# 4l3x4ndre/Metadata-Augmented-UNET-for-LST-NDVI

Measured on AMD Instinct MI355X. Metric: train images/sec (256x256x6->2 U-Net, B=32/GPU), higher is better.
Workload: dtype bf16; 1 GPU; metadata-unet base_filters=64, 32x6x256x256 tiles + 4-dim metadata per GPU, fwd+MSE+bwd+AdamW (src/train.py:243-256); global_batch=32, parallelism=dp1, sync_bn=False, launch=hipGraph replay of the captured step

## Files before the change

### include/mau_hip.h

```cpp
#ifndef MAU_HIP_H
#define MAU_HIP_H

#include <stddef.h>
#include <stdint.h>

#ifdef __cplusplus
extern "C" {
#endif

#define MAU_F32 0
#define MAU_BF16 1
#define MAU_F16 2

#define MAU_OK 0
#define MAU_ERR_ARG 1
#define MAU_ERR_HIP 2
#define MAU_ERR_DEVICE 3

typedef void* mau_stream_t;

#define MAU_ABI_VERSION 5
int mau_abi_version(void);
const char* mau_last_error(void);
int mau_device_check(void);

int mau_nchw_to_nhwc(const float* src, void* dst, int dtype, int N, int C, int H, int W, int ld,
                     mau_stream_t stream);
int mau_nhwc_to_nchw(const void* src, float* dst, int dtype, int N, int C, int H, int W, int ld,
                     mau_stream_t stream);

int mau_pack_tile_onehot(const unsigned char* cls_a, const unsigned char* cls_b, const float* cont,
                         const unsigned char* flip, void* out, int ldo, int dtype, int N, int H, int W,
                         int num_classes, int ncont, mau_stream_t stream);
int mau_flip_rows(const float* src, float* dst, const unsigned char* flip, int N, int C, int H, int W,
                  mau_stream_t stream);

int mau_conv3x3_kc(int dtype);
size_t mau_conv3x3_packed_elems(int dtype, int nout, int nin);
int mau_conv3x3_pack_weights(const float* w_oihw, void* wf, void* wd, int dtype, int Cout, int Cin,
                             mau_stream_t stream);
size_t mau_conv3x3_pack_desc_bytes(void);
int mau_conv3x3_pack_desc_fill(void* descs_host, int index, const float* w_oihw, void* wf, void* wd, int dtype, int Cout,
                               int Cin, int tile0, int* next_tile_host);
int mau_conv3x3_pack_weights_multi(const void* descs, int n, int total_tiles, int dtype, mau_stream_t stream);
int mau_conv3x3_num_pixel_tiles(int dtype, int N, int H, int W, int Cout);
int mau_conv3x3_fwd_pool(const void* x, int ldx, int C0, const void* wpk, const float* bias, const float* post_scale,
                         const float* post_shift, void* y, int ldy, int Cout, void* pooled, int ldpool, int dtype, int N, int H,
                         int W, mau_stream_t stream);
int mau_conv3x3_variant(int dtype, int N, int H, int W, int Cin, int Cout, int* tile_rows_host, int* waves_host, int* cout_block_host,
                        int* k_groups_host);
int mau_conv3x3_first_max_channels(void);
int mau_conv3x3_first_rows(int N, int H, int W);
size_t mau_conv3x3_first_wgrad_ws_elems(int N, int H, int W, int Cout);
int mau_conv3x3_first_wgrad(const void* x8, const void* dz, int lddz, float* dw_oihw, float* ws, int Cin, int Cout, int dtype, int N,
                            int H, int W, mau_stream_t stream);
int mau_conv3x3_first_fwd(const float* x_nchw, int Cin, const float* w_oihw, const float* bias, const float* post_scale,
                          const float* post_shift, void* y, int ldy, int Cout, float* slab, void* x8, int dtype, int N, int H,
                          int W, mau_stream_t stream);
int mau_conv3x3_fwd(const void* x, int ldx, int C0, const float* emb, void* emb_ws, int E, const void* wpk,
                    const float* bias, const float* post_scale, const float* post_shift, void* y, int ldy,
                    int Cout, float* slab, int dtype, int N, int H, int W, mau_stream_t stream);
int mau_conv3x3_fwd2(const void* x, int ldx, int C0, const void* x1, int ldx1, int C1, const float* emb, void* emb_ws,
                     int E, const void* wpk, const float* bias, const float* post_scale, const float* post_shift,
                     void* y, int ldy, int Cout, float* slab, int dtype, int N, int H, int W, mau_stream_t stream);
int mau_conv3x3_wgrad_splits(int dtype, int N, int H, int W, int Cout, int Cin);
size_t mau_conv3x3_wgrad_acc_elems(int dtype, int N, int H, int W, int Cout, int Cin);
int mau_conv3x3_wgrad(const void* x, int ldx, int C0, const float* emb, void* emb_ws, int E, const void* dy,
                      int lddy, int Cout, float* acc, int dtype, int N, int H, int W, mau_stream_t stream);
int mau_conv3x3_wgrad2(const void* x, int ldx, int C0, const void* x1, int ldx1, int C1, const float* emb, void* emb_ws,
                       int E, const void* dy, int lddy, int Cout, float* acc, int dtype, int N, int H, int W,
                       mau_stream_t stream);
int mau_conv3x3_unpack_wgrad(const float* acc, int nsplit, float* dw_oihw, int Cout, int Cin,
                             mau_stream_t stream);

size_t mau_reduce_rows_ws_elems(int rows, int M);
int mau_reduce_tickets_elems(void);
int mau_reduce_rows_f64(const float* slab, int rows, int M, int ldrow, double* sums, double* ws, unsigned* tickets,
                        mau_stream_t stream);
int mau_reduce_rows_f64_f32(const float* slab, int rows, int M, int ldrow, double* sums, float* sums32,
                            double* ws, unsigned* tickets, double append, mau_stream_t stream);
int mau_reduce_rows_f32(const float* slab, int rows, int M, int ldrow, float* out, double* ws, unsigned* tickets,
                        mau_stream_t stream);
int mau_bn_stats_sums_f64(const float* slab, int rows, int C, double* sums, double* ws, unsigned* tickets, double append,
                          mau_stream_t stream);
int mau_bn_finalize_train(const double* sums, double count, const float* gamma, const float* beta,
                          float* running_mean, float* running_var, int64_t* num_batches_tracked,
                          float momentum, float eps, float* scale, float* shift, float* mean,
                          float* invstd, int C, mau_stream_t stream);
size_t mau_bn_stats_ws_elems(int rows, int C);
int mau_bn_stats_finalize_train(const float* slab, int rows, double count, const float* gamma, const float* beta,
                                float* running_mean, float* running_var, int64_t* num_batches_tracked,
                                float momentum, float eps, float* scale, float* shift, float* mean, float* invstd,
                                double* ws, unsigned* tickets, int C, mau_stream_t stream);
int mau_bn_coeffs_eval(const float* gamma, const float* beta, const float* running_mean,
                       const float* running_var, float eps, float* scale, float* shift, float* mean,
                       float* invstd, int C, mau_stream_t stream);
int mau_bn_relu_apply(const void* y, int ldy, const float* scale, const float* shift, void* a, int lda,
                      int dtype, int64_t npix, int C, mau_stream_t stream);
int mau_bn_relu_apply_pool(const void* y, int ldy, const float* scale, const float* shift, void* a, int lda,
                           void* pooled, int ldp, unsigned short* argidx, int dtype, int N, int H, int W, int C,
                           mau_stream_t stream);
int mau_bn_relu_bwd_reduce(const void* da, int ldda, const void* y, int ldy, const float* scale,
                           const float* shift, const float* mean, const float* invstd, float* slab,
                           int ldslab, int dtype, int64_t npix, int C, mau_stream_t stream);
int mau_bn_relu_bwd_apply(const void* da, int ldda, const void* y, int ldy, const float* scale,
                          const float* shift, const float* mean, const float* invstd, const double* sums,
                          double count, void* dy, int lddy, int dtype, int64_t npix, int C,
                          mau_stream_t stream);
int mau_bn_bwd_rows(int64_t npix);

int mau_pool_bn_bwd_reduce(const void* y, int ldy, const void* dpl, int lddpl, const unsigned short* argidx,
                           const void* dskip, int lddskip,
                           const float* scale, const float* shift, const float* mean, const float* invstd, float* slab,
                           int ldslab, int dtype, int N, int H, int W, int C, mau_stream_t stream);
int mau_pool_bn_bwd_apply(const void* y, int ldy, const void* dpl, int lddpl, const unsigned short* argidx,
                          const void* dskip, int lddskip,
                          const float* scale, const float* shift, const float* mean, const float* invstd,
                          const double* sums, double count, void* dy, int lddy, int dtype, int N, int H, int W, int C,
                          mau_stream_t stream);
int mau_head_bn_max_channels(void);
int mau_head_bn_fwd(const void* y, int ldy, const float* scale, const float* shift, const float* w, const float* b, float* out,
                    int tanh0, int dtype, int N, int HW, int C, int Co, mau_stream_t stream);
int mau_head_bn_bwd_reduce(const void* y, int ldy, const float* scale, const float* shift, const float* mean,
                           const float* invstd, const float* w, const float* out, const float* dout, float* bn_slab,
                           int ldslab, float* head_slab, int tanh0, int dtype, int N, int HW, int C, int Co,
                           mau_stream_t stream);
int mau_head_bn_bwd_apply(const void* y, int ldy, const float* scale, const float* shift, const float* mean,
                          const float* invstd, const double* sums, double count, const float* w, const float* out,
                          const float* dout, void* dy, int lddy, int tanh0, int dtype, int N, int HW, int C, int Co,
                          mau_stream_t stream);

int mau_sum_tensors_max(void);
int mau_sum_tensors(const void* const* srcs, const int* lds, int k, void* dst, int lddst, int dtype, int64_t npix, int C,
                    mau_stream_t stream);

int mau_emb_fold_fwd(const float* w, const float* emb, float* weff, int Cout, int Ct, int E, int N, int Ep, mau_stream_t stream);
size_t mau_emb_fold_ws_elems(int Cout, int N, int E);
int mau_emb_fold_bwd(const float* w, const float* emb, const float* dweff, float* dw, float* demb, float* ws, int Cout, int Ct, int E,
                     int N, int Ep, mau_stream_t stream);

int mau_maxpool2x2_fwd(const void* x, int ldx, void* y, int ldy, int dtype, int N, int H, int W, int C,
                       mau_stream_t stream);
int mau_maxpool2x2_bwd(const void* x, int ldx, const void* dy, int lddy, void* dx, int lddx, int dtype,
                       int N, int H, int W, int C, mau_stream_t stream);
int mau_maxpool2x2_bwd_add(const void* x, int ldx, const void* dy, int lddy, const void* dskip, int lddskip, void* dx,
                           int lddx, int dtype, int N, int H, int W, int C, mau_stream_t stream);

int mau_resize_bilinear_fwd(const void* src, int ldsrc, int h, int w, void* dst, int lddst, int choff,
                            int dtype, int N, int H, int W, int C, mau_stream_t stream);
int mau_resize_bilinear_bn_fwd(const void* y, int ldy, int h, int w, const float* scale, const float* shift, void* dst,
                               int lddst, int choff, int dtype, int N, int H, int W, int C, mau_stream_t stream);
int mau_resize_bilinear_bwd(const void* ddst, int ldddst, int choff, int H, int W, void* dsrc, int lddsrc,
                            int dtype, int N, int h, int w, int C, mau_stream_t stream);
#define MAU_RESIZE_FWD_ROWCOL 0
#define MAU_RESIZE_FWD_CELL 1
#define MAU_RESIZE_FWD_DEST 2
#define MAU_RESIZE_BWD_2X2 0
#define MAU_RESIZE_BWD_GATHER 1
int mau_resize_bilinear_plan(int N, int h, int w, int H, int W, int C, int* fwd_kernel_host, int* fwd_rows_host, int* bwd_kernel_host);
int mau_copy_channels(const void* src, int ldsrc, void* dst, int lddst, int choff, int zero_to, int dtype,
                      int64_t npix, int C, mau_stream_t stream);
int mau_bcast_fill(const float* emb, void* dst, int lddst, int choff, int zero_to, int dtype, int N, int HW,
                   int E, mau_stream_t stream);
size_t mau_bcast_bwd_ws_elems(int N, int HW, int E);
int mau_bcast_bwd(const void* dx, int lddx, int choff, float* demb, float* ws, int dtype, int N, int HW, int E,
                  mau_stream_t stream);

int mau_head_fwd(const void* a, int lda, const float* w, const float* b, float* out, int tanh0, int dtype,
                 int N, int HW, int C, int Co, mau_stream_t stream);
size_t mau_head_mean_ws_elems(int N, int HW, int Co);
int mau_head_mean(const void* a, int lda, const float* w, const float* b, const double* scale, const double* shift,
                  double* means, double* ws, unsigned* tickets, int tanh0, int dtype, int N, int HW, int C, int Co,
                  mau_stream_t stream);
int mau_head_bwd(const void* a, int lda, const float* w, const float* out, const float* dout, void* da,
                 int ldda, float* slab, int tanh0, int dtype, int N, int HW, int C, int Co,
                 mau_stream_t stream);
int mau_head_bwd_rows(int N, int HW);
int mau_head_bwd_rowlen(int C, int Co);

int mau_meta_mlp_fwd(const float* md, const float* w0, const float* b0, const float* w2, const float* b2,
                     float* hidden, float* emb, int N, int F, int Hd, int D, mau_stream_t stream);
int mau_meta_mlp_bwd(const float* md, const float* w0, const float* w2, const float* hidden,
                     const float* demb, float* dw0, float* db0, float* dw2, float* db2, float* dhidden_ws,
                     int N, int F, int Hd, int D, mau_stream_t stream);

int mau_lstm_max_hidden(void);
int mau_lstm_fwd(const float* x, const float* w_ih, const float* w_hh, const float* b_ih, const float* b_hh,
                 float* h_last, float* gates, float* cells, int B, int T, int H, mau_stream_t stream);
size_t mau_lstm_bwd_ws_elems(int B, int T, int H);
int mau_lstm_bwd(const float* x, const float* w_hh, const float* gates, const float* cells, const float* dh_last,
                 float* dw_ih, float* dw_hh, float* db_ih, float* db_hh, float* ws, int B, int T, int H,
                 mau_stream_t stream);

int mau_linear_fwd(const float* x, const float* w, const float* b, float* out, int N, int F, int D, mau_stream_t stream);
int mau_linear_bwd(const float* x, const float* w, const float* dout, float* dx, float* dw, float* db, int N, int F,
                   int D, mau_stream_t stream);

size_t mau_adamw_pack_desc_bytes(void);
int mau_adamw_pack_desc_fill(void* descs_host, int index, float* w, const float* grad, float* exp_avg, float* exp_avg_sq,
                             void* wf, void* wd, int Cout, int Cin, int tile0, int* next_tile_host);
int mau_adamw_pack_step(const void* descs, int n, int total_tiles, int dtype, const float* step, float lr, float beta1,
                        float beta2, float eps, float weight_decay, mau_stream_t stream);

#define MAU_OPT_ADAMW 0
#define MAU_OPT_ADAM 1
#define MAU_OPT_SGD 2
int mau_opt_pack_desc_fill(void* descs_host, int index, float* w, const float* grad, float* m, float* v, void* wf, void* wd,
                           int Cout, int Cin, int tile0, int* next_tile_host);
// ... 107 lines not shown
```

### metadata-augmented-unet-for-lst-ndvi_amd/_lib.py

```python
from __future__ import annotations

import ctypes as C
import os

import torch

_HERE = os.path.dirname(os.path.abspath(__file__))
LIB_PATH = os.environ.get("MAU_LIB") or os.path.join(_HERE, "libmau_hip.so")

MAU_F32 = 0
MAU_BF16 = 1
MAU_F16 = 2
MAU_OPT_ADAMW, MAU_OPT_ADAM, MAU_OPT_SGD = 0, 1, 2

_p, _i, _i64, _f, _d, _sz = C.c_void_p, C.c_int, C.c_int64, C.c_float, C.c_double, C.c_size_t

PROTOTYPES = {
    "mau_abi_version": (_i, []),
    "mau_last_error": (C.c_char_p, []),
    "mau_device_check": (_i, []),
    "mau_nchw_to_nhwc": (_i, [_p, _p, _i, _i, _i, _i, _i, _i, _p]),
    "mau_pack_tile_onehot": (_i, [_p, _p, _p, _p, _p, _i, _i, _i, _i, _i, _i, _i, _p]),
    "mau_flip_rows": (_i, [_p, _p, _p, _i, _i, _i, _i, _p]),
    "mau_nhwc_to_nchw": (_i, [_p, _p, _i, _i, _i, _i, _i, _i, _p]),
    "mau_conv3x3_kc": (_i, [_i]),
    "mau_conv3x3_packed_elems": (_sz, [_i, _i, _i]),
    "mau_conv3x3_pack_weights": (_i, [_p, _p, _p, _i, _i, _i, _p]),
    "mau_conv3x3_pack_desc_bytes": (_sz, []),
    "mau_conv3x3_pack_desc_fill": (_i, [_p, _i, _p, _p, _p, _i, _i, _i, _i, _p]),
    "mau_conv3x3_pack_weights_multi": (_i, [_p, _i, _i, _i, _p]),
    "mau_conv3x3_num_pixel_tiles": (_i, [_i, _i, _i, _i, _i]),
    "mau_conv3x3_variant": (_i, [_i, _i, _i, _i, _i, _i, _p, _p, _p, _p]),
    "mau_conv3x3_first_max_channels": (_i, []),
    "mau_conv3x3_first_rows": (_i, [_i, _i, _i]),
    "mau_conv3x3_first_wgrad_ws_elems": (_sz, [_i, _i, _i, _i]),
    "mau_conv3x3_first_wgrad": (_i, [_p, _p, _i, _p, _p, _i, _i, _i, _i, _i, _i, _p]),
    "mau_conv3x3_first_fwd": (_i, [_p, _i, _p, _p, _p, _p, _p, _i, _i, _p, _p, _i, _i, _i, _i, _p]),
    "mau_conv3x3_fwd": (_i, [_p, _i, _i, _p, _p, _i, _p, _p, _p, _p, _p, _i, _i, _p, _i, _i, _i, _i, _p]),
    "mau_conv3x3_fwd_pool": (_i, [_p, _i, _i, _p, _p, _p, _p, _p, _i, _i, _p, _i, _i, _i, _i, _i, _p]),
    "mau_conv3x3_fwd2": (_i, [_p, _i, _i, _p, _i, _i, _p, _p, _i, _p, _p, _p, _p, _p, _i, _i, _p, _i, _i, _i, _i, _p]),
    "mau_conv3x3_wgrad_splits": (_i, [_i, _i, _i, _i, _i, _i]),
    "mau_conv3x3_wgrad_acc_elems": (_sz, [_i, _i, _i, _i, _i, _i]),
    "mau_conv3x3_wgrad": (_i, [_p, _i, _i, _p, _p, _i, _p, _i, _i, _p, _i, _i, _i, _i, _p]),
    "mau_conv3x3_wgrad2": (_i, [_p, _i, _i, _p, _i, _i, _p, _p, _i, _p, _i, _i, _p, _i, _i, _i, _i, _p]),
    "mau_conv3x3_unpack_wgrad": (_i, [_p, _i, _p, _i, _i, _p]),
    "mau_reduce_rows_ws_elems": (_sz, [_i, _i]),
    "mau_reduce_tickets_elems": (_i, []),
    "mau_reduce_rows_f64": (_i, [_p, _i, _i, _i, _p, _p, _p, _p]),
    "mau_reduce_rows_f64_f32": (_i, [_p, _i, _i, _i, _p, _p, _p, _p, _d, _p]),
    "mau_reduce_rows_f32": (_i, [_p, _i, _i, _i, _p, _p, _p, _p]),
    "mau_bn_stats_sums_f64": (_i, [_p, _i, _i, _p, _p, _p, _d, _p]),
    "mau_bn_finalize_train": (_i, [_p, _d, _p, _p, _p, _p, _p, _f, _f, _p, _p, _p, _p, _i, _p]),
    "mau_bn_stats_ws_elems": (_sz, [_i, _i]),
    "mau_bn_stats_finalize_train": (_i, [_p, _i, _d, _p, _p, _p, _p, _p, _f, _f, _p, _p, _p, _p, _p, _p, _i, _p]),
    "mau_bn_coeffs_eval": (_i, [_p, _p, _p, _p, _f, _p, _p, _p, _p, _i, _p]),
    "mau_bn_relu_apply": (_i, [_p, _i, _p, _p, _p, _i, _i, _i64, _i, _p]),
    "mau_bn_relu_apply_pool": (_i, [_p, _i, _p, _p, _p, _i, _p, _i, _p, _i, _i, _i, _i, _i, _p]),
    "mau_bn_relu_bwd_reduce": (_i, [_p, _i, _p, _i, _p, _p, _p, _p, _p, _i, _i, _i64, _i, _p]),
    "mau_bn_relu_bwd_apply": (_i, [_p, _i, _p, _i, _p, _p, _p, _p, _p, _d, _p, _i, _i, _i64, _i, _p]),
    "mau_bn_bwd_rows": (_i, [_i64]),
    "mau_pool_bn_bwd_reduce": (_i, [_p, _i, _p, _i, _p, _p, _i, _p, _p, _p, _p, _p, _i, _i, _i, _i, _i, _i, _p]),
    "mau_pool_bn_bwd_apply": (_i, [_p, _i, _p, _i, _p, _p, _i, _p, _p, _p, _p, _p, _d, _p, _i, _i, _i, _i, _i, _i, _p]),
    "mau_head_bn_max_channels": (_i, []),
    "mau_head_bn_fwd": (_i, [_p, _i, _p, _p, _p, _p, _p, _i, _i, _i, _i, _i, _i, _p]),
    "mau_head_bn_bwd_reduce": (_i, [_p, _i, _p, _p, _p, _p, _p, _p, _p, _p, _i, _p, _i, _i, _i, _i, _i, _i, _p]),
    "mau_head_bn_bwd_apply": (_i, [_p, _i, _p, _p, _p, _p, _p, _d, _p, _p, _p, _p, _i, _i, _i, _i, _i, _i, _i, _p]),
    "mau_resize_bilinear_bn_fwd": (_i, [_p, _i, _i, _i, _p, _p, _p, _i, _i, _i, _i, _i, _i, _i, _p]),
    "mau_maxpool2x2_fwd": (_i, [_p, _i, _p, _i, _i, _i, _i, _i, _i, _p]),
    "mau_maxpool2x2_bwd": (_i, [_p, _i, _p, _i, _p, _i, _i, _i, _i, _i, _i, _p]),
    "mau_maxpool2x2_bwd_add": (_i, [_p, _i, _p, _i, _p, _i, _p, _i, _i, _i, _i, _i, _i, _p]),
    "mau_resize_bilinear_fwd": (_i, [_p, _i, _i, _i, _p, _i, _i, _i, _i, _i, _i, _i, _p]),
    "mau_resize_bilinear_bwd": (_i, [_p, _i, _i, _i, _i, _p, _i, _i, _i, _i, _i, _i, _p]),
    "mau_resize_bilinear_plan": (_i, [_i, _i, _i, _i, _i, _i, _p, _p, _p]),
    "mau_copy_channels": (_i, [_p, _i, _p, _i, _i, _i, _i, _i64, _i, _p]),
    "mau_bcast_fill": (_i, [_p, _p, _i, _i, _i, _i, _i, _i, _i, _p]),
    "mau_bcast_bwd_ws_elems": (_sz, [_i, _i, _i]),
    "mau_bcast_bwd": (_i, [_p, _i, _i, _p, _p, _i, _i, _i, _i, _p]),
    "mau_head_fwd": (_i, [_p, _i, _p, _p, _p, _i, _i, _i, _i, _i, _i, _p]),
    "mau_head_mean_ws_elems": (_sz, [_i, _i, _i]),
    "mau_head_mean": (_i, [_p, _i, _p, _p, _p, _p, _p, _p, _p, _i, _i, _i, _i, _i, _i, _p]),
    "mau_head_bwd": (_i, [_p, _i, _p, _p, _p, _p, _i, _p, _i, _i, _i, _i, _i, _i, _p]),
    "mau_head_bwd_rows": (_i, [_i, _i]),
    "mau_head_bwd_rowlen": (_i, [_i, _i]),
    "mau_meta_mlp_fwd": (_i, [_p, _p, _p, _p, _p, _p, _p, _i, _i, _i, _i, _p]),
    "mau_meta_mlp_bwd": (_i, [_p, _p, _p, _p, _p, _p, _p, _p, _p, _p, _i, _i, _i, _i, _p]),
    "mau_lstm_max_hidden": (_i, []),
    "mau_lstm_fwd": (_i, [_p, _p, _p, _p, _p, _p, _p, _p, _i, _i, _i, _p]),
    "mau_lstm_bwd_ws_elems": (_sz, [_i, _i, _i]),
    "mau_lstm_bwd": (_i, [_p, _p, _p, _p, _p, _p, _p, _p, _p, _p, _i, _i, _i, _p]),
    "mau_linear_fwd": (_i, [_p, _p, _p, _p, _i, _i, _i, _p]),
    "mau_linear_bwd": (_i, [_p, _p, _p, _p, _p, _p, _i, _i, _i, _p]),
    "mau_adamw_pack_desc_bytes": (_sz, []),
    "mau_adamw_pack_desc_fill": (_i, [_p, _i, _p, _p, _p, _p, _p, _p, _i, _i, _i, _p]),
    "mau_adamw_pack_step": (_i, [_p, _i, _i, _i, _p, _f, _f, _f, _f, _f, _p]),
    "mau_opt_pack_desc_fill": (_i, [_p, _i, _p, _p, _p, _p, _p, _p, _i, _i, _i, _p]),
    "mau_opt_pack_step": (_i, [_p, _i, _i, _i, _i, _p, _p, _f, _f, _f, _f, _f, _i, _p]),
    "mau_grad_norm_chunk": (_i, []),
    "mau_grad_norm_seg_bytes": (_sz, []),
    "mau_grad_norm_seg_fill": (_i, [_p, _i, _p, _i64, _i, _p]),
    "mau_grad_norm_clip": (_i, [_p, _i, _i, _p, _p, _f, _p, _p, _p]),
    "mau_sum_tensors_max": (_i, []),
    "mau_sum_tensors": (_i, [_p, _p, _i, _p, _i, _i, _i64, _i, _p]),
    "mau_emb_fold_fwd": (_i, [_p, _p, _p, _i, _i, _i, _i, _i, _p]),
    "mau_emb_fold_ws_elems": (_sz, [_i, _i, _i]),
    "mau_emb_fold_bwd": (_i, [_p, _p, _p, _p, _p, _p, _i, _i, _i, _i, _i, _p]),
    "mau_eval_metrics_row_elems": (_i, [_i]),
    "mau_eval_metrics_chunks": (_i, [_i, _i]),
    "mau_eval_metrics_ws_elems": (_sz, [_i, _i, _i, _i, _i]),
    "mau_eval_metrics": (_i, [_p, _p, _p, _p, _p, _p, _p, _p, _i, _i, _i, _i, _i, _p]),
    "mau_eval_metrics_multi_max_models": (_i, []),
    "mau_eval_metrics_multi_ws_elems": (_sz, [_i, _i, _i, _i, _i, _i]),
    "mau_eval_metrics_multi": (_i, [_p, _p, _p, _p, _p, _p, _p, _p, _i, _i, _i, _i, _i, _i, _p]),
    "mau_paired_groups": (_i, []),
    "mau_paired_entry_elems": (_i, [_i]),
    "mau_paired_table_elems": (_sz, [_i, _i, _i]),
    "mau_paired_accumulate": (_i, [_p, _p, _p, _i, _i, _i, _i, _p]),
    "mau_rank_tile": (_i, []),
    "mau_rank_max_samples": (_i, []),
    "mau_rank_table_elems": (_sz, [_i, _i]),
    "mau_rank_ws_elems": (_sz, [_i, _i]),
    "mau_rank_tests": (_i, [_p, _p, _p, _p, _i, _i, _i, _i, _p]),
    "mau_scenario_max_classes": (_i, []),
    "mau_scenario_pack": (_i, [_p, _p, _p, _p, _p, _p, _p, _p, _p, _p, _i, _p, _i, _i, _i, _i, _i, _i, _i, _p]),
    "mau_scenario_result_row_elems": (_i, []),
    "mau_scenario_result_chunks": (_i, [_i, _i]),
    "mau_scenario_result_ws_elems": (_sz, [_i, _i, _i]),
    "mau_scenario_result": (_i, [_p, _p, _p, _p, _d, _d, _p, _p, _p, _p, _p, _p, _i, _i, _i, _p]),
    "mau_region_gather": (_i, [_p, _p, _p, _p, _p, _p, _p, _p, _i, _i, _i, _i, _i, _i, _i, _p]),
    "mau_region_stitch": (_i, [_p, _p, _p, _p, _i, _i, _i, _i, _i, _i, _i, _p]),
    "mau_compare_row_elems": (_i, []),
    "mau_compare_chunks": (_i, [_i, _i]),
    "mau_compare_ws_elems": (_sz, [_i, _i, _i]),
    "mau_compare_result": (_i, [_p, _p, _d, _d, _p, _p, _p, _p, _p, _p, _i, _i, _i, _p]),
    "mau_compare_inputs": (_i, [_p, _p, _p, _p, _p, _p, _p, _p, _p, _p, _i, _i, _i, _p]),
    "mau_moments_row_elems": (_i, []),
    "mau_plane_moments_chunks": (_i, [_i64]),
    "mau_plane_moments_ws_elems": (_sz, [_i, _i, _i64]),
    "mau_plane_moments": (_i, [_p, _p, _p, _p, _i, _i, _i64, _p]),
    "mau_bin_moments_max_entries": (_i, []),
    "mau_bin_moments": (_i, [_p, _p, _i, _p, _p, _p, _p, _p, _i, _i, _i, _i, _p]),
    "mau_tile_stats_row_elems": (_i, []),
    "mau_tile_stats_ws_elems": (_sz, [_i, _i64]),
    "mau_tile_stats": (_i, [_p, _p, _p, _p, _p, _p, _p, _i, _i64, _i, _p]),
    "mau_raw_tile_row_elems": (_i, []),
    "mau_raw_tile_ws_elems": (_sz, [_i, _i64]),
    "mau_raw_tile_process": (_i, [_p, _p, _p, _p, _p, _p, _p, _p, _p, _p, _p, _p, _p, _i, _i64, _i, _p]),
    "mau_climate_row_elems": (_i, []),
    "mau_climate_series_max_months": (_i, []),
    "mau_climate_baseline": (_i, [_p, _p, _i, _i, _p]),
    "mau_climate_normalise": (_i, [_p, _p, _p, _i, _i, _p]),
    "mau_climate_series": (_i, [_p, _p, _p, _p, _p, _p, _i, _i, _i, _i, _p]),
    "mau_mse_blocks": (_i, [_i64]),
    "mau_l1_gradient_blocks": (_i, [_i64]),
    "mau_l1_gradient_loss": (_i, [_p, _p, _p, _p, _p, _f, _f, _i, _i, _i, _i, _p]),
    "mau_ssim_ws_elems": (_sz, [_i, _i, _i, _i]),
    "mau_ssim_loss": (_i, [_p, _p, _p, _p, _p, _i, _i, _i, _i, _i, _p]),
    "mau_mse_fwd_bwd": (_i, [_p, _p, _p, _p, _p, _i64, _p]),
    "mau_loss_terms_ws_elems": (_sz, [_i, _i, _i, _i]),
    "mau_loss_terms": (_i, [_p, _p, _p, _p, _p, _p, _p, _f, _f, _i, _i, _i, _i, _p]),
}


class MauError(RuntimeError):
    pass


def _load():
    if not os.path.exists(LIB_PATH):
        raise ImportError(
            f"{LIB_PATH} not found: the MI355X-native HIP library has not been built "
            f"(run `python -c 'import __graft_entry__ as g; g.build()'` or `make -C {os.path.join(_HERE, 'csrc')}`). "
            "There is no CPU or PyTorch fallback for this path.")
    lib = C.CDLL(LIB_PATH)
    missing = [n for n in PROTOTYPES if not hasattr(lib, n)]
    if missing:
        raise ImportError(f"{LIB_PATH} does not export {missing}; rebuild it")
    for name, (res, args) in PROTOTYPES.items():
        fn = getattr(lib, name)
        fn.restype = res
        fn.argtypes = args
    return lib


lib = _load()


def check(status: int, what: str = ""):
    if status != 0:
        msg = lib.mau_last_error()
# ... 22 lines not shown
```

### metadata-augmented-unet-for-lst-ndvi_amd/csrc/bn.hip

```cpp
#include <stdlib.h>
#include "mau_common.h"

namespace mau {

template <int G, typename Load>
__device__ __forceinline__ void ordered_group(int& k, int end, Load load, double& s0, double& s1) {
  for (; k + 8 * (G - 1) + 4 < end; k += 8 * G) {
    double a[G], b[G];
#pragma unroll
    for (int i = 0; i < G; ++i) {
      a[i] = load(k + 8 * i);
      b[i] = load(k + 8 * i + 4);
    }
#pragma unroll
    for (int i = 0; i < G; ++i) {
      s0 += a[i];
      s1 += b[i];
    }
  }
}
template <typename Load>
__device__ __forceinline__ void ordered_pair_sum(int first, int end, Load load, double& s0, double& s1) {
  int k = first;
  ordered_group<16>(k, end, load, s0, s1);
  ordered_group<4>(k, end, load, s0, s1);
  for (; k + 4 < end; k += 8) {
    s0 += load(k);
    s1 += load(k + 4);
  }
  if (k < end) s0 += load(k);
}

template <typename InT, typename OutT>
__global__ __launch_bounds__(256) void reduce_rows_kernel(const InT* __restrict__ slab, int rows, int M, int ldrow,
                                                          OutT* __restrict__ out, int ldout, float* __restrict__ out32) {
  __shared__ double part[4][64];
  const int col = blockIdx.x * 64 + (threadIdx.x & 63);
  const int rl = threadIdx.x >> 6;
  const int per = (rows + gridDim.y - 1) / gridDim.y;
  const int r0 = blockIdx.y * per, r1 = min(rows, r0 + per);
  double s0 = 0.0, s1 = 0.0;
  if (col < M) {
    if (r0 + rl < r1) ordered_pair_sum(r0 + rl, r1, [&](int r) { return (double)slab[(size_t)r * ldrow + col]; }, s0, s1);
  }
  part[rl][threadIdx.x & 63] = s0 + s1;
  __syncthreads();
  if (rl == 0 && col < M) {
    const double v = part[0][threadIdx.x] + part[1][threadIdx.x] + part[2][threadIdx.x] + part[3][threadIdx.x];
    out[(size_t)blockIdx.y * ldout + col] = (OutT)v;
    if (out32 != nullptr) out32[col] = (float)v;
  }
}

constexpr int REDUCE_MAX_CHUNKS = 128;
static int reduce_chunks(int rows) {
  int c = rows / 32;
  if (c > REDUCE_MAX_CHUNKS) c = REDUCE_MAX_CHUNKS;
  return c < 1 ? 1 : c;
}

template <typename OutT>
static int reduce_rows_launch(const float* slab, int rows, int M, int ldrow, OutT* out, double* ws, hipStream_t st,
                              float* out32 = nullptr) {
  const int chunks = reduce_chunks(rows);
  float* const none = nullptr;
  if (chunks == 1 || ws == nullptr) {
    MAU_LAUNCH((reduce_rows_kernel<float, OutT>), dim3(ceil_div(M, 64), 1), dim3(256), 0, st, slab, rows, M, ldrow, out, M, out32);
  } else {
    MAU_LAUNCH((reduce_rows_kernel<float, double>), dim3(ceil_div(M, 64), chunks), dim3(256), 0, st, slab, rows, M, ldrow, ws, M, none);
    MAU_LAUNCH((reduce_rows_kernel<double, OutT>), dim3(ceil_div(M, 64), 1), dim3(256), 0, st, (const double*)ws, chunks, M, M, out, M, out32);
  }
  return check_launch("reduce_rows_kernel");
}


template <typename OutT>
__global__ __launch_bounds__(256) void reduce_rows_fused_kernel(const float* __restrict__ slab, int rows, int M, int ldrow, int split,
                                                                int gap, double* __restrict__ part, unsigned* __restrict__ tickets,
                                                                OutT* __restrict__ out, float* __restrict__ out32, double append) {
  __shared__ double ps[4][64];
  const int cl = threadIdx.x & 63, rl = threadIdx.x >> 6;
  const int j = blockIdx.x * 64 + cl;
  const int col = j < split ? j : j - split + gap;
  const int chunks = gridDim.y;
  const int per = (rows + chunks - 1) / chunks;
  const int r0 = blockIdx.y * per, r1 = min(rows, r0 + per);
  double s0 = 0.0, s1 = 0.0;
  if (j < M) {
    if (r0 + rl < r1) ordered_pair_sum(r0 + rl, r1, [&](int r) { return (double)slab[(size_t)r * ldrow + col]; }, s0, s1);
  }
  ps[rl][cl] = s0 + s1;
  __syncthreads();
  if (rl == 0 && j < M) part[(size_t)blockIdx.y * M + j] = ps[0][cl] + ps[1][cl] + ps[2][cl] + ps[3][cl];
  if (!last_block_of(tickets + blockIdx.x, (unsigned)chunks)) return;
  s0 = s1 = 0.0;
  if (j < M) {
    if (rl < chunks) ordered_pair_sum(rl, chunks, [&](int k) { return part[(size_t)k * M + j]; }, s0, s1);
  }
  ps[rl][cl] = s0 + s1;
  __syncthreads();
  if (rl == 0 && j < M) {
    const double v = ps[0][cl] + ps[1][cl] + ps[2][cl] + ps[3][cl];
    out[j] = (OutT)v;
    if (out32 != nullptr) out32[j] = (float)v;
  }
  if (append > 0.0 && blockIdx.x == 0 && threadIdx.x == 0) out[M] = (OutT)append;
}

template <typename OutT>
static int reduce_rows_fused_launch(const float* slab, int rows, int M, int ldrow, int split, int gap, OutT* out, double* ws,
                                    unsigned* tickets, hipStream_t st, float* out32 = nullptr, double append = 0.0) {
  const int chunks = reduce_chunks(rows);
  MAU_LAUNCH((reduce_rows_fused_kernel<OutT>), dim3(ceil_div(M, 64), chunks), dim3(256), 0, st, slab, rows, M, ldrow, split, gap, ws,
             tickets, out, out32, append);
  return check_launch("reduce_rows_fused_kernel");
}

__global__ void bn_finalize_train_kernel(const double* __restrict__ sums, double count, const float* __restrict__ gamma,
                                         const float* __restrict__ beta, float* __restrict__ rmean, float* __restrict__ rvar,
                                         int64_t* nbt, float momentum, float eps, float* __restrict__ scale,
                                         float* __restrict__ shift, float* __restrict__ mean_o, float* __restrict__ invstd_o,
                                         int C) {
  const int c = blockIdx.x * blockDim.x + threadIdx.x;
  if (c == 0 && nbt) *nbt += 1;
  if (c >= C) return;
  if (count <= 0.0) count = sums[2 * C];
  const double mean = sums[c] / count;
  double var = sums[C + c] / count - mean * mean;
  if (var < 0.0) var = 0.0;
  const float invstd = (float)(1.0 / sqrt(var + (double)eps));
  const float sc = gamma[c] * invstd;
  scale[c] = sc;
  shift[c] = beta[c] - (float)mean * sc;
  mean_o[c] = (float)mean;
  invstd_o[c] = invstd;
  if (rmean) {
    const double unbiased = count > 1.0 ? var * (count / (count - 1.0)) : var;
    rmean[c] = (1.f - momentum) * rmean[c] + momentum * (float)mean;
    rvar[c] = (1.f - momentum) * rvar[c] + momentum * (float)unbiased;
  }
}

__global__ __launch_bounds__(256) void bn_finalize_from_partials_kernel(const double* __restrict__ part, int chunks, int ldp, double count,
                                                 const float* __restrict__ gamma, const float* __restrict__ beta,
                                                 float* __restrict__ rmean, float* __restrict__ rvar, int64_t* nbt, float momentum,
                                                 float eps, float* __restrict__ scale, float* __restrict__ shift,
                                                 float* __restrict__ mean_o, float* __restrict__ invstd_o, int C) {
  __shared__ double ps[4][64], pq[4][64];
  const int cl = threadIdx.x & 63, kl = threadIdx.x >> 6;
  const int c = blockIdx.x * 64 + cl;
  if (blockIdx.x == 0 && threadIdx.x == 0 && nbt) *nbt += 1;
  double s0 = 0.0, q0 = 0.0, s1 = 0.0, q1 = 0.0;
  if (c < C && kl < chunks) {
// ... 132 lines not shown
#pragma unroll
      for (int u = 0; u < 4; ++u) {
        F8 o;
#pragma unroll
        for (int j = 0; j < 8; ++j) o.v[j] = fmaxf(fmaf(v[u].v[j], sc[j], sh[j]), 0.f);
        store8<T>(a + (pix + u * m.PS) * lda + c, o);
      }
    }
    for (; pix < p1; pix += m.PS) {
      const F8 v = load8<T>(y + pix * ldy + c);
      F8 o;
#pragma unroll
      for (int j = 0; j < 8; ++j) o.v[j] = fmaxf(fmaf(v.v[j], sc[j], sh[j]), 0.f);
      store8<T>(a + pix * lda + c, o);
    }
  }
}

template <typename T>
__global__ __launch_bounds__(256) void bn_relu_apply_pool_kernel(const T* __restrict__ y, int ldy, const float* __restrict__ scale,
                                                                 const float* __restrict__ shift, T* __restrict__ a, int lda,
                                                                 T* __restrict__ pl, int ldp, unsigned short* __restrict__ argidx, int H, int W,
                                                                 int C, int C8) {
  const int nv = C8 >> 3, Wc = (W + 1) >> 1, Ho = H >> 1, Wo = W >> 1;
  const int idx = blockIdx.x * 256 + threadIdx.x;
  if (idx >= Wc * nv) return;
  const int xo = idx / nv, c = (idx - xo * nv) * 8;
  const int yo = blockIdx.y, n = blockIdx.z;
  float sc[8], sh[8];
#pragma unroll
  for (int j = 0; j < 8; ++j) {
    sc[j] = coef(scale, c + j, C);
    sh[j] = coef(shift, c + j, C);
  }
  const int y0 = 2 * yo, x0 = 2 * xo;
  const bool hasx = x0 + 1 < W, hasy = y0 + 1 < H;
  const size_t row0 = ((size_t)n * H + y0) * W, row1 = row0 + W;
  F8 v[4];
  v[0] = load8<T>(y + (row0 + x0) * ldy + c);
  v[1] = hasx ? load8<T>(y + (row0 + x0 + 1) * ldy + c) : zero8();
  v[2] = hasy ? load8<T>(y + (row1 + x0) * ldy + c) : zero8();
  v[3] = (hasx && hasy) ? load8<T>(y + (row1 + x0 + 1) * ldy + c) : zero8();
  F8 o[4];
#pragma unroll
  for (int u = 0; u < 4; ++u)
#pragma unroll
    for (int j = 0; j < 8; ++j) o[u].v[j] = fmaxf(fmaf(v[u].v[j], sc[j], sh[j]), 0.f);
  store8<T>(a + (row0 + x0) * lda + c, o[0]);
  if (hasx) store8<T>(a + (row0 + x0 + 1) * lda + c, o[1]);
  if (hasy) store8<T>(a + (row1 + x0) * lda + c, o[2]);
  if (hasx && hasy) store8<T>(a + (row1 + x0 + 1) * lda + c, o[3]);
  if (yo < Ho && xo < Wo) {
    F8 m;
    unsigned bits = 0;
#pragma unroll
    for (int j = 0; j < 8; ++j) {
      const float a0 = opaque((float)(T)opaque(o[0].v[j])), a1 = opaque((float)(T)opaque(o[1].v[j]));
      const float a2 = opaque((float)(T)opaque(o[2].v[j])), a3 = opaque((float)(T)opaque(o[3].v[j]));
      unsigned arg = 0;
      float mx = a0;
      arg = a1 > mx ? 1u : arg;
      mx = fmaxf(mx, a1);
      arg = a2 > mx ? 2u : arg;
      mx = fmaxf(mx, a2);
      arg = a3 > mx ? 3u : arg;
      mx = fmaxf(mx, a3);
      m.v[j] = mx;
      bits |= arg << (2 * j);
    }
    store8<T>(pl + (((size_t)n * Ho + yo) * Wo + xo) * ldp + c, m);
    if (argidx != nullptr) argidx[(((size_t)n * Ho + yo) * Wo + xo) * nv + (c >> 3)] = (unsigned short)bits;
  }
}


template <typename T>
__global__ __launch_bounds__(256) void bn_relu_bwd_reduce_kernel(const T* __restrict__ da, int ldda, const T* __restrict__ y,
                                                                 int ldy, const float* __restrict__ scale,
                                                                 const float* __restrict__ shift, const float* __restrict__ mean,
                                                                 const float* __restrict__ invstd, float* __restrict__ slab,
                                                                 int ldslab, int64_t npix, int C) {
  __shared__ float red[2][32][64 + 1];
  const int cv = threadIdx.x & 7, ps = threadIdx.x >> 3;
  const int c0 = blockIdx.y * 64 + cv * 8;
  const int64_t p0 = (int64_t)blockIdx.x * BWD_PIX_PER_BLOCK;
  const int64_t p1 = p0 + BWD_PIX_PER_BLOCK < npix ? p0 + BWD_PIX_PER_BLOCK : npix;
  float s1[8], s2[8], sc[8], sh[8], mu[8], is[8];
#pragma unroll
  for (int j = 0; j < 8; ++j) {
    s1[j] = s2[j] = 0.f;
    const int cc = c0 + j;
    sc[j] = coef(scale, cc, C);
    sh[j] = coef(shift, cc, C);
    mu[j] = coef(mean, cc, C);
    is[j] = coef(invstd, cc, C);
  }
  if (c0 < C) {
    int64_t p = p0 + ps;
    for (; p + 32 < p1; p += 64) {
      F8 g[2], v[2];
#pragma unroll
      for (int u = 0; u < 2; ++u) {
        g[u] = load8<T>(da + (p + 32 * u) * ldda + c0);
        v[u] = load8<T>(y + (p + 32 * u) * ldy + c0);
      }
#pragma unroll
      for (int u = 0; u < 2; ++u)
#pragma unroll
        for (int j = 0; j < 8; ++j) {
          const float act = fmaf(v[u].v[j], sc[j], sh[j]);
          const float dz = act > 0.f ? g[u].v[j] : 0.f;
          s1[j] += dz;
          s2[j] = fmaf(dz, (v[u].v[j] - mu[j]) * is[j], s2[j]);
        }
    }
    for (; p < p1; p += 32) {
      const F8 g = load8<T>(da + p * ldda + c0);
      const F8 v = load8<T>(y + p * ldy + c0);
#pragma unroll
      for (int j = 0; j < 8; ++j) {
        const float act = fmaf(v.v[j], sc[j], sh[j]);
        const float dz = act > 0.f ? g.v[j] : 0.f;
        s1[j] += dz;
        s2[j] = fmaf(dz, (v.v[j] - mu[j]) * is[j], s2[j]);
      }
    }
  }
#pragma unroll
  for (int j = 0; j < 8; ++j) {
    red[0][ps][cv * 8 + j] = s1[j];
    red[1][ps][cv * 8 + j] = s2[j];
  }
  __syncthreads();
  if (threadIdx.x < 128) {
    const int which = threadIdx.x >> 6, c = threadIdx.x & 63;
    float s = 0.f;
#pragma unroll 8
    for (int r = 0; r < 32; ++r) s += red[which][r][c];
    const int cc = blockIdx.y * 64 + c;
    if (cc < ldslab) slab[((size_t)blockIdx.x * 2 + which) * ldslab + cc] = s;
  }
}

template <typename T, bool NT>
__global__ __launch_bounds__(256) void bn_relu_bwd_apply_kernel(const T* __restrict__ da, int ldda, const T* __restrict__ y,
                                                                int ldy, const float* __restrict__ scale,
                                                                const float* __restrict__ shift, const float* __restrict__ mean,
                                                                const float* __restrict__ invstd, const double* __restrict__ sums,
                                                                double inv_count, T* __restrict__ dy, int lddy, int64_t npix,
                                                                int C, int C8, int pixb) {
  const int nv = C8 >> 3;
  const PixVec m(nv);
  if (m.ps >= m.PS) return;
  if (inv_count <= 0.0) inv_count = 1.0 / sums[2 * C];
  const int64_t p0 = (int64_t)blockIdx.x * pixb;
  const int64_t p1 = p0 + pixb < npix ? p0 + pixb : npix;
  for (int vv = m.v; vv < nv; vv += m.nvl) {
    const int c = vv * 8;
    float sc[8], sh[8], k0[8], k1[8];
    double d1[8], d2[8];
#pragma unroll
    for (int j = 0; j < 8; ++j) {
      sc[j] = coef(scale, c + j, C);
      sh[j] = coef(shift, c + j, C);
      k0[j] = coef(mean, c + j, C);
      k1[j] = coef(invstd, c + j, C);
      d1[j] = coef(sums, c + j, C);
      d2[j] = coef(sums + C, c + j, C);
    }
#pragma unroll
    for (int j = 0; j < 8; ++j) {
      const float mu = k0[j], is = k1[j];
      const float m1 = (float)(d1[j] * inv_count), m2 = (float)(d2[j] * inv_count);
      k1[j] = __fmul_rn(__fmul_rn(sc[j], m2), is);
      k0[j] = fmaf(sc[j], m1, -__fmul_rn(k1[j], mu));
    }
    int64_t pix = p0 + m.ps;
    for (; pix + 3 * m.PS < p1; pix += 4 * m.PS) {
      F8 g[4], v[4];
#pragma unroll
      for (int u = 0; u < 4; ++u) {
        g[u] = NT ? load8_nt<T>(da + (pix + u * m.PS) * ldda + c) : load8<T>(da + (pix + u * m.PS) * ldda + c);
        v[u] = NT ? load8_nt<T>(y + (pix + u * m.PS) * ldy + c) : load8<T>(y + (pix + u * m.PS) * ldy + c);
      }
#pragma unroll
      for (int u = 0; u < 4; ++u) {
        F8 o;
#pragma unroll
        for (int j = 0; j < 8; ++j) {
          const float act = fmaf(v[u].v[j], sc[j], sh[j]);
          const float dz = act > 0.f ? g[u].v[j] : 0.f;
          o.v[j] = fmaf(sc[j], dz, -fmaf(k1[j], v[u].v[j], k0[j]));
        }
        if (NT) store8_nt<T>(dy + (pix + u * m.PS) * lddy + c, o); else store8<T>(dy + (pix + u * m.PS) * lddy + c, o);
      }
    }
    for (; pix < p1; pix += m.PS) {
      const F8 g = load8<T>(da + pix * ldda + c);
      const F8 v = load8<T>(y + pix * ldy + c);
      F8 o;
#pragma unroll
      for (int j = 0; j < 8; ++j) {
        const float act = fmaf(v.v[j], sc[j], sh[j]);
        const float dz = act > 0.f ? g.v[j] : 0.f;
        o.v[j] = fmaf(sc[j], dz, -fmaf(k1[j], v.v[j], k0[j]));
      }
      store8<T>(dy + pix * lddy + c, o);
    }
  }
}

}

using namespace mau;

extern "C" {

size_t mau_reduce_rows_ws_elems(int rows, int M) { return (size_t)reduce_chunks(rows) * M; }

int mau_reduce_tickets_elems(void) { return 64; }

#define MAU_REQUIRE_TICKETS(M) MAU_REQUIRE(tickets == nullptr || ceil_div((M), 64) <= mau_reduce_tickets_elems(), "reduce_rows: more than 4096 columns")

int mau_reduce_rows_f64(const float* slab, int rows, int M, int ldrow, double* sums, double* ws, unsigned* tickets,
                        mau_stream_t stream) {
  MAU_REQUIRE(slab && sums && rows > 0 && M > 0 && ldrow >= M, "reduce_rows: bad arguments");
  MAU_REQUIRE_TICKETS(M);
  if (tickets && ws) return reduce_rows_fused_launch<double>(slab, rows, M, ldrow, M, 0, sums, ws, tickets, (hipStream_t)stream);
  return reduce_rows_launch<double>(slab, rows, M, ldrow, sums, ws, (hipStream_t)stream);
}

int mau_reduce_rows_f64_f32(const float* slab, int rows, int M, int ldrow, double* sums, float* sums32, double* ws,
                            unsigned* tickets, double append, mau_stream_t stream) {
  MAU_REQUIRE(slab && sums && sums32 && rows > 0 && M > 0 && ldrow >= M, "reduce_rows: bad arguments");
  MAU_REQUIRE_TICKETS(M);
  MAU_REQUIRE(append <= 0.0 || (tickets && ws), "reduce_rows: the appended count needs the single-launch form (ws and tickets)");
  if (tickets && ws)
    return reduce_rows_fused_launch<double>(slab, rows, M, ldrow, M, 0, sums, ws, tickets, (hipStream_t)stream, sums32, append);
  return reduce_rows_launch<double>(slab, rows, M, ldrow, sums, ws, (hipStream_t)stream, sums32);
}

int mau_reduce_rows_f32(const float* slab, int rows, int M, int ldrow, float* out, double* ws, unsigned* tickets,
                        mau_stream_t stream) {
  MAU_REQUIRE(slab && out && rows > 0 && M > 0 && ldrow >= M, "reduce_rows: bad arguments");
  MAU_REQUIRE_TICKETS(M);
  if (tickets && ws) return reduce_rows_fused_launch<float>(slab, rows, M, ldrow, M, 0, out, ws, tickets, (hipStream_t)stream);
  return reduce_rows_launch<float>(slab, rows, M, ldrow, out, ws, (hipStream_t)stream);
}

int mau_bn_stats_sums_f64(const float* slab, int rows, int C, double* sums, double* ws, unsigned* tickets, double append,
                          mau_stream_t stream) {
  MAU_REQUIRE(slab && sums && ws && tickets && rows > 0 && C > 0, "bn_stats_sums: bad arguments");
  MAU_REQUIRE_TICKETS(2 * C);
  const int cpad = round_up(C, 64);
  return reduce_rows_fused_launch<double>(slab, rows, 2 * C, 2 * cpad, C, cpad, sums, ws, tickets, (hipStream_t)stream, nullptr, append);
}

int mau_bn_finalize_train(const double* sums, double count, const float* gamma, const float* beta,
                          float* running_mean, float* running_var, int64_t* nbt, float momentum, float eps,
                          float* scale, float* shift, float* mean, float* invstd, int C, mau_stream_t stream) {
  MAU_REQUIRE(sums && gamma && beta && scale && shift && mean && invstd && C > 0 && count >= 0, "bn_finalize_train: bad arguments");
  MAU_REQUIRE((running_mean == nullptr) == (running_var == nullptr), "bn_finalize_train: running_mean/var must come together");
  MAU_LAUNCH(bn_finalize_train_kernel, dim3(ceil_div(C, 256)), dim3(256), 0, (hipStream_t)stream, sums, count, gamma,
                     beta, running_mean, running_var, nbt, momentum, eps, scale, shift, mean, invstd, C);
  return check_launch("bn_finalize_train_kernel");
}

size_t mau_bn_stats_ws_elems(int rows, int C) { return (size_t)reduce_chunks(rows) * 2 * round_up(C, 64); }

int mau_bn_stats_finalize_train(const float* slab, int rows, double count, const float* gamma, const float* beta,
                                float* running_mean, float* running_var, int64_t* nbt, float momentum, float eps,
                                float* scale, float* shift, float* mean, float* invstd, double* ws, unsigned* tickets, int C,
                                mau_stream_t stream) {
  MAU_REQUIRE(slab && ws && gamma && beta && scale && shift && mean && invstd && rows > 0 && C > 0 && count > 0, "bn_stats_finalize_train: bad arguments");
  MAU_REQUIRE((running_mean == nullptr) == (running_var == nullptr), "bn_stats_finalize_train: running_mean/var must come together");
  hipStream_t st = (hipStream_t)stream;
  const int cpad = round_up(C, 64), M = 2 * cpad, chunks = reduce_chunks(rows);
  MAU_REQUIRE_TICKETS(cpad);
  if (tickets) {
    MAU_LAUNCH(bn_stats_finalize_fused_kernel, dim3(cpad / 64, chunks), dim3(256), 0, st, slab, rows, cpad, ws, tickets, count, gamma,
               beta, running_mean, running_var, nbt, momentum, eps, scale, shift, mean, invstd, C);
    return check_launch("bn_stats_finalize_fused_kernel");
  }
  MAU_LAUNCH((reduce_rows_kernel<float, double>), dim3(ceil_div(M, 64), chunks), dim3(256), 0, st, slab, rows, M, M, ws, M, (float*)nullptr);
  MAU_LAUNCH(bn_finalize_from_partials_kernel, dim3(ceil_div(C, 64)), dim3(256), 0, st, (const double*)ws, chunks, cpad, count, gamma,
             beta, running_mean, running_var, nbt, momentum, eps, scale, shift, mean, invstd, C);
  return check_launch("bn_stats_finalize_train");
}

int mau_bn_coeffs_eval(const float* gamma, const float* beta, const float* running_mean, const float* running_var,
                       float eps, float* scale, float* shift, float* mean, float* invstd, int C, mau_stream_t stream) {
  MAU_REQUIRE(gamma && beta && running_mean && running_var && scale && shift && C > 0, "bn_coeffs_eval: bad arguments");
  MAU_LAUNCH(bn_coeffs_eval_kernel, dim3(ceil_div(C, 256)), dim3(256), 0, (hipStream_t)stream, gamma, beta,
                     running_mean, running_var, eps, scale, shift, mean, invstd, C);
  return check_launch("bn_coeffs_eval_kernel");
}

int mau_bn_relu_apply(const void* y, int ldy, const float* scale, const float* shift, void* a, int lda, int dtype,
                      int64_t npix, int C, mau_stream_t stream) {
  MAU_REQUIRE(y && a && scale && shift && npix > 0 && C > 0, "bn_relu_apply: bad arguments");
  const int C8 = round_up(C, 8);
  MAU_REQUIRE(ldy % 8 == 0 && lda % 8 == 0 && ldy >= C8 && lda >= C8, "bn_relu_apply: bad ld");
  const bool big = npix >= (int64_t)1 << 20;
  const int pixb = pixvec_pixels_per_block(C8 / 8, npix, big ? 8 : 32, big ? 2048 : 256);
  MAU_DISPATCH_DTYPE(dtype, MAU_LAUNCH(bn_relu_apply_kernel<T>, dim3(ceil_div(npix, pixb)), dim3(256), 0, (hipStream_t)stream,
                                               (const T*)y, ldy, scale, shift, (T*)a, lda, npix, C, C8, pixb));
  return check_launch("bn_relu_apply_kernel");
}

int mau_bn_relu_apply_pool(const void* y, int ldy, const float* scale, const float* shift, void* a, int lda, void* pooled,
                           int ldp, unsigned short* argidx, int dtype, int N, int H, int W, int C, mau_stream_t stream) {
  MAU_REQUIRE(y && a && pooled && scale && shift && N > 0 && H >= 2 && W >= 2 && C > 0, "bn_relu_apply_pool: bad arguments");
  const int C8 = round_up(C, 8);
  MAU_REQUIRE(ldy % 8 == 0 && lda % 8 == 0 && ldp % 8 == 0 && ldy >= C8 && lda >= C8 && ldp >= C8, "bn_relu_apply_pool: bad ld");
  MAU_REQUIRE((H + 1) / 2 <= 65535 && N <= 65535, "bn_relu_apply_pool: H/2 and N must fit a grid dimension");
  dim3 grid(ceil_div(((W + 1) / 2) * (C8 / 8), 256), (H + 1) / 2, N);
  MAU_DISPATCH_DTYPE(dtype, MAU_LAUNCH(bn_relu_apply_pool_kernel<T>, grid, dim3(256), 0, (hipStream_t)stream, (const T*)y, ldy, scale,
                                       shift, (T*)a, lda, (T*)pooled, ldp, argidx, H, W, C, C8));
  return check_launch("bn_relu_apply_pool_kernel");
}

int mau_bn_bwd_rows(int64_t npix) { return ceil_div(npix, BWD_PIX_PER_BLOCK); }

int mau_bn_relu_bwd_reduce(const void* da, int ldda, const void* y, int ldy, const float* scale, const float* shift,
                           const float* mean, const float* invstd, float* slab, int ldslab, int dtype, int64_t npix,
                           int C, mau_stream_t stream) {
  MAU_REQUIRE(da && y && scale && shift && mean && invstd && slab && npix > 0 && C > 0, "bn_relu_bwd_reduce: bad arguments");
  const int C8 = round_up(C, 8);
  MAU_REQUIRE(ldda % 8 == 0 && ldy % 8 == 0 && ldda >= C8 && ldy >= C8 && ldslab >= C, "bn_relu_bwd_reduce: bad ld");
  dim3 grid(mau_bn_bwd_rows(npix), ceil_div(C, 64));
  MAU_DISPATCH_DTYPE(dtype, MAU_LAUNCH(bn_relu_bwd_reduce_kernel<T>, grid, dim3(256), 0, (hipStream_t)stream,
                                               (const T*)da, ldda, (const T*)y, ldy, scale, shift, mean, invstd, slab,
                                               ldslab, npix, C));
  return check_launch("bn_relu_bwd_reduce_kernel");
}

int mau_bn_relu_bwd_apply(const void* da, int ldda, const void* y, int ldy, const float* scale, const float* shift,
                          const float* mean, const float* invstd, const double* sums, double count, void* dy, int lddy,
                          int dtype, int64_t npix, int C, mau_stream_t stream) {
  MAU_REQUIRE(da && y && dy && sums && scale && shift && mean && invstd && npix > 0 && C > 0 && count >= 0, "bn_relu_bwd_apply: bad arguments");
  const int C8 = round_up(C, 8);
  MAU_REQUIRE(ldda % 8 == 0 && ldy % 8 == 0 && lddy % 8 == 0 && ldda >= C8 && ldy >= C8 && lddy >= C8, "bn_relu_bwd_apply: bad ld");
  const int pixb = pixvec_pixels_per_block(C8 / 8, npix, 64, 256);
  MAU_DISPATCH_DTYPE(dtype, MAU_LAUNCH((bn_relu_bwd_apply_kernel<T, false>), dim3(ceil_div(npix, pixb)), dim3(256), 0, (hipStream_t)stream,
                                               (const T*)da, ldda, (const T*)y, ldy, scale, shift, mean, invstd, sums,
                                               count > 0 ? 1.0 / count : 0.0, (T*)dy, lddy, npix, C, C8, pixb));
  return check_launch("bn_relu_bwd_apply_kernel");
}

}
```

### metadata-augmented-unet-for-lst-ndvi_amd/csrc/bn_fused.hip

```cpp
#include "mau_common.h"

namespace mau {

template <typename T>
__device__ __forceinline__ float round_to(float v) {
  return opaque((float)(T)opaque(v));
}

typedef float f2 __attribute__((ext_vector_type(2)));
__device__ __forceinline__ f2 pk_fma(f2 a, f2 b, f2 c) { return __builtin_elementwise_fma(a, b, c); }
__device__ __forceinline__ f2 splat(float v) { return f2{v, v}; }
template <typename T>
__device__ __forceinline__ f2 round_to2(f2 v) {
  if constexpr (sizeof(T) == 4) return v;
  else if constexpr (__is_same(T, bf16)) {
    typedef __bf16 b2 __attribute__((ext_vector_type(2)));
    asm("" : "+v"(v));
    f2 r = __builtin_convertvector(__builtin_convertvector(v, b2), f2);
    asm("" : "+v"(r));
    return r;
  } else return f2{round_to<T>(v[0]), round_to<T>(v[1])};
}
template <typename T>
struct P4 {
  f2 p[4];
  __device__ __forceinline__ static P4 load(const T* ptr) {
    const F8 v = load8<T>(ptr);
    P4 r;
#pragma unroll
    for (int i = 0; i < 4; ++i) r.p[i] = f2{v.v[2 * i], v.v[2 * i + 1]};
    return r;
  }
};

struct Coef8 {
  float sc[8], sh[8], mu[8], is[8];
  __device__ __forceinline__ void load(const float* scale, const float* shift, const float* mean, const float* invstd, int c0, int C) {
#pragma unroll
    for (int j = 0; j < 8; ++j) {
      sc[j] = coef(scale, c0 + j, C);
      sh[j] = coef(shift, c0 + j, C);
      mu[j] = mean ? coef(mean, c0 + j, C) : 0.f;
      is[j] = invstd ? coef(invstd, c0 + j, C) : 0.f;
    }
  }
};

template <typename T>
struct PoolLoads {
  F8 g, sk;
  unsigned bits;
  bool inpool;
  int me;
};
template <typename T, bool POOL, bool SKIP>
__device__ __forceinline__ PoolLoads<T> pool_load(const T* __restrict__ dpl, int lddpl, const unsigned short* __restrict__ argidx, int nv,
                                                  const T* __restrict__ dskip, int lddskip, int n, int yi, int xi, int H, int W, int c0) {
  PoolLoads<T> L;
  const int Ho = H >> 1, Wo = W >> 1, yo = yi >> 1, xo = xi >> 1;
  L.inpool = POOL && yo < Ho && xo < Wo;
  L.me = (yi & 1) * 2 + (xi & 1);
  L.bits = 0;
  if constexpr (POOL) {
    const int yc = yo < Ho ? yo : Ho - 1, xc = xo < Wo ? xo : Wo - 1;
    const size_t win = ((size_t)n * Ho + yc) * Wo + xc;
    L.g = load8<T>(dpl + win * lddpl + c0);
    L.bits = argidx[win * nv + (c0 >> 3)];
  }
  if constexpr (SKIP) L.sk = load8<T>(dskip + (((size_t)n * H + yi) * W + xi) * lddskip + c0);
  return L;
}
template <typename T, bool POOL, bool SKIP>
__device__ __forceinline__ F8 pool_eval(const PoolLoads<T>& L) {
  F8 o;
#pragma unroll
  for (int j = 0; j < 8; ++j) {
    float r = 0.f;
    if constexpr (POOL) r = (L.inpool && (int)((L.bits >> (2 * j)) & 3u) == L.me) ? L.g.v[j] : 0.f;
    if constexpr (SKIP) r += L.sk.v[j];
    o.v[j] = round_to<T>(r);
  }
  return o;
}

__device__ __forceinline__ void bn_sums_to_slab(float (*red)[32][64 + 1], const float* s1, const float* s2, int cv, int ps, float* slab,
                                                int ldslab) {
#pragma unroll
  for (int j = 0; j < 8; ++j) {
    red[0][ps][cv * 8 + j] = s1[j];
    red[1][ps][cv * 8 + j] = s2[j];
  }
  __syncthreads();
  if (threadIdx.x < 128) {
    const int which = threadIdx.x >> 6, c = threadIdx.x & 63;
    float s = 0.f;
#pragma unroll 8
    for (int r = 0; r < 32; ++r) s += red[which][r][c];
    const int cc = blockIdx.y * 64 + c;
    if (cc < ldslab) slab[((size_t)blockIdx.x * 2 + which) * ldslab + cc] = s;
  }
}

__device__ __forceinline__ void advance32(int& n, int& yi, int& xi, int H, int W) {
  xi += 32;
  while (xi >= W) {
    xi -= W;
    if (++yi == H) {
      yi = 0;
      ++n;
    }
  }
}
template <typename T, bool POOL, bool SKIP>
__global__ __launch_bounds__(256) void pool_bn_bwd_reduce_kernel(const T* __restrict__ y, int ldy, const T* __restrict__ dpl, int lddpl,
                                                                 const unsigned short* __restrict__ argidx,
                                                                 const T* __restrict__ dskip, int lddskip, const float* __restrict__ scale,
                                                                 const float* __restrict__ shift, const float* __restrict__ mean,
                                                                 const float* __restrict__ invstd, float* __restrict__ slab, int ldslab,
                                                                 int H, int W, int64_t npix, int C) {
  __shared__ float red[2][32][64 + 1];
  const int cv = threadIdx.x & 7, ps = threadIdx.x >> 3;
  const int c0 = blockIdx.y * 64 + cv * 8;
  const int64_t p0 = (int64_t)blockIdx.x * BWD_PIX_PER_BLOCK;
  const int64_t p1 = p0 + BWD_PIX_PER_BLOCK < npix ? p0 + BWD_PIX_PER_BLOCK : npix;
  Coef8 k;
  k.load(scale, shift, mean, invstd, c0, C);
  float s1[8], s2[8];
#pragma unroll
  for (int j = 0; j < 8; ++j) s1[j] = s2[j] = 0.f;
  auto accumulate = [&](const F8& v, const F8& g) {
#pragma unroll
    for (int j = 0; j < 8; ++j) {
      const float act = fmaf(v.v[j], k.sc[j], k.sh[j]);
      const float dz = act > 0.f ? g.v[j] : 0.f;
      s1[j] += dz;
      s2[j] = fmaf(dz, (v.v[j] - k.mu[j]) * k.is[j], s2[j]);
    }
  };
  if (c0 < C) {
    int64_t p = p0 + ps;
    const int HW = H * W, nv = (C + 7) >> 3;
    int n = (int)(p / HW), r = (int)(p - (int64_t)n * HW);
    int yi = r / W, xi = r - yi * W;
    for (; p + 32 < p1; p += 64) {
      int n2 = n, yi2 = yi, xi2 = xi;
      advance32(n2, yi2, xi2, H, W);
      const F8 va = load8<T>(y + p * ldy + c0), vb = load8<T>(y + (p + 32) * ldy + c0);
      const PoolLoads<T> La = pool_load<T, POOL, SKIP>(dpl, lddpl, argidx, nv, dskip, lddskip, n, yi, xi, H, W, c0);
      const PoolLoads<T> Lb = pool_load<T, POOL, SKIP>(dpl, lddpl, argidx, nv, dskip, lddskip, n2, yi2, xi2, H, W, c0);
      accumulate(va, pool_eval<T, POOL, SKIP>(La));
      accumulate(vb, pool_eval<T, POOL, SKIP>(Lb));
      n = n2, yi = yi2, xi = xi2;
      advance32(n, yi, xi, H, W);
    }
    for (; p < p1; p += 32) {
      const F8 v = load8<T>(y + p * ldy + c0);
      const PoolLoads<T> L = pool_load<T, POOL, SKIP>(dpl, lddpl, argidx, nv, dskip, lddskip, n, yi, xi, H, W, c0);
      accumulate(v, pool_eval<T, POOL, SKIP>(L));
      advance32(n, yi, xi, H, W);
    }
  }
  bn_sums_to_slab(red, s1, s2, cv, ps, slab, ldslab);
}

struct Apply8 {
  float sc[8], sh[8], k0[8], k1[8];
  __device__ __forceinline__ void load(const float* scale, const float* shift, const float* mean, const float* invstd, const double* sums,
                                       double inv_count, int c0, int C) {
    double d1[8], d2[8];
#pragma unroll
    for (int j = 0; j < 8; ++j) {
      sc[j] = coef(scale, c0 + j, C);
      sh[j] = coef(shift, c0 + j, C);
      k0[j] = coef(mean, c0 + j, C);
      k1[j] = coef(invstd, c0 + j, C);
      d1[j] = coef(sums, c0 + j, C);
      d2[j] = coef(sums + C, c0 + j, C);
    }
#pragma unroll
    for (int j = 0; j < 8; ++j) {
      const float mu = k0[j], is = k1[j];
      const float m1 = (float)(d1[j] * inv_count), m2 = (float)(d2[j] * inv_count);
      k1[j] = __fmul_rn(__fmul_rn(sc[j], m2), is);
      k0[j] = fmaf(sc[j], m1, -__fmul_rn(k1[j], mu));
    }
  }
  __device__ __forceinline__ float dy(int j, float yv, float da) const {
    const float act = fmaf(yv, sc[j], sh[j]);
    const float dz = act > 0.f ? da : 0.f;
    return fmaf(sc[j], dz, -fmaf(k1[j], yv, k0[j]));
  }
};

template <typename T, bool POOL, bool SKIP>
__global__ __launch_bounds__(256) void pool_bn_bwd_apply_kernel(const T* __restrict__ y, int ldy, const T* __restrict__ dpl, int lddpl,
                                                                const unsigned short* __restrict__ argidx,
                                                                const T* __restrict__ dskip, int lddskip, const float* __restrict__ scale,
                                                                const float* __restrict__ shift, const float* __restrict__ mean,
                                                                const float* __restrict__ invstd, const double* __restrict__ sums,
                                                                double inv_count, T* __restrict__ dyo, int lddy, int H, int W, int C, int C8,
                                                                int RY) {
  const int nv = C8 >> 3, Wc = (W + 1) >> 1, Hc = (H + 1) >> 1, Ho = H >> 1, Wo = W >> 1;
  const int idx = blockIdx.x * 256 + threadIdx.x;
  if (idx >= Wc * nv) return;
  const int xo = idx / nv, c = (idx - xo * nv) * 8;
  const int n = blockIdx.z;
  if (inv_count <= 0.0) inv_count = 1.0 / sums[2 * C];
  Apply8 k;
  k.load(scale, shift, mean, invstd, sums, inv_count, c, C);
  const int x0 = 2 * xo;
  const bool hasx = x0 + 1 < W;
  const int x1 = hasx ? x0 + 1 : x0;
  const int xpc = xo < Wo ? xo : Wo - 1;
  for (int yo = blockIdx.y * RY; yo < min(Hc, (int)(blockIdx.y + 1) * RY); ++yo) {
    const int y0 = 2 * yo;
    const bool hasy = y0 + 1 < H;
    const size_t row0 = ((size_t)n * H + y0) * W, row1 = ((size_t)n * H + (hasy ? y0 + 1 : y0)) * W;
    F8 v[4], d[4], g;
    v[0] = load8<T>(y + (row0 + x0) * ldy + c);
    v[1] = load8<T>(y + (row0 + x1) * ldy + c);
    v[2] = load8<T>(y + (row1 + x0) * ldy + c);
    v[3] = load8<T>(y + (row1 + x1) * ldy + c);
    if constexpr (SKIP) {
      d[0] = load8<T>(dskip + (row0 + x0) * lddskip + c);
      d[1] = load8<T>(dskip + (row0 + x1) * lddskip + c);
      d[2] = load8<T>(dskip + (row1 + x0) * lddskip + c);
      d[3] = load8<T>(dskip + (row1 + x1) * lddskip + c);
    }
    const bool inpool = POOL && yo < Ho && xo < Wo;
    unsigned bits = 0;
    if constexpr (POOL) {
      const size_t win = ((size_t)n * Ho + (yo < Ho ? yo : Ho - 1)) * Wo + xpc;
      g = load8<T>(dpl + win * lddpl + c);
      bits = argidx[win * nv + (c >> 3)];
    }
    F8 o[4];
#pragma unroll
    for (int j = 0; j < 8; ++j) {
      const int arg = inpool ? (int)((bits >> (2 * j)) & 3u) : -1;
#pragma unroll
      for (int u = 0; u < 4; ++u) {
        float r = 0.f;
        if constexpr (POOL) r = arg == u ? g.v[j] : 0.f;
        if constexpr (SKIP) r += d[u].v[j];
        o[u].v[j] = k.dy(j, v[u].v[j], round_to<T>(r));
      }
    }
    store8<T>(dyo + (row0 + x0) * lddy + c, o[0]);
    if (hasx) store8<T>(dyo + (row0 + x0 + 1) * lddy + c, o[1]);
    if (hasy) store8<T>(dyo + (row1 + x0) * lddy + c, o[2]);
    if (hasx && hasy) store8<T>(dyo + (row1 + x0 + 1) * lddy + c, o[3]);
  }
}

__device__ __forceinline__ void pos_step32(int& n, int& q, int HW) {
  q += 32;
  const bool w = q >= HW;
  q -= w ? HW : 0;
  n += w ? 1 : 0;
}

template <typename T, int MC, bool EX, bool BN = true>
__global__ __launch_bounds__(256) void head_bn_fwd_kernel(const T* __restrict__ y, int ldy, const float* __restrict__ scale,
                                                          const float* __restrict__ shift, const float* __restrict__ w,
                                                          const float* __restrict__ b, float* __restrict__ out, int tanh0, int HW, int C,
                                                          int Co, int64_t npix, int pixb) {
  const int sub = threadIdx.x & 7, ps = threadIdx.x >> 3;
  float wr[MC][8];
#pragma unroll
  for (int o = 0; o < MC; ++o)
#pragma unroll
    for (int j = 0; j < 8; ++j) wr[o][j] = (EX || o < Co) ? coef(w + o * C, sub * 8 + j, C) : 0.f;
  Coef8 k;
  if (BN) k.load(scale, shift, nullptr, nullptr, sub * 8, C);
  float bo[MC];
#pragma unroll
  for (int o = 0; o < MC; ++o) bo[o] = (EX || o < Co) ? b[o] : 0.f;
  const int64_t p0 = (int64_t)blockIdx.x * pixb;
  const int64_t p1 = p0 + pixb < npix ? p0 + pixb : npix;
  int n = (int)((p0 + ps) / HW);
  int q = (int)((p0 + ps) - (int64_t)n * HW);
  for (int64_t p = p0 + ps; p - ps < p1; p += 128) {
    F8 x[4];
    int nn[4], qq[4];
#pragma unroll
    for (int u = 0; u < 4; ++u) {
      const int64_t pix = p + 32 * u;
      const int64_t pc = pix < npix ? pix : npix - 1;
      x[u] = load8<T>(y + pc * ldy + (sub * 8 < C ? sub * 8 : 0));
      nn[u] = n;
      qq[u] = q;
      pos_step32(n, q, HW);
    }
    float acc[4][MC];
#pragma unroll
    for (int u = 0; u < 4; ++u) {
#pragma unroll
      for (int o = 0; o < MC; ++o) acc[u][o] = 0.f;
      if (sub * 8 < C) {
#pragma unroll
        for (int j = 0; j < 8; ++j) {
          const float a = BN ? round_to<T>(fmaxf(fmaf(x[u].v[j], k.sc[j], k.sh[j]), 0.f)) : x[u].v[j];
#pragma unroll
          for (int o = 0; o < MC; ++o) acc[u][o] = fmaf(a, wr[o][j], acc[u][o]);
        }
      }
#pragma unroll
      for (int o = 0; o < MC; ++o) {
        acc[u][o] += __shfl_xor(acc[u][o], 1);
        acc[u][o] += __shfl_xor(acc[u][o], 2);
        acc[u][o] += __shfl_xor(acc[u][o], 4);
      }
    }
    const int us = sub & 3;
    const int nu = us == 0 ? nn[0] : us == 1 ? nn[1] : us == 2 ? nn[2] : nn[3];
    const int qu = us == 0 ? qq[0] : us == 1 ? qq[1] : us == 2 ? qq[2] : qq[3];
    const bool live = sub < 4 && p + 32 * us < p1;
#pragma unroll
    for (int o = 0; o < MC; ++o) {
      if (EX || o < Co) {
        float r = us == 0 ? acc[0][o] : us == 1 ? acc[1][o] : us == 2 ? acc[2][o] : acc[3][o];
        r += bo[o];
        if (o == 0 && tanh0) r = tanhf(r);
        if (live) out[((size_t)nu * Co + o) * HW + qu] = r;
      }
    }
  }
}

template <int MC, bool EX>
__device__ __forceinline__ void head_dz(const float* __restrict__ out, const float* __restrict__ dout, int tanh0, int Co, int HW, int n,
                                        int q, float* dz) {
  const size_t base = (size_t)n * Co * HW + q;
  const float t = out[base];
  const float f0 = tanh0 ? fmaf(-t, t, 1.f) : 1.f;
#pragma unroll
  for (int o = 0; o < MC; ++o) {
    const float g = dout[base + (size_t)((EX || o < Co) ? o : Co - 1) * HW];
    dz[o] = (EX || o < Co) ? (o == 0 ? g * f0 : g) : 0.f;
  }
}

constexpr int HEAD_WAVES = 3;
template <typename T, int MC, bool EX>
__global__ __launch_bounds__(256, HEAD_WAVES) void head_bn_bwd_reduce_kernel(const T* __restrict__ y, int ldy, const float* __restrict__ scale,
                                                                 const float* __restrict__ shift, const float* __restrict__ mean,
                                                                 const float* __restrict__ invstd, const float* __restrict__ w,
                                                                 const float* __restrict__ out, const float* __restrict__ dout,
                                                                 float* __restrict__ bn_slab, int ldslab, float* __restrict__ head_slab,
                                                                 int tanh0, int HW, int C, int C8, int Co, int64_t npix) {
  __shared__ float red[2][32][64 + 1];
  __shared__ float hred[32 * HEAD_MAX_CO * 65];
  const int cv = threadIdx.x & 7, ps = threadIdx.x >> 3;
  const int c0 = cv * 8;
  const int64_t p0 = (int64_t)blockIdx.x * BWD_PIX_PER_BLOCK;
  const int64_t p1 = p0 + BWD_PIX_PER_BLOCK < npix ? p0 + BWD_PIX_PER_BLOCK : npix;
  const int rowlen = Co * (C8 + 8);
  float* row = head_slab + (size_t)blockIdx.x * rowlen;
  Coef8 k;
  k.load(scale, shift, mean, invstd, c0, C);
  f2 sc2[4], sh2[4], mu2[4], is2[4], s1p[4], s2p[4], dwq[MC][4], wq[MC][4];
  float dbp[MC];
#pragma unroll
  for (int i = 0; i < 4; ++i) {
    sc2[i] = f2{k.sc[2 * i], k.sc[2 * i + 1]};
    sh2[i] = f2{k.sh[2 * i], k.sh[2 * i + 1]};
    mu2[i] = f2{k.mu[2 * i], k.mu[2 * i + 1]};
    is2[i] = f2{k.is[2 * i], k.is[2 * i + 1]};
    s1p[i] = s2p[i] = f2{0.f, 0.f};
  }
#pragma unroll
  for (int o = 0; o < MC; ++o) {
    dbp[o] = 0.f;
#pragma unroll
    for (int i = 0; i < 4; ++i) {
      dwq[o][i] = f2{0.f, 0.f};
      wq[o][i] = f2{o < Co ? coef(w + o * C, c0 + 2 * i, C) : 0.f, o < Co ? coef(w + o * C, c0 + 2 * i + 1, C) : 0.f};
    }
  }
  auto one = [&](const P4<T>& v, const float* dz) {
#pragma unroll
    for (int o = 0; o < MC; ++o) dbp[o] += dz[o];
#pragma unroll
    for (int i = 0; i < 4; ++i) {
      const f2 act = pk_fma(v.p[i], sc2[i], sh2[i]);
      const f2 a = round_to2<T>(f2{fmaxf(act[0], 0.f), fmaxf(act[1], 0.f)});
      f2 s = f2{0.f, 0.f};
#pragma unroll
      for (int o = 0; o < MC; ++o)
        if (EX || o < Co) {
          s = pk_fma(splat(dz[o]), wq[o][i], s);
          dwq[o][i] = pk_fma(splat(dz[o]), a, dwq[o][i]);
        }
      const f2 da = round_to2<T>(s);
      const f2 dzb = f2{act[0] > 0.f ? da[0] : 0.f, act[1] > 0.f ? da[1] : 0.f};
      s1p[i] += dzb;
      s2p[i] = pk_fma(dzb, (v.p[i] - mu2[i]) * is2[i], s2p[i]);
    }
  };
  struct Raw {
    P4<T> v;
    float t, g[MC];
  };
  auto fetch = [&](int64_t pa, int na, int qa, Raw& r) {
    r.v = P4<T>::load(y + pa * ldy + c0);
    const size_t base = (size_t)na * Co * HW + qa;
    r.t = out[base];
#pragma unroll
    for (int o = 0; o < MC; ++o) r.g[o] = dout[base + (size_t)((EX || o < Co) ? o : Co - 1) * HW];
  };
  auto eval = [&](const Raw& r) {
    float dz[MC];
    const float f0 = tanh0 ? fmaf(-r.t, r.t, 1.f) : 1.f;
#pragma unroll
    for (int o = 0; o < MC; ++o) dz[o] = (EX || o < Co) ? (o == 0 ? r.g[o] * f0 : r.g[o]) : 0.f;
    one(r.v, dz);
  };
  if (c0 < C8) {
    int n = (int)((p0 + ps) / HW);
    int q = (int)((p0 + ps) - (int64_t)n * HW);
    int64_t p = p0 + ps;
    if (p + 32 < p1) {
      Raw a, b;
      int n2 = n, q2 = q;
      pos_step32(n2, q2, HW);
      fetch(p, n, q, a);
      fetch(p + 32, n2, q2, b);
      n = n2;
      q = q2;
      pos_step32(n, q, HW);
      for (; p + 96 < p1; p += 64) {
        Raw na, nb;
        n2 = n;
        q2 = q;
        pos_step32(n2, q2, HW);
        fetch(p + 64, n, q, na);
        fetch(p + 96, n2, q2, nb);
        eval(a);
        eval(b);
        a = na;
        b = nb;
        n = n2;
        q = q2;
        pos_step32(n, q, HW);
      }
      eval(a);
      eval(b);
      p += 64;
    }
    for (; p < p1; p += 32) {
      Raw r;
      fetch(p, n, q, r);
      eval(r);
      pos_step32(n, q, HW);
    }
  }
  float s1[8], s2[8], dwp[MC][8];
#pragma unroll
  for (int i = 0; i < 4; ++i) {
    s1[2 * i] = s1p[i][0];
    s1[2 * i + 1] = s1p[i][1];
    s2[2 * i] = s2p[i][0];
    s2[2 * i + 1] = s2p[i][1];
#pragma unroll
    for (int o = 0; o < MC; ++o) {
      dwp[o][2 * i] = dwq[o][i][0];
      dwp[o][2 * i + 1] = dwq[o][i][1];
    }
  }
#pragma unroll
  for (int o = 0; o < MC; ++o)
    if (EX || o < Co) {
#pragma unroll
      for (int j = 0; j < 8; ++j) hred[(ps * HEAD_MAX_CO + o) * 65 + cv * 8 + j] = dwp[o][j];
    }
  __syncthreads();
  for (int t = threadIdx.x; t < Co * 64; t += 256) {
    const int o = t >> 6, c = t & 63;
    float s = 0.f;
    for (int r = 0; r < 32; ++r) s += hred[(r * HEAD_MAX_CO + o) * 65 + c];
    if (c < C8) row[o * (C8 + 8) + c] = s;
  }
  __syncthreads();
  if (cv == 0) {
#pragma unroll
    for (int o = 0; o < MC; ++o)
      if (o < Co) hred[ps * HEAD_MAX_CO + o] = dbp[o];
  }
  __syncthreads();
  if (threadIdx.x < Co) {
    float s = 0.f;
    for (int r = 0; r < 32; ++r) s += hred[r * HEAD_MAX_CO + threadIdx.x];
    row[threadIdx.x * (C8 + 8) + C8] = s;
  }
  bn_sums_to_slab(red, s1, s2, cv, ps, bn_slab, ldslab);
}

template <typename T, int MC, bool EX>
__global__ __launch_bounds__(256) void head_bn_bwd_apply_kernel(const T* __restrict__ y, int ldy, const float* __restrict__ scale,
                                                                const float* __restrict__ shift, const float* __restrict__ mean,
                                                                const float* __restrict__ invstd, const double* __restrict__ sums,
                                                                double inv_count, const float* __restrict__ w, const float* __restrict__ out,
                                                                const float* __restrict__ dout, T* __restrict__ dyo, int lddy, int tanh0,
                                                                int HW, int C, int Co, int64_t npix, int pixb) {
  const int cv = threadIdx.x & 7, ps = threadIdx.x >> 3;
  const int c0 = cv * 8;
  if (c0 >= ((C + 7) & ~7)) return;
  if (inv_count <= 0.0) inv_count = 1.0 / sums[2 * C];
  Apply8 k;
  k.load(scale, shift, mean, invstd, sums, inv_count, c0, C);
  float wr[MC][8];
#pragma unroll
  for (int o = 0; o < MC; ++o)
#pragma unroll
    for (int j = 0; j < 8; ++j) wr[o][j] = o < Co ? coef(w + o * C, c0 + j, C) : 0.f;
  const int64_t p0 = (int64_t)blockIdx.x * pixb;
  const int64_t p1 = p0 + pixb < npix ? p0 + pixb : npix;
  int n = (int)((p0 + ps) / HW);
  int q = (int)((p0 + ps) - (int64_t)n * HW);
  auto one = [&](int64_t p, const F8& v, const float* dz) {
    F8 o8;
#pragma unroll
    for (int j = 0; j < 8; ++j) {
      float s = 0.f;
#pragma unroll
      for (int o = 0; o < MC; ++o)
        if (EX || o < Co) s = fmaf(dz[o], wr[o][j], s);
      o8.v[j] = k.dy(j, v.v[j], round_to<T>(s));
    }
    store8<T>(dyo + p * lddy + c0, o8);
  };
  int64_t p = p0 + ps;
  for (; p + 96 < p1; p += 128) {
    int nn[4], qq[4];
    F8 v[4];
    float dz[4][MC];
#pragma unroll
    for (int u = 0; u < 4; ++u) {
      nn[u] = n;
      qq[u] = q;
      pos_step32(n, q, HW);
    }
#pragma unroll
    for (int u = 0; u < 4; ++u) {
      v[u] = load8<T>(y + (p + 32 * u) * ldy + c0);
      head_dz<MC, EX>(out, dout, tanh0, Co, HW, nn[u], qq[u], dz[u]);
    }
#pragma unroll
    for (int u = 0; u < 4; ++u) one(p + 32 * u, v[u], dz[u]);
  }
  for (; p < p1; p += 32) {
    float dz[MC];
    const F8 v = load8<T>(y + p * ldy + c0);
    head_dz<MC, EX>(out, dout, tanh0, Co, HW, n, q, dz);
    one(p, v, dz);
    pos_step32(n, q, HW);
  }
}

int head_fwd_fast(const void* a, int lda, const float* w, const float* b, float* out, int tanh0, int dtype, int64_t npix, int HW, int C, int Co,
                  hipStream_t stream) {
  const int pixb = npix >= ((int64_t)1 << 20) ? 1024 : 128;
  const dim3 grid(ceil_div(npix, pixb));
  const float* none = nullptr;
#define MAU_HEAD_PLAIN(MC_, EX_)                                                                                                            \
  MAU_DISPATCH_DTYPE(dtype, MAU_LAUNCH((head_bn_fwd_kernel<T, MC_, EX_, false>), grid, dim3(256), 0, stream, (const T*)a, lda, none, none, w, b, out, \
                                       tanh0, HW, C, Co, npix, pixb))
  if (Co == 2) MAU_HEAD_PLAIN(2, true);
  else if (Co == 1) MAU_HEAD_PLAIN(2, false);
  else if (Co == HEAD_MAX_CO) MAU_HEAD_PLAIN(HEAD_MAX_CO, true);
  else MAU_HEAD_PLAIN(HEAD_MAX_CO, false);
#undef MAU_HEAD_PLAIN
  return check_launch("head_fwd_kernel");
}

}

using namespace mau;

extern "C" {

int mau_pool_bn_bwd_reduce(const void* y, int ldy, const void* dpl, int lddpl, const unsigned short* argidx, const void* dskip, int lddskip, const float* scale,
                           const float* shift, const float* mean, const float* invstd, float* slab, int ldslab, int dtype, int N, int H,
                           int W, int C, mau_stream_t stream) {
  MAU_REQUIRE(y && (dpl || dskip) && (!dpl || argidx) && scale && shift && mean && invstd && slab && N > 0 && H >= 2 && W >= 2 && C > 0, "pool_bn_bwd_reduce: bad arguments");
  const int C8 = round_up(C, 8);
  MAU_REQUIRE(ldy % 8 == 0 && ldy >= C8 && (!dpl || (lddpl % 8 == 0 && lddpl >= C8)) && (!dskip || (lddskip % 8 == 0 && lddskip >= C8)) && ldslab >= C,
              "pool_bn_bwd_reduce: bad ld");
  const int64_t npix = (int64_t)N * H * W;
  dim3 grid(ceil_div(npix, BWD_PIX_PER_BLOCK), ceil_div(C, 64));
#define MAU_POOL_REDUCE(P, S)                                                                                                                  \
  MAU_DISPATCH_DTYPE(dtype, MAU_LAUNCH((pool_bn_bwd_reduce_kernel<T, P, S>), grid, dim3(256), 0, (hipStream_t)stream, (const T*)y, ldy, (const T*)dpl, \
                                       lddpl, argidx, (const T*)dskip, lddskip, scale, shift, mean, invstd, slab, ldslab, H, W, npix, C))
  if (dpl && dskip) MAU_POOL_REDUCE(true, true);
  else if (dpl) MAU_POOL_REDUCE(true, false);
  else MAU_POOL_REDUCE(false, true);
#undef MAU_POOL_REDUCE
  return check_launch("pool_bn_bwd_reduce_kernel");
}

int mau_pool_bn_bwd_apply(const void* y, int ldy, const void* dpl, int lddpl, const unsigned short* argidx, const void* dskip, int lddskip, const float* scale,
                          const float* shift, const float* mean, const float* invstd, const double* sums, double count, void* dy, int lddy,
                          int dtype, int N, int H, int W, int C, mau_stream_t stream) {
  MAU_REQUIRE(y && (dpl || dskip) && (!dpl || argidx) && dy && sums && scale && shift && mean && invstd && N > 0 && H >= 2 && W >= 2 && C > 0 && count >= 0,
              "pool_bn_bwd_apply: bad arguments");
  const int C8 = round_up(C, 8);
  MAU_REQUIRE(ldy % 8 == 0 && ldy >= C8 && lddy % 8 == 0 && lddy >= C8 && (!dpl || (lddpl % 8 == 0 && lddpl >= C8)) &&
                  (!dskip || (lddskip % 8 == 0 && lddskip >= C8)), "pool_bn_bwd_apply: bad ld");
  MAU_REQUIRE((H + 1) / 2 <= 65535 && N <= 65535, "pool_bn_bwd_apply: H/2 and N must fit a grid dimension");
  const int xb = ceil_div(((W + 1) / 2) * (C8 / 8), 256), Hc = (H + 1) / 2;
  int RY = 8;
  while (RY > 1 && (int64_t)xb * ceil_div(Hc, RY) * N < 1024) RY >>= 1;
  dim3 grid(xb, ceil_div(Hc, RY), N);
#define MAU_POOL_APPLY(P, S)                                                                                                                   \
  MAU_DISPATCH_DTYPE(dtype, MAU_LAUNCH((pool_bn_bwd_apply_kernel<T, P, S>), grid, dim3(256), 0, (hipStream_t)stream, (const T*)y, ldy, (const T*)dpl, lddpl, \
                                       argidx, (const T*)dskip, lddskip, scale, shift, mean, invstd, sums, count > 0 ? 1.0 / count : 0.0, (T*)dy, lddy, \
                                       H, W, C, C8, RY))
  if (dpl && dskip) MAU_POOL_APPLY(true, true);
  else if (dpl) MAU_POOL_APPLY(true, false);
  else MAU_POOL_APPLY(false, true);
#undef MAU_POOL_APPLY
  return check_launch("pool_bn_bwd_apply_kernel");
}

int mau_head_bn_max_channels(void) { return 64; }

int mau_head_bn_fwd(const void* y, int ldy, const float* scale, const float* shift, const float* w, const float* b, float* out, int tanh0,
                    int dtype, int N, int HW, int C, int Co, mau_stream_t stream) {
  MAU_REQUIRE(y && scale && shift && w && b && out && N > 0 && HW > 0 && C > 0, "head_bn_fwd: bad arguments");
  MAU_REQUIRE(Co >= 1 && Co <= HEAD_MAX_CO && C <= mau_head_bn_max_channels(), "head_bn_fwd: out_channels in [1,%d], C <= %d", HEAD_MAX_CO,
              mau_head_bn_max_channels());
  MAU_REQUIRE(ldy % 8 == 0 && ldy >= round_up(C, 8), "head_bn_fwd: bad ld");
  MAU_REQUIRE(HW >= 32 && (int64_t)N * HW < ((int64_t)1 << 31), "head_bn_fwd: images of at least 32 pixels, fewer than 2^31 pixels in all");
  const int64_t npix = (int64_t)N * HW;
  const int pixb = npix >= ((int64_t)1 << 20) ? 1024 : 128;
  const dim3 grid(ceil_div(npix, pixb));
#define MAU_HEAD_FWD(MC_, EX_)                                                                                                              \
  MAU_DISPATCH_DTYPE(dtype, MAU_LAUNCH((head_bn_fwd_kernel<T, MC_, EX_>), grid, dim3(256), 0, (hipStream_t)stream, (const T*)y, ldy, scale, shift, w, b, \
                                       out, tanh0, HW, C, Co, npix, pixb))
  if (Co == 2) MAU_HEAD_FWD(2, true);
  else if (Co == 1) MAU_HEAD_FWD(2, false);
  else if (Co == HEAD_MAX_CO) MAU_HEAD_FWD(HEAD_MAX_CO, true);
  else MAU_HEAD_FWD(HEAD_MAX_CO, false);
#undef MAU_HEAD_FWD
  return check_launch("head_bn_fwd_kernel");
}

int mau_head_bn_bwd_reduce(const void* y, int ldy, const float* scale, const float* shift, const float* mean, const float* invstd,
                           const float* w, const float* out, const float* dout, float* bn_slab, int ldslab, float* head_slab, int tanh0,
                           int dtype, int N, int HW, int C, int Co, mau_stream_t stream) {
  MAU_REQUIRE(y && scale && shift && mean && invstd && w && out && dout && bn_slab && head_slab && N > 0 && HW > 0 && C > 0,
              "head_bn_bwd_reduce: bad arguments");
  MAU_REQUIRE(Co >= 1 && Co <= HEAD_MAX_CO && C <= mau_head_bn_max_channels(), "head_bn_bwd_reduce: out_channels in [1,%d], C <= %d", HEAD_MAX_CO,
              mau_head_bn_max_channels());
  const int C8 = round_up(C, 8);
  MAU_REQUIRE(ldy % 8 == 0 && ldy >= C8 && ldslab >= C, "head_bn_bwd_reduce: bad ld");
  MAU_REQUIRE(HW >= 32 && (int64_t)N * HW < ((int64_t)1 << 31), "head_bn_bwd_reduce: images of at least 32 pixels, fewer than 2^31 pixels in all");
  const int64_t npix = (int64_t)N * HW;
#define MAU_HEAD_RED(MC_, EX_)                                                                                                              \
  MAU_DISPATCH_DTYPE(dtype, MAU_LAUNCH((head_bn_bwd_reduce_kernel<T, MC_, EX_>), dim3(ceil_div(npix, BWD_PIX_PER_BLOCK)), dim3(256), 0, (hipStream_t)stream, \
                                       (const T*)y, ldy, scale, shift, mean, invstd, w, out, dout, bn_slab, ldslab, head_slab, tanh0, HW, C, C8, Co, npix))
// ... 33 lines not shown
```

### metadata-augmented-unet-for-lst-ndvi_amd/csrc/conv3x3_first.hip

```cpp
#include "igemm_bf16_util.h"

namespace mau {
namespace first {
using namespace igemm;

constexpr int TH = 16, TW = 64, HR = TH + 2, HC = TW + 2, HPIX = HR * HC;
constexpr int NT = 256, NWAVE = NT / 64;
constexpr int LOADS = (HPIX + NT - 1) / NT;
typedef float f32x4v __attribute__((ext_vector_type(4)));

struct P {
  const float* x;
  int Cin;
  const float* w;
  const float* bias;
  const float* post_scale;
  const float* post_shift;
  void* y;
  int ldy, Cout, CoutPad;
  float* slab;
  void* x8;
  int N, H, W, tilesX, tilesY, nTiles;
};

template <bool F16>
__device__ __forceinline__ f32x4v mfma(const bf16x8& a, const bf16x8& b, f32x4v c) {
  if constexpr (F16) return __builtin_amdgcn_mfma_f32_16x16x32_f16(__builtin_bit_cast(f16x8, a), __builtin_bit_cast(f16x8, b), c, 0, 0, 0);
  else return __builtin_amdgcn_mfma_f32_16x16x32_bf16(a, b, c, 0, 0, 0);
}

template <bool F16>
__device__ __forceinline__ u32x4 pack8(const float (&v)[8]) {
  u32x4 r;
#pragma unroll
  for (int i = 0; i < 4; ++i) {
    if constexpr (F16) r[i] = pack_lp2<true>(f32x2{opaque(v[2 * i]), opaque(v[2 * i + 1])});
    else r[i] = pack_lp2<false>(f32x2{v[2 * i], v[2 * i + 1]});
  }
  return r;
}

__device__ __forceinline__ int chan_of(int t, int q, int r) { return 32 * (t >> 1) + 8 * q + 4 * (t & 1) + r; }

constexpr int FIRST_UNROLL = 2;
constexpr int FIRST_WAVES = 2;
template <bool F16, int EPI>
__global__ __launch_bounds__(NT, FIRST_WAVES) void first_fwd_kernel(P p) {
  __shared__ __attribute__((aligned(16))) unsigned char halo[HPIX * 16];
  __shared__ float red[NWAVE][2 * 64];
  const int tid = threadIdx.x, lane = tid & 63, wave = tid >> 6;
  const int q = lane >> 4, n = lane & 15;
  const int co0 = blockIdx.y * 64;

  bf16x8 A[3][4];
  {
    float* wl = reinterpret_cast<float*>(halo);
    static_assert(64 * 8 * 9 * sizeof(float) <= sizeof(halo), "weight tile fits the halo buffer");
    const int rowlen = p.Cin * 9, nrows = min(64, p.Cout - co0);
    const float* wsrc = p.w + (size_t)co0 * rowlen;
    for (int i = tid; i < nrows * rowlen; i += NT) wl[i] = wsrc[i];
    __syncthreads();
#pragma unroll
    for (int s = 0; s < 3; ++s)
#pragma unroll
      for (int t = 0; t < 4; ++t) {
        const int col = chan_of(t, n >> 2, n & 3), tau = 4 * s + q;
        float v[8];
#pragma unroll
        for (int j = 0; j < 8; ++j) {
          const bool ok = tau < 9 && j < p.Cin && col < nrows;
          const float wv = wl[ok ? (col * p.Cin + j) * 9 + tau : 0];
          v[j] = ok ? wv : 0.f;
        }
        A[s][t] = __builtin_bit_cast(bf16x8, pack8<F16>(v));
      }
  }
  f32x2 bb2[4][2], psc2[4][2], psh2[4][2], s1[4][2], s2[4][2];
#pragma unroll
  for (int t = 0; t < 4; ++t)
#pragma unroll
    for (int h = 0; h < 2; ++h) {
#pragma unroll
      for (int e = 0; e < 2; ++e) {
        const int co = co0 + chan_of(t, q, 2 * h + e);
        const float bv = p.bias != nullptr ? coef(p.bias, co, p.Cout) : 0.f;
        bb2[t][h][e] = bv;
        if (EPI == EPI_POST) {
          psc2[t][h][e] = coef(p.post_scale, co, p.Cout);
          psh2[t][h][e] = fmaf(psc2[t][h][e], bv, coef(p.post_shift, co, p.Cout));
        }
      }
      s1[t][h] = s2[t][h] = f32x2{0.f, 0.f};
    }
  unsigned lane_lds[3];
#pragma unroll
  for (int s = 0; s < 3; ++s) {
    const int tau = min(4 * s + q, 8), dy = tau / 3, dx = tau - 3 * dy;
    lane_lds[s] = (unsigned)((dy * HC + n + dx) * 16);
  }
  const int wv = __builtin_amdgcn_readfirstlane(wave);

  const bool lowhalf = n < 8;
  const int ch1 = lowhalf ? q : 4 + q, ch2 = lowhalf ? 4 + q : q;
  const bool st1 = co0 + 8 * ch1 < p.ldy, st2 = co0 + 8 * ch2 < p.ldy;
  const unsigned off1 = (unsigned)(((n & 7) * p.ldy + co0 + 8 * ch1) * 2), off2 = (unsigned)(((8 + (n & 7)) * p.ldy + co0 + 8 * ch2) * 2);
  unsigned char* const yb = reinterpret_cast<unsigned char*>(p.y);
  const size_t plane = (size_t)p.H * p.W;

  float hv[LOADS][8];
  auto coords = [&](int item, int& img, int& ty0, int& tx0) {
    const int txi = item % p.tilesX;
    item /= p.tilesX;
    img = item / p.tilesY;
    ty0 = (item - img * p.tilesY) * TH;
    tx0 = txi * TW;
  };
  auto fetch = [&](int item) {
    int img, ty0, tx0;
    coords(item, img, ty0, tx0);
    const float* src[LOADS];
    bool in[LOADS];
#pragma unroll
    for (int k = 0; k < LOADS; ++k) {
      const int pidx = tid + k * NT;
      const int hy = pidx / HC, hx = pidx - hy * HC;
      const int gy = ty0 + hy - 1, gx = tx0 + hx - 1;
      in[k] = pidx < HPIX && gy >= 0 && gy < p.H && gx >= 0 && gx < p.W;
      src[k] = p.x + (size_t)img * p.Cin * plane + (in[k] ? (size_t)gy * p.W + gx : 0);
    }
#pragma unroll
    for (int c = 0; c < 8; ++c) {
      if (c < p.Cin) {
#pragma unroll
        for (int k = 0; k < LOADS; ++k) {
          const float v = src[k][(size_t)c * plane];
          hv[k][c] = in[k] ? v : 0.f;
        }
      } else {
#pragma unroll
        for (int k = 0; k < LOADS; ++k) hv[k][c] = 0.f;
      }
    }
  };
  auto commit = [&](int item) {
    int img, ty0, tx0;
    coords(item, img, ty0, tx0);
#pragma unroll
    for (int k = 0; k < LOADS; ++k) {
      const int pidx = tid + k * NT;
      if (pidx < HPIX) {
        const u32x4 pk = pack8<F16>(hv[k]);
        *reinterpret_cast<u32x4*>(halo + pidx * 16) = pk;
// ... 25 lines not shown
#pragma unroll FIRST_UNROLL
        for (int gc = 0; gc < 4; ++gc) {
          const int cx = gc * 16;
          const unsigned la = (unsigned)((ry * HC + cx) * 16);
          f32x4v acc[4];
#pragma unroll
          for (int t = 0; t < 4; ++t) acc[t] = f32x4v{0.f, 0.f, 0.f, 0.f};
#pragma unroll
          for (int s = 0; s < 3; ++s) {
            const bf16x8 B = *reinterpret_cast<const bf16x8*>(halo + lane_lds[s] + la);
#pragma unroll
            for (int t = 0; t < 4; ++t) acc[t] = mfma<F16>(A[s][t], B, acc[t]);
          }
          const bool valid = FULL || (yok && tx0 + cx + n < p.W);
          f32x2 v[4][2];
#pragma unroll
          for (int t = 0; t < 4; ++t)
#pragma unroll
            for (int h = 0; h < 2; ++h) {
              f32x2 o = f32x2{acc[t][2 * h], acc[t][2 * h + 1]};
              if (EPI != EPI_POST) o += bb2[t][h];
              if (EPI == EPI_STATS) {
                const f32x2 m = FULL ? o : (valid ? o : f32x2{0.f, 0.f});
                s1[t][h] += m;
                s2[t][h] = __builtin_elementwise_fma(m, m, s2[t][h]);
              }
              if (EPI == EPI_POST) o = __builtin_elementwise_max(__builtin_elementwise_fma(o, psc2[t][h], psh2[t][h]), f32x2{0.f, 0.f});
              v[t][h] = o;
            }
          const u32x4 plo = {pack_lp2<F16>(v[0][0]), pack_lp2<F16>(v[0][1]), pack_lp2<F16>(v[1][0]), pack_lp2<F16>(v[1][1])};
          const u32x4 phi = {pack_lp2<F16>(v[2][0]), pack_lp2<F16>(v[2][1]), pack_lp2<F16>(v[3][0]), pack_lp2<F16>(v[3][1])};
          u32x4 d1, d2;
#pragma unroll
          for (int i = 0; i < 4; ++i) {
            const unsigned other = (unsigned)__builtin_amdgcn_update_dpp(0, (int)phi[i], 0x128, 0xf, 0xf, false);
            d1[i] = lowhalf ? plo[i] : other;
            d2[i] = lowhalf ? other : plo[i];
          }
          unsigned char* const base = rowp + (size_t)cx * p.ldy * 2;
          const int gx1 = tx0 + cx + (n & 7);
          const bool ok1 = st1 && (FULL || (yok && gx1 < p.W)), ok2 = st2 && (FULL || (yok && gx1 + 8 < p.W));
          if (ok1) __builtin_nontemporal_store(d1, reinterpret_cast<u32x4*>(base + off1));
          if (ok2) __builtin_nontemporal_store(d2, reinterpret_cast<u32x4*>(base + off2));
        }
      }
    };
    if (full) rows(std::true_type{});
    else rows(std::false_type{});
  }
  if (EPI == EPI_STATS) {
#pragma unroll
    for (int t = 0; t < 4; ++t)
#pragma unroll
      for (int r = 0; r < 4; ++r) {
        float a1 = s1[t][r >> 1][r & 1], a2 = s2[t][r >> 1][r & 1];
#pragma unroll
        for (int d = 1; d < 16; d <<= 1) {
          a1 += __shfl_xor(a1, d);
          a2 += __shfl_xor(a2, d);
        }
        if (n == 0) {
          red[wave][chan_of(t, q, r)] = a1;
          red[wave][64 + chan_of(t, q, r)] = a2;
        }
      }
    __syncthreads();
    if (tid < 128) {
      const int c = tid & 63, which = tid >> 6;
      const float tot = ((red[0][tid] + red[1][tid]) + red[2][tid]) + red[3][tid];
      if (co0 + c < p.CoutPad) p.slab[(size_t)blockIdx.x * 2 * p.CoutPad + which * p.CoutPad + co0 + c] = tot;
    }
  }
}

static int grid_x(int nTiles, int per_cu = FIRST_WAVES) {
  const int cap = device_shape().cus * per_cu;
  return nTiles < cap ? nTiles : cap;
}

template <bool F16>
static int launch(const P& p, hipStream_t st) {
  dim3 grid(grid_x(p.nTiles), p.CoutPad / 64);
  if (p.post_scale != nullptr) MAU_LAUNCH((first_fwd_kernel<F16, EPI_POST>), grid, dim3(NT), 0, st, p);
  else if (p.slab != nullptr) MAU_LAUNCH((first_fwd_kernel<F16, EPI_STATS>), grid, dim3(NT), 0, st, p);
  else MAU_LAUNCH((first_fwd_kernel<F16, EPI_PLAIN>), grid, dim3(NT), 0, st, p);
  return check_launch("first_fwd_kernel");
}
}
}

extern "C" {

int mau_conv3x3_first_max_channels(void) { return 8; }

int mau_conv3x3_first_rows(int N, int H, int W) {
  if (N <= 0 || H <= 0 || W <= 0) return 0;
  return mau::first::grid_x(N * mau::ceil_div(H, mau::first::TH) * mau::ceil_div(W, mau::first::TW));
}

int mau_conv3x3_first_fwd(const float* x, int Cin, const float* w, const float* bias, const float* post_scale, const float* post_shift, void* y,
                          int ldy, int Cout, float* slab, void* x8, int dtype, int N, int H, int W, mau_stream_t stream) {
  using namespace mau;
  MAU_REQUIRE(x && w && y && N > 0 && H > 0 && W > 0 && Cout > 0, "conv3x3_first_fwd: bad arguments");
  MAU_REQUIRE(Cin >= 1 && Cin <= 8, "conv3x3_first_fwd: %d input channels (this kernel serves <= 8; use mau_conv3x3_fwd)", Cin);
  MAU_REQUIRE(dtype == MAU_BF16 || dtype == MAU_F16, "conv3x3_first_fwd: 16-bit activation types only (fp32 = parity mode: mau_conv3x3_fwd)");
  MAU_REQUIRE(ldy % 8 == 0 && ldy >= Cout, "conv3x3_first_fwd: ldy must be a multiple of 8 and >= Cout");
  MAU_REQUIRE((post_scale == nullptr) == (post_shift == nullptr), "conv3x3_first_fwd: post_scale and post_shift come together");
  MAU_REQUIRE(!(post_scale != nullptr && slab != nullptr), "conv3x3_first_fwd: post_scale/post_shift and the statistics slab are mutually exclusive");
  MAU_REQUIRE((long long)N * H * W * ldy * 2 < (1ll << 40), "conv3x3_first_fwd: tensor too large");
  first::P p;
  p.x = x;
  p.Cin = Cin;
  p.w = w;
  p.bias = bias;
  p.post_scale = post_scale;
  p.post_shift = post_shift;
  p.y = y;
  p.ldy = ldy;
  p.Cout = Cout;
  p.CoutPad = round_up(Cout, 64);
  p.slab = slab;
  p.x8 = x8;
  p.N = N;
  p.H = H;
  p.W = W;
  p.tilesX = ceil_div(W, first::TW);
  p.tilesY = ceil_div(H, first::TH);
  p.nTiles = N * p.tilesX * p.tilesY;
  return dtype == MAU_F16 ? first::launch<true>(p, (hipStream_t)stream) : first::launch<false>(p, (hipStream_t)stream);
}

}

namespace mau {
namespace firstw {
using namespace igemm;
typedef float f32x4v __attribute__((ext_vector_type(4)));
typedef unsigned u32x2 __attribute__((ext_vector_type(2)));

constexpr int TWW = 32;
constexpr int DZ_BYTES = TWW * 128;
constexpr int XROW = 1024;
constexpr int BUF = DZ_BYTES + 3 * XROW;
constexpr int NT = 256, NWAVE = 4, NDMA = 7;
constexpr int NBT = 6, NCOL = 16 * NBT;

struct WP {
  const void* x8;
  const void* dz;
  int lddz, Cout;
  float* ws;
  int N, H, W, tilesX, nTiles;
};

template <bool F16>
__device__ __forceinline__ void mfma(const u32x4& a, const u32x4& b, f32x4v& c) {
  if constexpr (F16) asm volatile("v_mfma_f32_16x16x32_f16 %0, %1, %2, %0" : "+v"(c) : "v"(a), "v"(b));
  else asm volatile("v_mfma_f32_16x16x32_bf16 %0, %1, %2, %0" : "+v"(c) : "v"(a), "v"(b));
}
template <int OFF_HI>
__device__ __forceinline__ u32x4 tr_frag(unsigned addr_lo, unsigned addr_hi) {
  u32x2 lo, hi;
  asm volatile("ds_read_b64_tr_b16 %0, %2\n\tds_read_b64_tr_b16 %1, %3 offset:%4" : "=&v"(lo), "=&v"(hi) : "v"(addr_lo), "v"(addr_hi), "n"(OFF_HI));
  return __builtin_shufflevector(lo, hi, 0, 1, 2, 3);
}

template <bool F16>
__global__ __launch_bounds__(NT, 2) void first_wgrad_kernel(WP p) {
  extern __shared__ __attribute__((aligned(16))) unsigned char smem[];
  const int tid = threadIdx.x, lane = tid & 63;
  const int wave = __builtin_amdgcn_readfirstlane(tid >> 6);
  const int co0 = blockIdx.y * 64;
  const unsigned lds0 = (unsigned)(size_t)((__attribute__((address_space(3))) unsigned char*)smem) + wave * (2 * BUF);
  const unsigned long long dz_a = (unsigned long long)p.dz, x_a = (unsigned long long)p.x8, zero_a = (unsigned long long)g_zero_page;

  const int dz_px = lane >> 3, dz_ch = lane & 7;
  const bool dz_ch_ok = co0 + 8 * dz_ch < p.lddz;
  auto issue = [&](int tile, int buf) {
    const int txi = tile % p.tilesX, rowi = tile / p.tilesX;
    const int x0 = txi * TWW, y = rowi % p.H;
    unsigned char* dst = smem + wave * (2 * BUF) + buf * BUF;
#pragma unroll
    for (int d = 0; d < 4; ++d) {
      const int gx = x0 + 8 * d + dz_px;
      unsigned long long src = dz_a + 2ull * ((unsigned long long)((long long)rowi * p.W + gx) * (unsigned)p.lddz + (unsigned)(co0 + 8 * dz_ch));
      asm volatile("" : "+v"(src));
      src = (gx < p.W && dz_ch_ok) ? src : zero_a;
      __builtin_amdgcn_global_load_lds((glb_ptr)src, (lds_ptr)(dst + d * 1024), 16, 0, 0);
    }
#pragma unroll
    for (int dy = 0; dy < 3; ++dy) {
      const int gy = y + dy - 1, gx = x0 + lane - 1;
      const bool in = lane < TWW + 2 && gy >= 0 && gy < p.H && gx >= 0 && gx < p.W;
      unsigned long long src = x_a + 16ull * (unsigned long long)((long long)(rowi + dy - 1) * p.W + gx);
      asm volatile("" : "+v"(src));
      src = in ? src : zero_a;
      __builtin_amdgcn_global_load_lds((glb_ptr)src, (lds_ptr)(dst + DZ_BYTES + dy * XROW), 16, 0, 0);
    }
  };
  const int g = lane >> 4, q = (lane >> 2) & 3, pq = lane & 3;
  const unsigned a_lane = (unsigned)((8 * g + q) * 128 + 8 * pq);
  unsigned b_lane[NBT];
#pragma unroll
  for (int j = 0; j < NBT; ++j) b_lane[j] = (unsigned)(DZ_BYTES + (j >> 1) * XROW + (8 * g + q + 2 * (j & 1)) * 16 + 8 * pq);
  f32x4v acc[4][NBT];
#pragma unroll
  for (int t = 0; t < 4; ++t)
#pragma unroll
    for (int j = 0; j < NBT; ++j) acc[t][j] = f32x4v{0.f, 0.f, 0.f, 0.f};

  const int nw = gridDim.x * NWAVE, w0 = blockIdx.x * NWAVE + wave;
  int buf = 0;
  if (w0 < p.nTiles) issue(w0, 0);
  for (int tile = w0; tile < p.nTiles; tile += nw) {
    const bool more = tile + nw < p.nTiles;
    if (more) {
      issue(tile + nw, buf ^ 1);
      wait_vmcnt<NDMA>();
    } else {
      wait_vmcnt<0>();
    }
    const unsigned base = lds0 + buf * BUF;
    u32x4 A[4], B[NBT];
#pragma unroll
    for (int t = 0; t < 4; ++t) A[t] = tr_frag<4 * 128>(base + a_lane + 32 * t, base + a_lane + 32 * t);
#pragma unroll
    for (int j = 0; j < NBT; ++j) B[j] = tr_frag<4 * 16>(base + b_lane[j], base + b_lane[j]);
    asm volatile("s_waitcnt lgkmcnt(0)" ::: "memory");
#pragma unroll
    for (int t = 0; t < 4; ++t)
#pragma unroll
      for (int j = 0; j < NBT; ++j) mfma<F16>(A[t], B[j], acc[t][j]);
    buf ^= 1;
  }
  wait_vmcnt<0>();
  __syncthreads();
  float* red = reinterpret_cast<float*>(smem);
  const int dn = lane & 15, dq = lane >> 4;
  for (int wv = 0; wv < NWAVE; ++wv) {
    if (wave == wv) {
#pragma unroll
      for (int t = 0; t < 4; ++t)
#pragma unroll
        for (int j = 0; j < NBT; ++j)
#pragma unroll
          for (int r = 0; r < 4; ++r) {
            float* e = red + (16 * t + 4 * dq + r) * NCOL + 16 * j + dn;
            *e = wv == 0 ? acc[t][j][r] : *e + acc[t][j][r];
          }
    }
    __syncthreads();
  }
  float* out = p.ws + ((size_t)blockIdx.x * gridDim.y + blockIdx.y) * 64 * NCOL;
  for (int i = tid; i < 64 * NCOL; i += NT) out[i] = red[i];
}

constexpr int SUM_SL = 8, SUM_EL = 32;
__global__ __launch_bounds__(SUM_SL * SUM_EL) void first_wgrad_sum_kernel(const float* __restrict__ ws, int nwg, int coTiles, float* __restrict__ dw, int Cout, int Cin) {
  __shared__ float part[SUM_SL][SUM_EL];
  const int el = threadIdx.x % SUM_EL, sl = threadIdx.x / SUM_EL;
  const int i = blockIdx.x * SUM_EL + el, total = Cout * Cin * 9;
  const int ic = i < total ? i : 0;
  const int tap = ic % 9, ci = (ic / 9) % Cin, co = ic / (9 * Cin);
  const int dy = tap / 3, dx = tap - 3 * dy;
  const int col = 16 * (2 * dy + (dx == 2)) + 8 * (dx == 1) + ci;
  const float* src = ws + (size_t)co * NCOL + col;
  const size_t stride = (size_t)coTiles * 64 * NCOL;
  float s = 0.f;
  int wgi = sl;
  for (; wgi + 7 * SUM_SL < nwg; wgi += 8 * SUM_SL) {
    float v[8];
#pragma unroll
    for (int u = 0; u < 8; ++u) v[u] = src[(size_t)(wgi + u * SUM_SL) * stride];
#pragma unroll
    for (int u = 0; u < 8; ++u) s += v[u];
  }
  for (; wgi < nwg; wgi += SUM_SL) s += src[(size_t)wgi * stride];
  part[sl][el] = s;
  __syncthreads();
  if (sl == 0 && i < total) {
    float o = part[0][el];
#pragma unroll
    for (int k = 1; k < SUM_SL; ++k) o += part[k][el];
    dw[i] = o;
  }
}

static int grid_x(int nTiles) {
  const int cap = device_shape().cus * 2;
  const int need = ceil_div(nTiles, NWAVE);
  return need < cap ? need : cap;
}
}
}

extern "C" {

size_t mau_conv3x3_first_wgrad_ws_elems(int N, int H, int W, int Cout) {
  if (N <= 0 || H <= 0 || W <= 0 || Cout <= 0) return 0;
  return (size_t)mau::firstw::grid_x(N * H * mau::ceil_div(W, mau::firstw::TWW)) * mau::round_up(Cout, 64) * mau::firstw::NCOL;
}

int mau_conv3x3_first_wgrad(const void* x8, const void* dz, int lddz, float* dw, float* ws, int Cin, int Cout, int dtype, int N, int H, int W,
                            mau_stream_t stream) {
  using namespace mau;
  MAU_REQUIRE(x8 && dz && dw && ws && N > 0 && H > 0 && W > 0 && Cout > 0, "conv3x3_first_wgrad: bad arguments");
  MAU_REQUIRE(Cin >= 1 && Cin <= 8, "conv3x3_first_wgrad: %d input channels (this kernel serves <= 8; use mau_conv3x3_wgrad2)", Cin);
  MAU_REQUIRE(dtype == MAU_BF16 || dtype == MAU_F16, "conv3x3_first_wgrad: 16-bit activation types only");
  MAU_REQUIRE(lddz % 8 == 0 && lddz >= Cout && ((uintptr_t)x8 % 16) == 0 && ((uintptr_t)dz % 16) == 0, "conv3x3_first_wgrad: bad lddz / alignment");
  firstw::WP p;
  p.x8 = x8;
  p.dz = dz;
  p.lddz = lddz;
  p.Cout = Cout;
  p.ws = ws;
  p.N = N;
  p.H = H;
  p.W = W;
  p.tilesX = ceil_div(W, firstw::TWW);
  p.nTiles = N * H * p.tilesX;
  const int coTiles = round_up(Cout, 64) / 64;
  const dim3 grid(firstw::grid_x(p.nTiles), coTiles);
  constexpr size_t lds = (size_t)firstw::NWAVE * 2 * firstw::BUF;
  static_assert(lds >= 64 * firstw::NCOL * sizeof(float), "the cross-wave sum fits the DMA buffers");
  hipStream_t st = (hipStream_t)stream;
  if (dtype == MAU_F16) {
    MAU_LDS_ATTR(lds, &firstw::first_wgrad_kernel<true>);
    MAU_LAUNCH(firstw::first_wgrad_kernel<true>, grid, dim3(firstw::NT), lds, st, p);
  } else {
    MAU_LDS_ATTR(lds, &firstw::first_wgrad_kernel<false>);
    MAU_LAUNCH(firstw::first_wgrad_kernel<false>, grid, dim3(firstw::NT), lds, st, p);
  }
  const int rc = check_launch("first_wgrad_kernel");
  if (rc != MAU_OK) return rc;
  MAU_LAUNCH(firstw::first_wgrad_sum_kernel, dim3(ceil_div(Cout * Cin * 9, firstw::SUM_EL)), dim3(firstw::SUM_SL * firstw::SUM_EL), 0, st, ws, (int)grid.x,
             coTiles, dw, Cout, Cin);
  return check_launch("first_wgrad_sum_kernel");
}

}
```

### metadata-augmented-unet-for-lst-ndvi_amd/csrc/mau_common.h

```cpp
#pragma once
#include <hip/hip_runtime.h>
#include <stdint.h>
#include <stdio.h>
#include "../../include/mau_hip.h"

typedef __bf16 bf16;
typedef _Float16 f16;
typedef __attribute__((ext_vector_type(8))) __bf16 bf16x8;
typedef __attribute__((ext_vector_type(8))) _Float16 f16x8;
typedef __attribute__((ext_vector_type(4))) __bf16 bf16x4;
typedef __attribute__((ext_vector_type(4))) short s16x4;
typedef __attribute__((ext_vector_type(4))) float f32x4;
typedef __attribute__((ext_vector_type(16))) float f32x16;

namespace mau {

void set_error(const char* fmt, ...);
int check_launch(const char* what);

#define MAU_LAUNCH(...)               \
  do {                                \
    (void)hipGetLastError();          \
    hipLaunchKernelGGL(__VA_ARGS__);  \
  } while (0)

#define MAU_REQUIRE(cond, ...)                      \
  do {                                              \
    if (!(cond)) {                                  \
      ::mau::set_error(__VA_ARGS__);                \
      return MAU_ERR_ARG;                           \
    }                                               \
  } while (0)

static inline int ceil_div(int64_t a, int64_t b) { return (int)((a + b - 1) / b); }
static inline int round_up(int a, int b) { return (a + b - 1) / b * b; }

struct F8 {
  float v[8];
};

__device__ __forceinline__ float opaque(float v) {
  asm("" : "+v"(v));
  return v;
}

template <typename T>
__device__ __forceinline__ F8 load8(const T* p);
template <>
__device__ __forceinline__ F8 load8<float>(const float* p) {
  F8 r;
  f32x4 a = *reinterpret_cast<const f32x4*>(p);
  f32x4 b = *reinterpret_cast<const f32x4*>(p + 4);
#pragma unroll
  for (int i = 0; i < 4; ++i) {
    r.v[i] = a[i];
    r.v[4 + i] = b[i];
  }
  return r;
}
template <>
__device__ __forceinline__ F8 load8<bf16>(const bf16* p) {
  F8 r;
  bf16x8 a = *reinterpret_cast<const bf16x8*>(p);
#pragma unroll
  for (int i = 0; i < 8; ++i) r.v[i] = (float)a[i];
  return r;
}
template <>
__device__ __forceinline__ F8 load8<f16>(const f16* p) {
  F8 r;
  f16x8 a = *reinterpret_cast<const f16x8*>(p);
#pragma unroll
  for (int i = 0; i < 8; ++i) r.v[i] = opaque((float)a[i]);
  return r;
}
template <typename T>
__device__ __forceinline__ void store8(T* p, const F8& r);
template <>
__device__ __forceinline__ void store8<float>(float* p, const F8& r) {
  f32x4 a, b;
#pragma unroll
  for (int i = 0; i < 4; ++i) {
    a[i] = r.v[i];
    b[i] = r.v[4 + i];
  }
  *reinterpret_cast<f32x4*>(p) = a;
  *reinterpret_cast<f32x4*>(p + 4) = b;
}
template <>
__device__ __forceinline__ void store8<bf16>(bf16* p, const F8& r) {
  bf16x8 a;
#pragma unroll
  for (int i = 0; i < 8; ++i) a[i] = (bf16)r.v[i];
  *reinterpret_cast<bf16x8*>(p) = a;
}

template <>
__device__ __forceinline__ void store8<f16>(f16* p, const F8& r) {
  f16x8 a;
#pragma unroll
  for (int i = 0; i < 8; ++i) a[i] = (f16)opaque(r.v[i]);
  *reinterpret_cast<f16x8*>(p) = a;
}

template <typename T>
__device__ __forceinline__ F8 load8_nt(const T* p);
template <>
__device__ __forceinline__ F8 load8_nt<float>(const float* p) {
  F8 r;
  const f32x4 a = __builtin_nontemporal_load(reinterpret_cast<const f32x4*>(p));
  const f32x4 b = __builtin_nontemporal_load(reinterpret_cast<const f32x4*>(p + 4));
#pragma unroll
  for (int i = 0; i < 4; ++i) {
    r.v[i] = a[i];
    r.v[4 + i] = b[i];
  }
  return r;
}
template <>
__device__ __forceinline__ F8 load8_nt<bf16>(const bf16* p) {
  F8 r;
  const bf16x8 a = __builtin_nontemporal_load(reinterpret_cast<const bf16x8*>(p));
#pragma unroll
  for (int i = 0; i < 8; ++i) r.v[i] = (float)a[i];
  return r;
}
template <>
__device__ __forceinline__ F8 load8_nt<f16>(const f16* p) {
  F8 r;
  const f16x8 a = __builtin_nontemporal_load(reinterpret_cast<const f16x8*>(p));
#pragma unroll
  for (int i = 0; i < 8; ++i) r.v[i] = opaque((float)a[i]);
  return r;
}
template <typename T>
__device__ __forceinline__ void store8_nt(T* p, const F8& r);
template <>
__device__ __forceinline__ void store8_nt<float>(float* p, const F8& r) {
  f32x4 a, b;
#pragma unroll
  for (int i = 0; i < 4; ++i) {
    a[i] = r.v[i];
    b[i] = r.v[4 + i];
  }
  __builtin_nontemporal_store(a, reinterpret_cast<f32x4*>(p));
  __builtin_nontemporal_store(b, reinterpret_cast<f32x4*>(p + 4));
}
template <>
__device__ __forceinline__ void store8_nt<bf16>(bf16* p, const F8& r) {
  bf16x8 a;
#pragma unroll
  for (int i = 0; i < 8; ++i) a[i] = (bf16)r.v[i];
  __builtin_nontemporal_store(a, reinterpret_cast<bf16x8*>(p));
}

template <>
__device__ __forceinline__ void store8_nt<f16>(f16* p, const F8& r) {
  f16x8 a;
#pragma unroll
  for (int i = 0; i < 8; ++i) a[i] = (f16)opaque(r.v[i]);
  __builtin_nontemporal_store(a, reinterpret_cast<f16x8*>(p));
}

__device__ __forceinline__ float coef(const float* __restrict__ p, int c, int C) {
  const float v = p[c < C ? c : C - 1];
  return c < C ? v : 0.f;
}
__device__ __forceinline__ double coef(const double* __restrict__ p, int c, int C) {
  const double v = p[c < C ? c : C - 1];
  return c < C ? v : 0.0;
}

__device__ __forceinline__ F8 zero8() {
  F8 r;
#pragma unroll
  for (int i = 0; i < 8; ++i) r.v[i] = 0.f;
  return r;
}

template <typename T>
__device__ __forceinline__ float to_f(T x) {
  return (float)x;
}

constexpr int BWD_PIX_PER_BLOCK = 1024;
constexpr int HEAD_MAX_CO = 4;
constexpr int HEAD_PIX_PER_BLOCK = BWD_PIX_PER_BLOCK;

struct DeviceShape {
  int cus, xcds, xcd_shift;
};
static inline DeviceShape device_shape() {
  static DeviceShape cache[64];
  static bool have[64];
  int dev = 0;
  if (hipGetDevice(&dev) != hipSuccess || dev < 0 || dev >= 64) return DeviceShape{256, 8, 3};
  if (!have[dev]) {
    int cus = 0;
    if (hipDeviceGetAttribute(&cus, hipDeviceAttributeMultiprocessorCount, dev) != hipSuccess || cus <= 0) cus = 256;
    int x = 1, s = 0;
    while (x < 8 && x * 2 * 32 <= cus) {
      x *= 2;
      ++s;
    }
    cache[dev] = DeviceShape{cus, x, s};
    have[dev] = true;
  }
  return cache[dev];
}
static inline int launch_cus() { return device_shape().cus; }
#define MAU_LDS_ATTR(bytes, ...)                                                                                        \
  do {                                                                                                                  \
    static bool done_[64];                                                                                              \
    int d_ = 0;                                                                                                         \
    if (hipGetDevice(&d_) == hipSuccess && d_ >= 0 && d_ < 64 && !done_[d_]) {                                          \
      (void)hipFuncSetAttribute(reinterpret_cast<const void*>(__VA_ARGS__), hipFuncAttributeMaxDynamicSharedMemorySize, \
                                (int)(bytes));                                                                          \
      done_[d_] = true;                                                                                                 \
    }                                                                                                                   \
  } while (0)

static inline int stream_grid(int64_t work_items, int block) {
  int64_t g = (work_items + block - 1) / block;
  const int64_t cap = (int64_t)device_shape().cus * 8;
  if (g > cap) g = cap;
  if (g < 1) g = 1;
  return (int)g;
}

__device__ __forceinline__ bool last_block_of(unsigned* ticket, unsigned n) {
  __shared__ unsigned s_last;
  asm volatile("s_waitcnt vmcnt(0)" ::: "memory");
  __syncthreads();
  if (threadIdx.x == 0) {
    __builtin_amdgcn_fence(__ATOMIC_RELEASE, "agent");
    asm volatile("s_waitcnt vmcnt(0)" ::: "memory");
    const unsigned t = __hip_atomic_fetch_add(ticket, 1u, __ATOMIC_RELAXED, __HIP_MEMORY_SCOPE_AGENT);
    const unsigned last = t == n - 1 ? 1u : 0u;
    if (last) {
      __builtin_amdgcn_fence(__ATOMIC_ACQUIRE, "agent");
      asm volatile("s_waitcnt vmcnt(0)" ::: "memory");
      __hip_atomic_store(ticket, 0u, __ATOMIC_RELAXED, __HIP_MEMORY_SCOPE_AGENT);
    }
    s_last = last;
  }
  __syncthreads();
  return s_last != 0;
}

int head_fwd_fast(const void* a, int lda, const float* w, const float* b, float* out, int tanh0, int dtype, int64_t npix, int HW, int C, int Co,
                  hipStream_t stream);

}

#define MAU_DISPATCH_DTYPE(dtype, ...)              \
  do {                                              \
    if ((dtype) == MAU_F32) {                       \
      using T = float;                              \
      __VA_ARGS__;                                  \
    } else if ((dtype) == MAU_BF16) {               \
      using T = bf16;                               \
      __VA_ARGS__;                                  \
    } else if ((dtype) == MAU_F16) {                \
      using T = f16;                                \
      __VA_ARGS__;                                  \
    } else {                                        \
      ::mau::set_error("bad dtype %d", (int)dtype); \
      return MAU_ERR_ARG;                           \
    }                                               \
  } while (0)
```

### metadata-augmented-unet-for-lst-ndvi_amd/functional.py

```python
from __future__ import annotations

import contextlib
import dataclasses
import os
from collections import namedtuple
from dataclasses import dataclass
from typing import List, Optional

import torch

from . import _lib
from ._lib import MAU_BF16, MAU_F16, MAU_F32, call, lib

BN_EPS = 1e-5
BN_MOMENTUM = 0.1


def pad8(c: int) -> int:
    return (c + 7) // 8 * 8


def dtype_code(dt: torch.dtype) -> int:
    if dt == torch.float32:
        return MAU_F32
# ... 124 lines not shown
        t = _TICKETS[key] = torch.zeros(lib.mau_reduce_tickets_elems(), dtype=torch.int32, device=dev)
    return t


class PackGroup:

    def __init__(self):
        self.params: List[torch.Tensor] = []
        self._state = {}
        self.fresh_after_step = -1

    def add(self, w: torch.Tensor):
        if not any(w is q for q in self.params):
            self.params.append(w)
            self._state = {}
        w._mau_group = self

    def _build(self, code: int, ptrs):
        import ctypes
        dev = self.params[0].device
        dt = _DT[code]
        wf = [torch.empty(lib.mau_conv3x3_packed_elems(code, w.shape[0], w.shape[1]), dtype=dt, device=dev) for w in self.params]
        wd = [torch.empty(lib.mau_conv3x3_packed_elems(code, w.shape[1], w.shape[0]), dtype=dt, device=dev) for w in self.params]
        nbytes = lib.mau_conv3x3_pack_desc_bytes()
        host = ctypes.create_string_buffer(nbytes * len(self.params))
        nxt = ctypes.c_int(0)
        for i, w in enumerate(self.params):
            call("mau_conv3x3_pack_desc_fill", ctypes.addressof(host), i, w.data_ptr(), wf[i].data_ptr(), wd[i].data_ptr(), code,
                 w.shape[0], w.shape[1], nxt.value, ctypes.addressof(nxt))
        table = torch.frombuffer(bytearray(host.raw), dtype=torch.uint8).to(dev)
        return {"ptrs": ptrs, "wf": wf, "wd": wd, "table": table, "tiles": nxt.value, "key": None}

    def ensure(self, code: int):
        ptrs = tuple(w.data_ptr() for w in self.params)
        st = self._state.get(code)
        if st is None or st["ptrs"] != ptrs:
            st = self._state[code] = self._build(code, ptrs)
        key = (_GENERATION[0], tuple(w._version for w in self.params))
        if st["key"] != key:
            if not (self.fresh_after_step == _GENERATION[0] and st["key"] is not None and st["key"][1] == key[1] and len(self._state) == 1):
                call("mau_conv3x3_pack_weights_multi", st["table"].data_ptr(), len(self.params), st["tiles"], code, _stream())
            st["key"] = key
            for w, f, d in zip(self.params, st["wf"], st["wd"]):
                w._mau_pack = [(key[0], w._version, w.data_ptr(), code), f, d]
        return st


def pack_conv_weights(w: torch.Tensor, code: int, forward: bool = True, dgrad: bool = False):
    cout, cin = w.shape[0], w.shape[1]
    key = (_GENERATION[0], w._version, w.data_ptr(), code)
    cache = getattr(w, "_mau_pack", None)
    if cache is not None and cache[0] == key and (cache[1] is not None or not forward) and (cache[2] is not None or not dgrad):
        return (cache[1] if forward else None), (cache[2] if dgrad else None)
    group = getattr(w, "_mau_group", None)
    if group is not None and _PACK_MULTI:
        group.ensure(code)
        cache = w._mau_pack
        return (cache[1] if forward else None), (cache[2] if dgrad else None)
    dt = _DT[code]
    if cache is None:
        cache = [None, None, None]
        try:
            w._mau_pack = cache
        except (AttributeError, RuntimeError):
            pass

    def buf(old, n):
        if old is not None and old.dtype == dt and old.device == w.device and old.numel() == n:
            return old
        return torch.empty(n, dtype=dt, device=w.device)

    stale = cache[0] != key
    need_f = forward and (stale or cache[1] is None or cache[1].dtype != dt)
    need_d = dgrad and (stale or cache[2] is None or cache[2].dtype != dt)
    wf = buf(cache[1], lib.mau_conv3x3_packed_elems(code, cout, cin)) if need_f else None
    wd = buf(cache[2], lib.mau_conv3x3_packed_elems(code, cin, cout)) if need_d else None
    if need_f or need_d:
        call("mau_conv3x3_pack_weights", w.detach().data_ptr(), wf.data_ptr() if need_f else None, wd.data_ptr() if need_d else None,
             code, cout, cin, _stream())
    if stale:
        cache[1] = wf
        cache[2] = wd
    else:
        if need_f:
            cache[1] = wf
        if need_d:
            cache[2] = wd
    cache[0] = key
    return (cache[1] if forward else None), (cache[2] if dgrad else None)


class ToNHWC(torch.autograd.Function):

    @staticmethod
    def forward(ctx, x: torch.Tensor, dt: torch.dtype):
        _require_cuda(x, "UrbanPredictor.forward(maps)")
        x = x.contiguous().float()
        N, Cc, H, W = x.shape
        ld = pad8(Cc)
        out = torch.empty((N, H, W, ld), dtype=dt, device=x.device)
        call("mau_nchw_to_nhwc", x.data_ptr(), out.data_ptr(), dtype_code(dt), N, Cc, H, W, ld, _stream())
        ctx.C = Cc
        return out

    @staticmethod
    def backward(ctx, g):
        return to_nchw(Act(g, ctx.C)), None


def to_nchw(a: Act) -> torch.Tensor:
    t = _as_nhwc(a.t.detach())
    N, H, W, _ = t.shape
    out = torch.empty((N, a.C, H, W), dtype=torch.float32, device=t.device)
    call("mau_nhwc_to_nchw", t.data_ptr(), out.data_ptr(), dtype_code(t.dtype), N, a.C, H, W, _ld(t), _stream())
    return out


@dataclass
class BNState:
    training: bool
    C0: int
    momentum: float = BN_MOMENTUM
    eps: float = BN_EPS
    group: object = None
    comm: object = None
    world: int = 1
    grad_enabled: bool = True
    frozen: object = None
    C1: int = 0
    pool: bool = False
    out_view: object = None
    head: object = None
    up_to: object = None
    first: bool = False
    dtype: object = None
    dgrad_first: bool = False


def _all_reduce_(t: torch.Tensor, st: BNState):
    if st.comm is not None:
        st.comm.all_reduce(t, 0, _stream())
    elif st.group is not None:
        from .dist import all_reduce_sum
        all_reduce_sum(t, st.group)


_OVERLAP_WGRAD = int(os.environ.get("MAU_OVERLAP_WGRAD", "2") or 0)
_FUSED_REDUCE = True
_FUSED_BN = True
_FUSED_UP = True
_PACK_MULTI = True
_INFER_POOL_FUSED = True
_FIRST_WGRAD = True
_SIDE_STREAMS = {}


def _side_stream(dev) -> "torch.cuda.Stream":
    s = _SIDE_STREAMS.get(dev)
    if s is None:
        s = _SIDE_STREAMS[dev] = torch.cuda.Stream(device=dev)
    return s


def _join_side_when_backward_ends(dev):
    def join():
        torch.cuda.current_stream(dev).wait_stream(_side_stream(dev))

    torch.autograd.Variable._execution_engine.queue_callback(join)


_DGRAD_FIRST = None


_Geom = namedtuple("_Geom", "N H W Cin Cout ldy code act_dt dev stream")
_Saved = namedtuple("_Saved", "x x1 emb weight y scale shift mean invstd a w2 out argidx")


def _ptr(t):
    return None if t is None else t.data_ptr()


def _pool_fwd(x, C, stream):
    N, H, W, _ = x.shape
    ldy = pad8(C)
    y = torch.empty((N, H // 2, W // 2, ldy), dtype=x.dtype, device=x.device)
    call("mau_maxpool2x2_fwd", x.data_ptr(), _ld(x), y.data_ptr(), ldy, dtype_code(x.dtype), N, H, W, C, stream)
    return y


def _pool_bwd(x, C, dy, dskip, stream):
    dy = _as_nhwc(dy)
    N, H, W, _ = x.shape
    dx = torch.empty((N, H, W, pad8(C)), dtype=x.dtype, device=x.device)
    tail = (dx.data_ptr(), pad8(C), dtype_code(x.dtype), N, H, W, C, stream)
    if dskip is None:
        call("mau_maxpool2x2_bwd", x.data_ptr(), _ld(x), dy.data_ptr(), _ld(dy), *tail)
    else:
        dskip = _as_nhwc(dskip)
        call("mau_maxpool2x2_bwd_add", x.data_ptr(), _ld(x), dy.data_ptr(), _ld(dy), dskip.data_ptr(), _ld(dskip), *tail)
    return dx


def _resize_fwd(src, C, size, stream, dst=None, choff=0):
    N, h, w, _ = src.shape
    H, W = size
    if dst is None:
        dst = torch.empty((N, H, W, pad8(C)), dtype=src.dtype, device=src.device)
    call("mau_resize_bilinear_fwd", src.data_ptr(), _ld(src), h, w, dst.data_ptr(), _ld(dst), choff, dtype_code(src.dtype), N, H, W, C, stream)
    return dst


def _resize_bwd(g, goff, C, size, stream):
    N, H, W, _ = g.shape
    h, w = size
    d = torch.empty((N, h, w, pad8(C)), dtype=g.dtype, device=g.device)
    call("mau_resize_bilinear_bwd", g.data_ptr(), _ld(g), goff, H, W, d.data_ptr(), pad8(C), dtype_code(g.dtype), N, h, w, C, stream)
    return d


def _head_fwd(a, C, w2, hb, tanh0, stream):
    N, H, W, _ = a.shape
    Co = w2.shape[0]
    out = torch.empty((N, Co, H, W), dtype=torch.float32, device=a.device)
    call("mau_head_fwd", a.data_ptr(), _ld(a), w2.data_ptr(), hb.data_ptr(), out.data_ptr(), tanh0, dtype_code(a.dtype), N, H * W, C, Co, stream)
    return out


def _head_slab(N, HW, C, Co, dev):
    return torch.empty((lib.mau_head_bwd_rows(N, HW), lib.mau_head_bwd_rowlen(C, Co)), dtype=torch.float32, device=dev)


def _head_param_grads(hslab, C, Co, wshape, stream):
    hrows, rowlen = hslab.shape
    red = torch.empty(rowlen, dtype=torch.float32, device=hslab.device)
    ws = torch.empty(lib.mau_reduce_rows_ws_elems(hrows, rowlen), dtype=torch.float64, device=hslab.device)
    call("mau_reduce_rows_f32", hslab.data_ptr(), hrows, rowlen, rowlen, red.data_ptr(), ws.data_ptr(),
         _tickets(hslab.device).data_ptr() if _FUSED_REDUCE else None, stream)
    red = red.view(Co, pad8(C) + 8)
    return red[:, :C].reshape(wshape).contiguous(), red[:, pad8(C)].contiguous()


def _head_bwd(a, C, w2, out, dout, tanh0, wshape, stream):
    N, H, W, _ = a.shape
    Co = w2.shape[0]
    dout = dout.contiguous().float()
    da = torch.empty((N, H, W, pad8(C)), dtype=a.dtype, device=a.device)
    hslab = _head_slab(N, H * W, C, Co, a.device)
    call("mau_head_bwd", a.data_ptr(), _ld(a), w2.data_ptr(), out.data_ptr(), dout.data_ptr(), da.data_ptr(), pad8(C), hslab.data_ptr(), tanh0,
         dtype_code(a.dtype), N, H * W, C, Co, stream)
    return (da, *_head_param_grads(hslab, C, Co, wshape, stream))


def _conv_launch(g: _Geom, st: BNState, src, w, bias, post, y, slab=None, x8=None):
    x, x1, emb, emb_ws = src
    scale, shift = post if post is not None else (None, None)
    if st.first:
        call("mau_conv3x3_first_fwd", x.data_ptr(), st.C0, w.data_ptr(), _ptr(bias), _ptr(scale), _ptr(shift), y.data_ptr(), _ld(y),
             g.Cout, _ptr(slab), _ptr(x8), g.code, g.N, g.H, g.W, g.stream)
        return
    E = 0 if emb is None else emb.shape[1]
    call("mau_conv3x3_fwd2", x.data_ptr(), _ld(x), st.C0, _ptr(x1), _ld(x1) if x1 is not None else 0, st.C1 if x1 is not None else 0,
         emb.data_ptr() if E else None, emb_ws.data_ptr() if E else None, E, w.data_ptr(), _ptr(bias), _ptr(scale), _ptr(shift),
         y.data_ptr(), _ld(y), g.Cout, _ptr(slab), g.code, g.N, g.H, g.W, g.stream)


def _conv_inputs(x, x1, emb, weight, hw, st: BNState):
    _require_cuda(x, "conv3x3")
    if st.first:
        if x1 is not None or emb is not None or x.dim() != 4 or x.shape[1] != st.C0 or st.C0 > lib.mau_conv3x3_first_max_channels():
            raise RuntimeError("conv3x3 (first layer): expects one (N, C <= 8, H, W) fp32 input")
        x = x.contiguous().float()
        N, _, H, W = x.shape
        act_dt = st.dtype
    else:
        x = _as_nhwc(x)
        if x1 is not None:
            x1 = _as_nhwc(x1)
        N, H, W, _ = x.shape
        act_dt = x.dtype
    Cout, Cin = weight.shape[0], weight.shape[1]
    g = _Geom(N, H, W, Cin, Cout, pad8(Cout), dtype_code(act_dt), act_dt, x.device, _stream())
    E = 0 if emb is None else emb.shape[1]
    C1 = st.C1 if x1 is not None else 0
    if st.C0 + C1 + E != Cin:
        raise RuntimeError(f"conv3x3: input has {st.C0}+{C1}+{E} channels, weight expects {Cin}")
    if emb is not None:
        emb = emb.contiguous().float()
    dst = st.out_view
    if dst is not None and (tuple(dst.shape) != (N, H, W, g.ldy) or dst.dtype != act_dt or Cout % 64 != 0):
        raise RuntimeError("conv3x3: out_view must be an (N,H,W,Cout) NHWC-ld view of the activation dtype with Cout % 64 == 0")
    if sum((st.pool, st.head is not None, st.up_to is not None)) > 1 or ((st.head is not None or st.up_to is not None) and dst is not None):
        raise RuntimeError("conv3x3: pool / head / up_to are exclusive, and head / up_to write no activation (no out_view)")
    head = None
    if st.head is not None:
        Co = hw.shape[0]
        head = (Co, 1 if (Co == 2 and st.head) else 0, hw.detach().reshape(Co, Cout).contiguous().float())
    emb_ws = torch.empty((N, E), dtype=act_dt, device=g.dev) if E else None
    return g, (x, x1, emb, emb_ws), head


def _conv_inference(g: _Geom, st: BNState, src, weight, bias, bn, head, hb):
    gamma, beta, rmean, rvar = bn[:4]
    x, x1, emb, _ = src
    y = st.out_view if st.out_view is not None else torch.empty((g.N, g.H, g.W, g.ldy), dtype=g.act_dt, device=g.dev)
    fz = st.frozen if st.frozen is not None else {}
    fkey = (_GENERATION[0], weight._version, gamma._version, rmean._version, rvar._version)
    if "wf" not in fz or fz["wf"].dtype != g.act_dt or fz.get("key") != fkey:
        fz["key"] = fkey
        fz["wf"] = weight if st.first else pack_conv_weights(weight, g.code, forward=True, dgrad=False)[0]
        if "scale" not in fz or fz["scale"].device != g.dev or fz["scale"].numel() != g.Cout:
            fz["scale"], fz["shift"] = (torch.empty(g.Cout, dtype=torch.float32, device=g.dev) for _ in range(2))
        call("mau_bn_coeffs_eval", gamma.data_ptr(), beta.data_ptr(), rmean.data_ptr(), rvar.data_ptr(), st.eps, fz["scale"].data_ptr(),
             fz["shift"].data_ptr(), None, None, g.Cout, g.stream)
    pl = None
    if st.pool and not st.first and _INFER_POOL_FUSED and x1 is None and (emb is None or not emb.shape[1]) and g.H >= 2 and g.W >= 2:
        pl = torch.empty((g.N, g.H // 2, g.W // 2, g.ldy), dtype=g.act_dt, device=g.dev)
        call("mau_conv3x3_fwd_pool", x.data_ptr(), _ld(x), st.C0, fz["wf"].data_ptr(), _ptr(bias), fz["scale"].data_ptr(),
             fz["shift"].data_ptr(), y.data_ptr(), _ld(y), g.Cout, pl.data_ptr(), g.ldy, g.code, g.N, g.H, g.W, g.stream)
    else:
        _conv_launch(g, st, src, fz["wf"], bias, (fz["scale"], fz["shift"]), y)
    if head is not None:
        return (_head_fwd(y, g.Cout, head[2], hb, head[1], g.stream),)
    if st.up_to is not None:
        return (_resize_fwd(y, g.Cout, st.up_to, g.stream),)
    if st.pool:
        return y, (pl if pl is not None else _pool_fwd(y, g.Cout, g.stream))
    return (y,)


def _conv_with_stats(g: _Geom, st: BNState, src, w, bias, bn, x8):
    gamma, beta, rmean, rvar, nbt = bn
    Cout, dev, stream = g.Cout, g.dev, g.stream
    y = torch.empty((g.N, g.H, g.W, g.ldy), dtype=g.act_dt, device=dev)
    coef = tuple(torch.empty(Cout, dtype=torch.float32, device=dev) for _ in range(4))
    cptrs = tuple(t.data_ptr() for t in coef)
    if not st.training:
        call("mau_bn_coeffs_eval", gamma.data_ptr(), beta.data_ptr(), rmean.data_ptr(), rvar.data_ptr(), st.eps, *cptrs, Cout, stream)
        _conv_launch(g, st, src, w, bias, None, y, None, x8)
        return y, coef
    npix = g.N * g.H * g.W
    tiles = lib.mau_conv3x3_first_rows(g.N, g.H, g.W) if st.first else lib.mau_conv3x3_num_pixel_tiles(g.code, g.N, g.H, g.W, Cout)
    slab = torch.empty((tiles, 2 * ((Cout + 63) // 64 * 64)), dtype=torch.float32, device=dev)
    _conv_launch(g, st, src, w, bias, None, y, slab, x8)
    if st.group is None:
        ws = torch.empty(lib.mau_bn_stats_ws_elems(tiles, Cout), dtype=torch.float64, device=dev)
        call("mau_bn_stats_finalize_train", slab.data_ptr(), tiles, float(npix), gamma.data_ptr(), beta.data_ptr(),
             rmean.data_ptr(), rvar.data_ptr(), _ptr(nbt), st.momentum, st.eps, *cptrs, ws.data_ptr(),
             _tickets(dev).data_ptr() if _FUSED_REDUCE else None, Cout, stream)
    else:
        sums = torch.empty(2 * Cout + 1, dtype=torch.float64, device=dev)
        ws = torch.empty(lib.mau_reduce_rows_ws_elems(tiles, 2 * Cout), dtype=torch.float64, device=dev)
        call("mau_bn_stats_sums_f64", slab.data_ptr(), tiles, Cout, sums.data_ptr(), ws.data_ptr(), _tickets(dev).data_ptr(), float(npix), stream)
        _all_reduce_(sums, st)
        call("mau_bn_finalize_train", sums.data_ptr(), 0.0, gamma.data_ptr(), beta.data_ptr(), rmean.data_ptr(), rvar.data_ptr(), _ptr(nbt),
             st.momentum, st.eps, *cptrs, Cout, stream)
    return y, coef


def _conv_activation(g: _Geom, st: BNState, y, scale, shift, head, hb):
    N, H, W, Cout, ldy, stream = g.N, g.H, g.W, g.Cout, g.ldy, g.stream
    fused = _FUSED_BN
    if head is not None and fused and Cout <= lib.mau_head_bn_max_channels() and H * W >= 32:
        Co, tanh0, w2 = head
        out = torch.empty((N, Co, H, W), dtype=torch.float32, device=g.dev)
        call("mau_head_bn_fwd", y.data_ptr(), ldy, scale.data_ptr(), shift.data_ptr(), w2.data_ptr(), hb.data_ptr(), out.data_ptr(), tanh0,
             g.code, N, H * W, Cout, Co, stream)
        return (out,), (None, out, None), True
    if st.up_to is not None and fused and _FUSED_UP and H <= st.up_to[0] and W <= st.up_to[1]:
        Hu, Wu = st.up_to
        up = torch.empty((N, Hu, Wu, ldy), dtype=g.act_dt, device=g.dev)
        call("mau_resize_bilinear_bn_fwd", y.data_ptr(), ldy, H, W, scale.data_ptr(), shift.data_ptr(), up.data_ptr(), ldy, 0, g.code,
             N, Hu, Wu, Cout, stream)
        return (up,), (None, None, None), True
    a = st.out_view if st.out_view is not None else torch.empty_like(y)
    if st.pool and H >= 2 and W >= 2:
        pl = torch.empty((N, H // 2, W // 2, ldy), dtype=g.act_dt, device=g.dev)
        argidx = torch.empty((N, H // 2, W // 2, ldy // 8), dtype=torch.int16, device=g.dev) if fused else None
        call("mau_bn_relu_apply_pool", y.data_ptr(), ldy, scale.data_ptr(), shift.data_ptr(), a.data_ptr(), _ld(a),
             pl.data_ptr(), ldy, _ptr(argidx), g.code, N, H, W, Cout, stream)
        return (a, pl), (None if fused else a, None, argidx), False
    call("mau_bn_relu_apply", y.data_ptr(), ldy, scale.data_ptr(), shift.data_ptr(), a.data_ptr(), _ld(a), g.code, N * H * W, Cout, stream)
    if head is not None:
        out = _head_fwd(a, Cout, head[2], hb, head[1], stream)
        return (out,), (a, out, None), False
    if st.up_to is not None:
        return (_resize_fwd(a, Cout, st.up_to, stream),), (None, None, None), False
    return ((a, None) if st.pool else (a,)), (None, None, None), False


def _conv_save(ctx, st: BNState, src, weight, wd, y, coef, head, hw, outs, kept, fused):
    ctx.st = st if st.out_view is None else dataclasses.replace(st, out_view=None)
    x, x1, emb, _ = src
    ctx.wd = wd
    ctx.pooled = len(outs) == 2 and outs[1] is not None
    ctx.head = (head[0], head[1], tuple(hw.shape), fused) if head is not None else None
    ctx.up = (st.up_to, fused) if st.up_to is not None else None
    a, out, argidx = kept
    ctx.save_for_backward(*_Saved(x, x1, emb, weight, y, *coef, a, head[2] if head is not None else None, out, argidx))


def _dz_begin(g: _Geom, sv):
    slab = torch.empty((lib.mau_bn_bwd_rows(g.N * g.H * g.W), 2 * g.Cout), dtype=torch.float32, device=g.dev)
    return slab, torch.empty_like(sv.y), (sv.scale.data_ptr(), sv.shift.data_ptr(), sv.mean.data_ptr(), sv.invstd.data_ptr())


def _finish_sums(g: _Geom, st: BNState, slab):
    rows, C2 = slab.shape
    npix = g.N * g.H * g.W
    sync = st.training and st.group is not None
    sums = torch.empty(C2 + 1, dtype=torch.float64, device=g.dev)
    g32 = torch.empty(C2, dtype=torch.float32, device=g.dev)
    ws = torch.empty(lib.mau_reduce_rows_ws_elems(rows, C2), dtype=torch.float64, device=g.dev)
    call("mau_reduce_rows_f64_f32", slab.data_ptr(), rows, C2, C2, sums.data_ptr(), g32.data_ptr(), ws.data_ptr(),
         _tickets(g.dev).data_ptr() if (_FUSED_REDUCE or sync) else None, float(npix) if sync else 0.0, g.stream)
    if not st.training:
        return torch.zeros_like(sums), float(npix), g32
    if sync:
        _all_reduce_(sums, st)
        return sums, 0.0, g32
    return sums, float(npix), g32


def _dz_fused_head(g: _Geom, st: BNState, ctx, sv, da, dpl):
    Co, tanh0, hshape, _ = ctx.head
    slab, dy, cptrs = _dz_begin(g, sv)
    dout = da.contiguous().float()
    hslab = _head_slab(g.N, g.H * g.W, g.Cout, Co, g.dev)
    call("mau_head_bn_bwd_reduce", sv.y.data_ptr(), g.ldy, *cptrs, sv.w2.data_ptr(), sv.out.data_ptr(), dout.data_ptr(), slab.data_ptr(),
         g.Cout, hslab.data_ptr(), tanh0, g.code, g.N, g.H * g.W, g.Cout, Co, g.stream)
    sums, count, g32 = _finish_sums(g, st, slab)
    dhw, dhb = _head_param_grads(hslab, g.Cout, Co, hshape, g.stream)
    call("mau_head_bn_bwd_apply", sv.y.data_ptr(), g.ldy, *cptrs, sums.data_ptr(), count, sv.w2.data_ptr(), sv.out.data_ptr(),
         dout.data_ptr(), dy.data_ptr(), g.ldy, tanh0, g.code, g.N, g.H * g.W, g.Cout, Co, g.stream)
    return dy, g32, dhw, dhb


def _dz_fused_pool(g: _Geom, st: BNState, ctx, sv, da, dpl):
    slab, dy, cptrs = _dz_begin(g, sv)
    dpl = _as_nhwc(dpl)
    dsk = _as_nhwc(da) if da is not None else None
    pargs = (sv.y.data_ptr(), g.ldy, dpl.data_ptr(), _ld(dpl), sv.argidx.data_ptr(), _ptr(dsk), _ld(dsk) if dsk is not None else 0)
    call("mau_pool_bn_bwd_reduce", *pargs, *cptrs, slab.data_ptr(), g.Cout, g.code, g.N, g.H, g.W, g.Cout, g.stream)
    sums, count, g32 = _finish_sums(g, st, slab)
    call("mau_pool_bn_bwd_apply", *pargs, *cptrs, sums.data_ptr(), count, dy.data_ptr(), g.ldy, g.code, g.N, g.H, g.W, g.Cout, g.stream)
    return dy, g32, None, None


def _dz_generic(g: _Geom, st: BNState, ctx, sv, da, dpl):
    y, ldy, npix, stream = sv.y, g.ldy, g.N * g.H * g.W, g.stream
    slab, dy, cptrs = _dz_begin(g, sv)
    dhw = dhb = None
    if ctx.head is not None:
        _, tanh0, hshape, _ = ctx.head
        da, dhw, dhb = _head_bwd(sv.a, g.Cout, sv.w2, sv.out, da, tanh0, hshape, stream)
    elif ctx.up is not None:
        da = _resize_bwd(_as_nhwc(da), 0, g.Cout, (g.H, g.W), stream)
    elif ctx.pooled and dpl is not None:
        act = sv.a
        if act is None:
            act = torch.empty_like(y)
            call("mau_bn_relu_apply", y.data_ptr(), ldy, sv.scale.data_ptr(), sv.shift.data_ptr(), act.data_ptr(), ldy, g.code, npix, g.Cout, stream)
        da = _pool_bwd(act, g.Cout, dpl, da, stream)
    elif da is None:
        da = torch.zeros((g.N, g.H, g.W, ldy), dtype=y.dtype, device=g.dev)
    da = _as_nhwc(da)
    call("mau_bn_relu_bwd_reduce", da.data_ptr(), _ld(da), y.data_ptr(), ldy, *cptrs, slab.data_ptr(), g.Cout, g.code, npix, g.Cout, stream)
    sums, count, g32 = _finish_sums(g, st, slab)
    call("mau_bn_relu_bwd_apply", da.data_ptr(), _ld(da), y.data_ptr(), ldy, *cptrs, sums.data_ptr(), count, dy.data_ptr(), ldy, g.code, npix, g.Cout, stream)
    return dy, g32, dhw, dhb


def _dgrad_launch(g: _Geom, dy, wd, weight):
    if wd is None:
        wd = pack_conv_weights(weight, g.code, forward=False, dgrad=True)[1]
    ldd = pad8(g.Cin)
    dfull = torch.empty((g.N, g.H, g.W, ldd), dtype=g.act_dt, device=g.dev)
    call("mau_conv3x3_fwd", dy.data_ptr(), g.ldy, g.Cout, None, None, 0, wd.data_ptr(), None, None, None, dfull.data_ptr(), ldd, g.Cin, None,
         g.code, g.N, g.H, g.W, g.stream)
    return dfull


def _conv_wgrad(g: _Geom, st: BNState, sv, E, C1, dy, side, overlap, waits_for_dy):
    x, x1, emb, weight = sv.x, sv.x1, sv.emb, sv.weight
    if side is not None and not waits_for_dy:
        side.wait_stream(torch.cuda.current_stream())
    with torch.cuda.stream(side) if side is not None else contextlib.nullcontext():
        acc = torch.empty(max(lib.mau_conv3x3_wgrad_acc_elems(g.code, g.N, g.H, g.W, g.Cout, g.Cin),
                              lib.mau_conv3x3_first_wgrad_ws_elems(g.N, g.H, g.W, g.Cout) if st.first else 0), dtype=torch.float32, device=g.dev)
        emb_ws = torch.empty((g.N, E), dtype=g.act_dt, device=g.dev) if E else None
    slot = getattr(weight, "_mau_grad_slot", None)
    dw = slot.view_as(weight) if (slot is not None and weight.is_leaf and weight.grad is None and slot.device == g.dev) else torch.empty_like(weight)
    wstream = side.cuda_stream if side is not None else g.stream
    deferred = side is not None and overlap >= 2 and weight.is_leaf and weight.grad is None
    if st.first and _FIRST_WGRAD:
        call("mau_conv3x3_first_wgrad", x.data_ptr(), dy.data_ptr(), g.ldy, dw.data_ptr(), acc.data_ptr(), g.Cin, g.Cout, g.code, g.N, g.H, g.W, wstream)
    else:
        call("mau_conv3x3_wgrad2", x.data_ptr(), _ld(x), st.C0, _ptr(x1), _ld(x1) if x1 is not None else 0, C1,
             emb.data_ptr() if E else None, emb_ws.data_ptr() if E else None, E, dy.data_ptr(), g.ldy, g.Cout, acc.data_ptr(),
             g.code, g.N, g.H, g.W, wstream)
        call("mau_conv3x3_unpack_wgrad", acc.data_ptr(), lib.mau_conv3x3_wgrad_splits(g.code, g.N, g.H, g.W, g.Cout, g.Cin),
             dw.data_ptr(), g.Cout, g.Cin, wstream)
    if deferred:
        for t in (x, x1, emb, dy, dw):
            if t is not None:
                t.record_stream(side)
        weight._mau_grad_stream = side
        _join_side_when_backward_ends(g.dev)
    return dw, deferred


def _conv_dgrad(g: _Geom, st: BNState, E, C1, dfull, needs):
    dx = dx1 = demb = None
    if E and needs[2]:
        demb = torch.empty((g.N, E), dtype=torch.float32, device=g.dev)
        ws = torch.empty(lib.mau_bcast_bwd_ws_elems(g.N, g.H * g.W, E), dtype=torch.float32, device=g.dev)
        call("mau_bcast_bwd", dfull.data_ptr(), pad8(g.Cin), st.C0 + C1, demb.data_ptr(), ws.data_ptr(), g.code, g.N, g.H * g.W, E, g.stream)
    if C1:
        if needs[0]:
            dx = dfull[..., :st.C0]
        if needs[1]:
            dx1 = dfull[..., st.C0:st.C0 + pad8(C1)]
    elif needs[0]:
        dx = dfull[..., :pad8(st.C0)] if E else dfull
    return dx, dx1, demb


class ConvBNReLU(torch.autograd.Function):

    @staticmethod
    def forward(ctx, x, x1, emb, weight, bias, gamma, beta, rmean, rvar, nbt, hw, hb, st: BNState):
        g, src, head = _conv_inputs(x, x1, emb, weight, hw, st)
        needs = ctx.needs_input_grad
        bn = (gamma, beta, rmean, rvar, nbt)
        if (not st.training) and (not st.grad_enabled or not any(needs)):
            outs = _conv_inference(g, st, src, weight, bias, bn, head, hb)
            ctx.mark_non_differentiable(*outs)
            return outs if st.pool else outs[0]
        need_dx = needs[0] or (src[1] is not None and needs[1]) or (src[3] is not None and needs[2])
        if st.first:
            if need_dx:
                raise RuntimeError("conv3x3 (first layer): no gradient w.r.t. the network input on this path")
            w, wd = weight, None
            x8 = torch.empty((g.N, g.H, g.W, 8), dtype=g.act_dt, device=g.dev) if (st.grad_enabled and needs[3]) else None
            saved_src = (x8, None, None, None)
        else:
            w, wd = pack_conv_weights(weight, g.code, forward=True, dgrad=st.grad_enabled and need_dx)
            x8, saved_src = None, src
        y, coef = _conv_with_stats(g, st, src, w, bias, bn, x8)
        outs, kept, fused = _conv_activation(g, st, y, coef[0], coef[1], head, hb)
        _conv_save(ctx, st, saved_src, weight, wd, y, coef, head, hw, outs, kept, fused)
        return outs if st.pool else outs[0]

    @staticmethod
    def backward(ctx, da, dpl=None):
        sv = _Saved(*ctx.saved_tensors)
        st: BNState = ctx.st
        E, C1 = (0 if sv.emb is None else sv.emb.shape[1]), (st.C1 if sv.x1 is not None else 0)
        y, weight = sv.y, sv.weight
        N, H, W, ldy = y.shape
        Cout = weight.shape[0]
        g = _Geom(N, H, W, weight.shape[1], Cout, ldy, dtype_code(y.dtype), y.dtype, y.device, _stream())
        needs = ctx.needs_input_grad
        dz = (_dz_fused_head if (ctx.head is not None and ctx.head[3])
              else _dz_fused_pool if (ctx.pooled and dpl is not None and sv.argidx is not None) else _dz_generic)
        dy, g32, dhw, dhb = dz(g, st, ctx, sv, da, dpl)
        dgamma, dbeta = g32[Cout:], g32[:Cout]
        need_dx = needs[0] or (sv.x1 is not None and needs[1]) or (E and needs[2])
        overlap = _OVERLAP_WGRAD
        side = _side_stream(g.dev) if (needs[3] and overlap and (need_dx or overlap >= 2)) else None
        dfull = None
        if (st.dgrad_first if _DGRAD_FIRST is None else _DGRAD_FIRST == "1") and need_dx and needs[3] and side is not None:
            dy_ready = torch.cuda.Event()
            dy_ready.record()
            dfull = _dgrad_launch(g, dy, ctx.wd, weight)
            side.wait_event(dy_ready)
        dw, deferred = _conv_wgrad(g, st, sv, E, C1, dy, side, overlap, dfull is not None) if needs[3] else (None, False)
        dx = dx1 = demb = None
        if need_dx:
            dx, dx1, demb = _conv_dgrad(g, st, E, C1, dfull if dfull is not None else _dgrad_launch(g, dy, ctx.wd, weight), needs)
        if side is not None and not deferred:
            torch.cuda.current_stream().wait_stream(side)
        dbias = None
        if needs[4]:
            dbias = _zero_bias_grad(Cout, g.dev) if st.training else sv.scale * dbeta
        return dx, dx1, demb, dw, dbias, dgamma, dbeta, None, None, None, dhw, dhb, None


class MaxPool2x2(torch.autograd.Function):

    @staticmethod
    def forward(ctx, x, C):
        x = _as_nhwc(x)
        ctx.save_for_backward(x)
        ctx.C = C
        return _pool_fwd(x, C, _stream())

    @staticmethod
    def backward(ctx, dy):
        (x,) = ctx.saved_tensors
        return _pool_bwd(x, ctx.C, dy, None, _stream()), None


class PoolSkip(torch.autograd.Function):

    @staticmethod
    def forward(ctx, x, C):
        x = _as_nhwc(x)
        ctx.save_for_backward(x)
        ctx.C = C
        return _pool_fwd(x, C, _stream()), x.view_as(x)

    @staticmethod
    def backward(ctx, dy, dskip):
        (x,) = ctx.saved_tensors
        if dy is None:
            return dskip, None
        return _pool_bwd(x, ctx.C, dy, dskip, _stream()), None


def _resize_into(src, Cs, dst, choff, code, stream):
    N, H, W, _ = dst.shape
    if choff % 8 == 0:
        _resize_fwd(src, Cs, (H, W), stream, dst, choff)
    else:
        tmp = _resize_fwd(src, Cs, (H, W), stream)
        call("mau_copy_channels", tmp.data_ptr(), pad8(Cs), dst.data_ptr(), _ld(dst), choff, 0, code, N * H * W, Cs, stream)


class RowPrefix(torch.autograd.Function):

    @staticmethod
    def forward(ctx, C, *xs):
        base = xs[0]
        ld, esz = base.stride(2), base.element_size()
        for j, t in enumerate(xs):
            if t.data_ptr() != base.data_ptr() + j * C * esz or t.stride() != base.stride() or t.shape != base.shape:
                raise RuntimeError("RowPrefix: inputs are not adjacent channel slots of one row buffer")
        N, H, W, _ = base.shape
        ctx.C, ctx.k = C, len(xs)
        return base.as_strided((N, H, W, C * len(xs)), base.stride())

    @staticmethod
    def backward(ctx, g):
        g = _as_nhwc(g)
        return (None, *[g[..., j * ctx.C:(j + 1) * ctx.C] for j in range(ctx.k)])


class Fanout(torch.autograd.Function):

    @staticmethod
    def forward(ctx, x, k: int):
        ctx.k = k
        ctx.meta = (x.shape, x.dtype, x.device)
        return tuple(x.as_strided(x.shape, x.stride()) for _ in range(k))

    @staticmethod
    def backward(ctx, *gs):
        import ctypes
        shape, dtype, dev = ctx.meta
        live = [_as_nhwc(g) for g in gs if g is not None]
        if not live:
            return None, None
        if len(live) == 1:
            return live[0], None
        N, H, W, C = shape
        ld = pad8(C)
        kmax = lib.mau_sum_tensors_max()
        out = torch.empty((N, H, W, ld), dtype=dtype, device=dev)
        while True:
            part = live[:kmax]
            ptrs = (ctypes.c_void_p * len(part))(*[g.data_ptr() for g in part])
            lds = (ctypes.c_int * len(part))(*[_ld(g) for g in part])
            call("mau_sum_tensors", ctypes.addressof(ptrs), ctypes.addressof(lds), len(part), out.data_ptr(), ld, dtype_code(dtype),
                 N * H * W, C, _stream())
            live = [out] + live[kmax:]
            if len(live) == 1:
                break
            out = torch.empty((N, H, W, ld), dtype=dtype, device=dev)
        res = live[0]
        return (res if ld == C else res[..., :C]), None


class EmbFold(torch.autograd.Function):

    @staticmethod
    def forward(ctx, weight, emb, Ct: int, Ep: int):
        _require_cuda(weight, "EmbFold")
        w = weight.detach().contiguous().float()
        e = emb.detach().contiguous().float()
        Cout, Cf = w.shape[0], w.shape[1]
        N, E = e.shape
        if Cf != Ct + E or Ep < N:
            raise RuntimeError(f"EmbFold: weight has {Cf} input channels, expected {Ct}+{E}; Ep={Ep} must cover the batch of {N}")
        weff = torch.empty((Cout, Ct + Ep, 3, 3), dtype=torch.float32, device=w.device)
        call("mau_emb_fold_fwd", w.data_ptr(), e.data_ptr(), weff.data_ptr(), Cout, Ct, E, N, Ep, _stream())
        ctx.save_for_backward(weight, emb)
        ctx.dims = (Cout, Ct, E, N, Ep)
        return weff

    @staticmethod
    def backward(ctx, dweff):
        weight, emb = ctx.saved_tensors
        Cout, Ct, E, N, Ep = ctx.dims
        dweff = dweff.contiguous().float()
        w = weight.detach().contiguous().float()
        e = emb.detach().contiguous().float()
        dw = demb = None
        if ctx.needs_input_grad[0]:
            slot = getattr(weight, "_mau_grad_slot", None)
            dw = slot.view_as(weight) if (slot is not None and weight.is_leaf and weight.grad is None and slot.device == w.device) else torch.empty_like(w)
        ws = None
        if ctx.needs_input_grad[1]:
            demb = torch.empty((N, E), dtype=torch.float32, device=w.device)
            ws = torch.empty(lib.mau_emb_fold_ws_elems(Cout, N, E), dtype=torch.float32, device=w.device)
        call("mau_emb_fold_bwd", w.data_ptr(), e.data_ptr(), dweff.data_ptr(), dw.data_ptr() if dw is not None else None,
             demb.data_ptr() if demb is not None else None, ws.data_ptr() if ws is not None else None, Cout, Ct, E, N, Ep, _stream())
        return dw, demb, None, None

# ... 303 lines not shown
```

Measured before the change: 2603 images/s.

## Fuse BN-ReLU backward apply into the first-layer weight-gradient kernel

For the first conv layer, the BN/ReLU backward apply that materialised dy is skipped. The first-layer wgrad kernel now loads da and the pre-activation y directly into registers, computes dy per tile, and writes it into LDS before the MFMA. This removes one full-resolution elementwise pass and the write and read of the dy tensor at 256x256x64. In exchange the wgrad pipeline uses register loads with hand-written waitcnt sequencing, which adds latency and complexity, and dy is recomputed for each Cout tile.

```diff
diff --git a/include/mau_hip.h b/include/mau_hip.h
--- a/include/mau_hip.h
+++ b/include/mau_hip.h
@@ -54,6 +54,9 @@
 size_t mau_conv3x3_first_wgrad_ws_elems(int N, int H, int W, int Cout);
 int mau_conv3x3_first_wgrad(const void* x8, const void* dz, int lddz, float* dw_oihw, float* ws, int Cin, int Cout, int dtype, int N,
                             int H, int W, mau_stream_t stream);
+int mau_conv3x3_first_wgrad_bn(const void* x8, const void* da, int ldda, const void* z, int ldz, const float* scale, const float* shift,
+                               const float* mean, const float* invstd, const double* sums, double count, float* dw_oihw, float* ws,
+                               int Cin, int Cout, int dtype, int N, int H, int W, mau_stream_t stream);
 int mau_conv3x3_first_fwd(const float* x_nchw, int Cin, const float* w_oihw, const float* bias, const float* post_scale,
                           const float* post_shift, void* y, int ldy, int Cout, float* slab, void* x8, int dtype, int N, int H,
                           int W, mau_stream_t stream);
diff --git a/metadata-augmented-unet-for-lst-ndvi_amd/_lib.py b/metadata-augmented-unet-for-lst-ndvi_amd/_lib.py
--- a/metadata-augmented-unet-for-lst-ndvi_amd/_lib.py
+++ b/metadata-augmented-unet-for-lst-ndvi_amd/_lib.py
@@ -35,6 +35,7 @@
     "mau_conv3x3_first_rows": (_i, [_i, _i, _i]),
     "mau_conv3x3_first_wgrad_ws_elems": (_sz, [_i, _i, _i, _i]),
     "mau_conv3x3_first_wgrad": (_i, [_p, _p, _i, _p, _p, _i, _i, _i, _i, _i, _i, _p]),
+    "mau_conv3x3_first_wgrad_bn": (_i, [_p, _p, _i, _p, _i, _p, _p, _p, _p, _p, _d, _p, _p, _i, _i, _i, _i, _i, _i, _p]),
     "mau_conv3x3_first_fwd": (_i, [_p, _i, _p, _p, _p, _p, _p, _i, _i, _p, _p, _i, _i, _i, _i, _p]),
     "mau_conv3x3_fwd": (_i, [_p, _i, _i, _p, _p, _i, _p, _p, _p, _p, _p, _i, _i, _p, _i, _i, _i, _i, _p]),
     "mau_conv3x3_fwd_pool": (_i, [_p, _i, _i, _p, _p, _p, _p, _p, _i, _i, _p, _i, _i, _i, _i, _i, _p]),
diff --git a/metadata-augmented-unet-for-lst-ndvi_amd/csrc/bn.hip b/metadata-augmented-unet-for-lst-ndvi_amd/csrc/bn.hip
--- a/metadata-augmented-unet-for-lst-ndvi_amd/csrc/bn.hip
+++ b/metadata-augmented-unet-for-lst-ndvi_amd/csrc/bn.hip
@@ -1,4 +1,5 @@
 #include <stdlib.h>
+#include "bn_bwd_apply.h"
 #include "mau_common.h"
 
 namespace mau {
@@ -437,29 +438,13 @@
   const int nv = C8 >> 3;
   const PixVec m(nv);
   if (m.ps >= m.PS) return;
-  if (inv_count <= 0.0) inv_count = 1.0 / sums[2 * C];
+  inv_count = bn_bwd_inv_count(sums, inv_count, C);
   const int64_t p0 = (int64_t)blockIdx.x * pixb;
   const int64_t p1 = p0 + pixb < npix ? p0 + pixb : npix;
   for (int vv = m.v; vv < nv; vv += m.nvl) {
     const int c = vv * 8;
-    float sc[8], sh[8], k0[8], k1[8];
-    double d1[8], d2[8];
-#pragma unroll
-    for (int j = 0; j < 8; ++j) {
-      sc[j] = coef(scale, c + j, C);
-      sh[j] = coef(shift, c + j, C);
-      k0[j] = coef(mean, c + j, C);
-      k1[j] = coef(invstd, c + j, C);
-      d1[j] = coef(sums, c + j, C);
-      d2[j] = coef(sums + C, c + j, C);
-    }
-#pragma unroll
-    for (int j = 0; j < 8; ++j) {
-      const float mu = k0[j], is = k1[j];
-      const float m1 = (float)(d1[j] * inv_count), m2 = (float)(d2[j] * inv_count);
-      k1[j] = __fmul_rn(__fmul_rn(sc[j], m2), is);
-      k0[j] = fmaf(sc[j], m1, -__fmul_rn(k1[j], mu));
-    }
+    Apply8 k;
+    k.load(scale, shift, mean, invstd, sums, inv_count, c, C);
     int64_t pix = p0 + m.ps;
     for (; pix + 3 * m.PS < p1; pix += 4 * m.PS) {
       F8 g[4], v[4];
@@ -472,11 +457,7 @@
       for (int u = 0; u < 4; ++u) {
         F8 o;
 #pragma unroll
-        for (int j = 0; j < 8; ++j) {
-          const float act = fmaf(v[u].v[j], sc[j], sh[j]);
-          const float dz = act > 0.f ? g[u].v[j] : 0.f;
-          o.v[j] = fmaf(sc[j], dz, -fmaf(k1[j], v[u].v[j], k0[j]));
-        }
+        for (int j = 0; j < 8; ++j) o.v[j] = k.dy(j, v[u].v[j], g[u].v[j]);
         if (NT) store8_nt<T>(dy + (pix + u * m.PS) * lddy + c, o); else store8<T>(dy + (pix + u * m.PS) * lddy + c, o);
       }
     }
@@ -485,11 +466,7 @@
       const F8 v = load8<T>(y + pix * ldy + c);
       F8 o;
 #pragma unroll
-      for (int j = 0; j < 8; ++j) {
-        const float act = fmaf(v.v[j], sc[j], sh[j]);
-        const float dz = act > 0.f ? g.v[j] : 0.f;
-        o.v[j] = fmaf(sc[j], dz, -fmaf(k1[j], v.v[j], k0[j]));
-      }
+      for (int j = 0; j < 8; ++j) o.v[j] = k.dy(j, v.v[j], g.v[j]);
       store8<T>(dy + pix * lddy + c, o);
     }
   }
diff --git a/metadata-augmented-unet-for-lst-ndvi_amd/csrc/bn_bwd_apply.h b/metadata-augmented-unet-for-lst-ndvi_amd/csrc/bn_bwd_apply.h
--- /dev/null
+++ b/metadata-augmented-unet-for-lst-ndvi_amd/csrc/bn_bwd_apply.h
@@ -0,0 +1,39 @@
+#pragma once
+#include "mau_common.h"
+
+namespace mau {
+
+__device__ __forceinline__ double bn_bwd_inv_count(const double* __restrict__ sums, double inv_count, int C) {
+  return inv_count <= 0.0 ? 1.0 / sums[2 * C] : inv_count;
+}
+
+struct Apply8 {
+  float sc[8], sh[8], k0[8], k1[8];
+  __device__ __forceinline__ void load(const float* scale, const float* shift, const float* mean, const float* invstd, const double* sums,
+                                       double inv_count, int c0, int C) {
+    double d1[8], d2[8];
+#pragma unroll
+    for (int j = 0; j < 8; ++j) {
+      sc[j] = coef(scale, c0 + j, C);
+      sh[j] = coef(shift, c0 + j, C);
+      k0[j] = coef(mean, c0 + j, C);
+      k1[j] = coef(invstd, c0 + j, C);
+      d1[j] = coef(sums, c0 + j, C);
+      d2[j] = coef(sums + C, c0 + j, C);
+    }
+#pragma unroll
+    for (int j = 0; j < 8; ++j) {
+      const float mu = k0[j], is = k1[j];
+      const float m1 = (float)(d1[j] * inv_count), m2 = (float)(d2[j] * inv_count);
+      k1[j] = __fmul_rn(__fmul_rn(sc[j], m2), is);
+      k0[j] = fmaf(sc[j], m1, -__fmul_rn(k1[j], mu));
+    }
+  }
+  __device__ __forceinline__ float dy(int j, float yv, float da) const {
+    const float act = fmaf(yv, sc[j], sh[j]);
+    const float dz = act > 0.f ? da : 0.f;
+    return fmaf(sc[j], dz, -fmaf(k1[j], yv, k0[j]));
+  }
+};
+
+}
diff --git a/metadata-augmented-unet-for-lst-ndvi_amd/csrc/bn_fused.hip b/metadata-augmented-unet-for-lst-ndvi_amd/csrc/bn_fused.hip
--- a/metadata-augmented-unet-for-lst-ndvi_amd/csrc/bn_fused.hip
+++ b/metadata-augmented-unet-for-lst-ndvi_amd/csrc/bn_fused.hip
@@ -1,3 +1,4 @@
+#include "bn_bwd_apply.h"
 #include "mau_common.h"
 
 namespace mau {
@@ -163,35 +164,6 @@
   bn_sums_to_slab(red, s1, s2, cv, ps, slab, ldslab);
 }
 
-struct Apply8 {
-  float sc[8], sh[8], k0[8], k1[8];
-  __device__ __forceinline__ void load(const float* scale, const float* shift, const float* mean, const float* invstd, const double* sums,
-                                       double inv_count, int c0, int C) {
-    double d1[8], d2[8];
-#pragma unroll
-    for (int j = 0; j < 8; ++j) {
-      sc[j] = coef(scale, c0 + j, C);
-      sh[j] = coef(shift, c0 + j, C);
-      k0[j] = coef(mean, c0 + j, C);
-      k1[j] = coef(invstd, c0 + j, C);
-      d1[j] = coef(sums, c0 + j, C);
-      d2[j] = coef(sums + C, c0 + j, C);
-    }
-#pragma unroll
-    for (int j = 0; j < 8; ++j) {
-      const float mu = k0[j], is = k1[j];
-      const float m1 = (float)(d1[j] * inv_count), m2 = (float)(d2[j] * inv_count);
-      k1[j] = __fmul_rn(__fmul_rn(sc[j], m2), is);
-      k0[j] = fmaf(sc[j], m1, -__fmul_rn(k1[j], mu));
-    }
-  }
-  __device__ __forceinline__ float dy(int j, float yv, float da) const {
-    const float act = fmaf(yv, sc[j], sh[j]);
-    const float dz = act > 0.f ? da : 0.f;
-    return fmaf(sc[j], dz, -fmaf(k1[j], yv, k0[j]));
-  }
-};
-
 template <typename T, bool POOL, bool SKIP>
 __global__ __launch_bounds__(256) void pool_bn_bwd_apply_kernel(const T* __restrict__ y, int ldy, const T* __restrict__ dpl, int lddpl,
                                                                 const unsigned short* __restrict__ argidx,
@@ -205,7 +177,7 @@
   if (idx >= Wc * nv) return;
   const int xo = idx / nv, c = (idx - xo * nv) * 8;
   const int n = blockIdx.z;
-  if (inv_count <= 0.0) inv_count = 1.0 / sums[2 * C];
+  inv_count = bn_bwd_inv_count(sums, inv_count, C);
   Apply8 k;
   k.load(scale, shift, mean, invstd, sums, inv_count, c, C);
   const int x0 = 2 * xo;
@@ -506,7 +478,7 @@
   const int cv = threadIdx.x & 7, ps = threadIdx.x >> 3;
   const int c0 = cv * 8;
   if (c0 >= ((C + 7) & ~7)) return;
-  if (inv_count <= 0.0) inv_count = 1.0 / sums[2 * C];
+  inv_count = bn_bwd_inv_count(sums, inv_count, C);
   Apply8 k;
   k.load(scale, shift, mean, invstd, sums, inv_count, c0, C);
   float wr[MC][8];
diff --git a/metadata-augmented-unet-for-lst-ndvi_amd/csrc/conv3x3_first.hip b/metadata-augmented-unet-for-lst-ndvi_amd/csrc/conv3x3_first.hip
--- a/metadata-augmented-unet-for-lst-ndvi_amd/csrc/conv3x3_first.hip
+++ b/metadata-augmented-unet-for-lst-ndvi_amd/csrc/conv3x3_first.hip
@@ -1,3 +1,4 @@
+#include "bn_bwd_apply.h"
 #include "igemm_bf16_util.h"
 
 namespace mau {
@@ -329,6 +330,14 @@
   float* ws;
   int N, H, W, tilesX, nTiles;
 };
+struct BNArgs {
+  const void* da;
+  const void* z;
+  int ldda, ldz;
+  const float *scale, *shift, *mean, *invstd;
+  const double* sums;
+  double inv_count;
+};
 
 template <bool F16>
 __device__ __forceinline__ void mfma(const u32x4& a, const u32x4& b, f32x4v& c) {
@@ -342,8 +351,31 @@
   return __builtin_shufflevector(lo, hi, 0, 1, 2, 3);
 }
 
+__device__ __forceinline__ void load4(u32x4 (&r)[4], const unsigned long long (&a)[4]) {
+#pragma unroll
+  for (int d = 0; d < 4; ++d) asm volatile("global_load_dwordx4 %0, %1, off" : "=&v"(r[d]) : "v"(a[d]) : "memory");
+}
+template <int N>
+__device__ __forceinline__ void load_land(u32x4 (&g)[4], u32x4 (&v)[4]) {
+  asm volatile("s_waitcnt vmcnt(%8)" : "+v"(g[0]), "+v"(g[1]), "+v"(g[2]), "+v"(g[3]), "+v"(v[0]), "+v"(v[1]), "+v"(v[2]), "+v"(v[3]) : "n"(N) : "memory");
+}
 template <bool F16>
-__global__ __launch_bounds__(NT, 2) void first_wgrad_kernel(WP p) {
+__device__ __forceinline__ F8 unpack8(const u32x4& r) {
+  F8 o;
+  if constexpr (F16) {
+    const f16x8 a = __builtin_bit_cast(f16x8, r);
+#pragma unroll
+    for (int i = 0; i < 8; ++i) o.v[i] = opaque((float)a[i]);
+  } else {
+    const bf16x8 a = __builtin_bit_cast(bf16x8, r);
+#pragma unroll
+    for (int i = 0; i < 8; ++i) o.v[i] = (float)a[i];
+  }
+  return o;
+}
+
+template <bool F16, bool BN>
+__global__ __launch_bounds__(NT, 2) void first_wgrad_kernel(WP p, BNArgs bn) {
   extern __shared__ __attribute__((aligned(16))) unsigned char smem[];
   const int tid = threadIdx.x, lane = tid & 63;
   const int wave = __builtin_amdgcn_readfirstlane(tid >> 6);
@@ -353,9 +385,9 @@
 
   const int dz_px = lane >> 3, dz_ch = lane & 7;
   const bool dz_ch_ok = co0 + 8 * dz_ch < p.lddz;
-  auto issue = [&](int tile, int buf) {
+  auto issue_dz = [&](int tile, int buf) {
     const int txi = tile % p.tilesX, rowi = tile / p.tilesX;
-    const int x0 = txi * TWW, y = rowi % p.H;
+    const int x0 = txi * TWW;
     unsigned char* dst = smem + wave * (2 * BUF) + buf * BUF;
 #pragma unroll
     for (int d = 0; d < 4; ++d) {
@@ -365,6 +397,11 @@
       src = (gx < p.W && dz_ch_ok) ? src : zero_a;
       __builtin_amdgcn_global_load_lds((glb_ptr)src, (lds_ptr)(dst + d * 1024), 16, 0, 0);
     }
+  };
+  auto issue_x = [&](int tile, int buf) {
+    const int txi = tile % p.tilesX, rowi = tile / p.tilesX;
+    const int x0 = txi * TWW, y = rowi % p.H;
+    unsigned char* dst = smem + wave * (2 * BUF) + buf * BUF;
 #pragma unroll
     for (int dy = 0; dy < 3; ++dy) {
       const int gy = y + dy - 1, gx = x0 + lane - 1;
@@ -375,6 +412,45 @@
       __builtin_amdgcn_global_load_lds((glb_ptr)src, (lds_ptr)(dst + DZ_BYTES + dy * XROW), 16, 0, 0);
     }
   };
+  Apply8 k;
+  u32x4 rg[4], rv[4];
+  const unsigned long long da_a = (unsigned long long)bn.da, z_a = (unsigned long long)bn.z;
+  if constexpr (BN) k.load(bn.scale, bn.shift, bn.mean, bn.invstd, bn.sums, bn_bwd_inv_count(bn.sums, bn.inv_count, p.Cout), co0 + 8 * dz_ch, p.Cout);
+  auto load_dz = [&](int tile) {
+    const int txi = tile % p.tilesX, rowi = tile / p.tilesX;
+    const int x0 = txi * TWW;
+    unsigned long long ga[4], va[4];
+#pragma unroll
+    for (int d = 0; d < 4; ++d) {
+      const int gx = x0 + 8 * d + dz_px;
+      const unsigned long long pix = (unsigned long long)((long long)rowi * p.W + gx);
+      ga[d] = da_a + 2ull * (pix * (unsigned)bn.ldda + (unsigned)(co0 + 8 * dz_ch));
+      va[d] = z_a + 2ull * (pix * (unsigned)bn.ldz + (unsigned)(co0 + 8 * dz_ch));
+      asm volatile("" : "+v"(ga[d]), "+v"(va[d]));
+      const bool in = gx < p.W && dz_ch_ok;
+      ga[d] = in ? ga[d] : zero_a;
+      va[d] = in ? va[d] : zero_a;
+    }
+    load4(rg, ga);
+    load4(rv, va);
+  };
+  auto commit_dz = [&](int tile, int buf) {
+    const int x0 = (tile % p.tilesX) * TWW;
+    u32x4 o[4];
+#pragma unroll
+    for (int d = 0; d < 4; ++d) {
+      const F8 g = unpack8<F16>(rg[d]), v = unpack8<F16>(rv[d]);
+      F8 r;
+#pragma unroll
+      for (int j = 0; j < 8; ++j) r.v[j] = k.dy(j, v.v[j], g.v[j]);
+      const u32x4 pk = __builtin_bit_cast(u32x4, Lp8<std::conditional_t<F16, f16, bf16>>::from(r));
+      const bool in = x0 + 8 * d + dz_px < p.W && dz_ch_ok;
+#pragma unroll
+      for (int i = 0; i < 4; ++i) o[d][i] = in ? pk[i] : 0u;
+    }
+    asm volatile("ds_write_b128 %0, %1\n\tds_write_b128 %0, %2 offset:1024\n\tds_write_b128 %0, %3 offset:2048\n\tds_write_b128 %0, %4 offset:3072\n\ts_nop 1"
+                 :: "v"(lds0 + buf * BUF + lane * 16), "v"(o[0]), "v"(o[1]), "v"(o[2]), "v"(o[3]) : "memory");
+  };
   const int g = lane >> 4, q = (lane >> 2) & 3, pq = lane & 3;
   const unsigned a_lane = (unsigned)((8 * g + q) * 128 + 8 * pq);
   unsigned b_lane[NBT];
@@ -388,11 +464,31 @@
 
   const int nw = gridDim.x * NWAVE, w0 = blockIdx.x * NWAVE + wave;
   int buf = 0;
-  if (w0 < p.nTiles) issue(w0, 0);
+  if (w0 < p.nTiles) {
+    if constexpr (BN) {
+      load_dz(w0);
+      issue_x(w0, 0);
+      load_land<3>(rg, rv);
+    } else {
+      issue_dz(w0, 0);
+      issue_x(w0, 0);
+    }
+  }
   for (int tile = w0; tile < p.nTiles; tile += nw) {
     const bool more = tile + nw < p.nTiles;
-    if (more) {
-      issue(tile + nw, buf ^ 1);
+    if constexpr (BN) {
+      commit_dz(tile, buf);
+      if (more) {
+        load_dz(tile + nw);
+        issue_x(tile + nw, buf ^ 1);
+        wait_vmcnt<8 + 3>();
+      } else {
+        wait_vmcnt<0>();
+      }
+      asm volatile("s_waitcnt lgkmcnt(0)" ::: "memory");
+    } else if (more) {
+      issue_dz(tile + nw, buf ^ 1);
+      issue_x(tile + nw, buf ^ 1);
       wait_vmcnt<NDMA>();
     } else {
       wait_vmcnt<0>();
@@ -408,6 +504,9 @@
     for (int t = 0; t < 4; ++t)
 #pragma unroll
       for (int j = 0; j < NBT; ++j) mfma<F16>(A[t], B[j], acc[t][j]);
+    if constexpr (BN) {
+      if (more) load_land<3>(rg, rv);
+    }
     buf ^= 1;
   }
   wait_vmcnt<0>();
@@ -468,6 +567,29 @@
   const int need = ceil_div(nTiles, NWAVE);
   return need < cap ? need : cap;
 }
+
+template <bool BN>
+static int launch(WP p, const BNArgs& bn, float* dw, int Cin, int dtype, mau_stream_t stream) {
+  p.tilesX = ceil_div(p.W, TWW);
+  p.nTiles = p.N * p.H * p.tilesX;
+  const int coTiles = round_up(p.Cout, 64) / 64;
+  const dim3 grid(grid_x(p.nTiles), coTiles);
+  constexpr size_t lds = (size_t)NWAVE * 2 * BUF;
+  static_assert(lds >= 64 * NCOL * sizeof(float), "the cross-wave sum fits the DMA buffers");
+  hipStream_t st = (hipStream_t)stream;
+  if (dtype == MAU_F16) {
+    MAU_LDS_ATTR(lds, &first_wgrad_kernel<true, BN>);
+    MAU_LAUNCH((first_wgrad_kernel<true, BN>), grid, dim3(NT), lds, st, p, bn);
+  } else {
+    MAU_LDS_ATTR(lds, &first_wgrad_kernel<false, BN>);
+    MAU_LAUNCH((first_wgrad_kernel<false, BN>), grid, dim3(NT), lds, st, p, bn);
+  }
+  const int rc = check_launch("first_wgrad_kernel");
+  if (rc != MAU_OK) return rc;
+  MAU_LAUNCH(first_wgrad_sum_kernel, dim3(ceil_div(p.Cout * Cin * 9, SUM_EL)), dim3(SUM_SL * SUM_EL), 0, st, p.ws, (int)grid.x,
+             coTiles, dw, p.Cout, Cin);
+  return check_launch("first_wgrad_sum_kernel");
+}
 }
 }
 
@@ -485,7 +607,7 @@
   MAU_REQUIRE(Cin >= 1 && Cin <= 8, "conv3x3_first_wgrad: %d input channels (this kernel serves <= 8; use mau_conv3x3_wgrad2)", Cin);
   MAU_REQUIRE(dtype == MAU_BF16 || dtype == MAU_F16, "conv3x3_first_wgrad: 16-bit activation types only");
   MAU_REQUIRE(lddz % 8 == 0 && lddz >= Cout && ((uintptr_t)x8 % 16) == 0 && ((uintptr_t)dz % 16) == 0, "conv3x3_first_wgrad: bad lddz / alignment");
-  firstw::WP p;
+  firstw::WP p{};
   p.x8 = x8;
   p.dz = dz;
   p.lddz = lddz;
@@ -494,25 +616,40 @@
   p.N = N;
   p.H = H;
   p.W = W;
-  p.tilesX = ceil_div(W, firstw::TWW);
-  p.nTiles = N * H * p.tilesX;
-  const int coTiles = round_up(Cout, 64) / 64;
-  const dim3 grid(firstw::grid_x(p.nTiles), coTiles);
-  constexpr size_t lds = (size_t)firstw::NWAVE * 2 * firstw::BUF;
-  static_assert(lds >= 64 * firstw::NCOL * sizeof(float), "the cross-wave sum fits the DMA buffers");
-  hipStream_t st = (hipStream_t)stream;
-  if (dtype == MAU_F16) {
-    MAU_LDS_ATTR(lds, &firstw::first_wgrad_kernel<true>);
-    MAU_LAUNCH(firstw::first_wgrad_kernel<true>, grid, dim3(firstw::NT), lds, st, p);
-  } else {
-    MAU_LDS_ATTR(lds, &firstw::first_wgrad_kernel<false>);
-    MAU_LAUNCH(firstw::first_wgrad_kernel<false>, grid, dim3(firstw::NT), lds, st, p);
-  }
-  const int rc = check_launch("first_wgrad_kernel");
-  if (rc != MAU_OK) return rc;
-  MAU_LAUNCH(firstw::first_wgrad_sum_kernel, dim3(ceil_div(Cout * Cin * 9, firstw::SUM_EL)), dim3(firstw::SUM_SL * firstw::SUM_EL), 0, st, ws, (int)grid.x,
-             coTiles, dw, Cout, Cin);
-  return check_launch("first_wgrad_sum_kernel");
-}
-
-}
+  return firstw::launch<false>(p, firstw::BNArgs{}, dw, Cin, dtype, stream);
+}
+
+int mau_conv3x3_first_wgrad_bn(const void* x8, const void* da, int ldda, const void* z, int ldz, const float* scale, const float* shift,
+                               const float* mean, const float* invstd, const double* sums, double count, float* dw, float* ws, int Cin,
+                               int Cout, int dtype, int N, int H, int W, mau_stream_t stream) {
+  using namespace mau;
+  MAU_REQUIRE(x8 && da && z && scale && shift && mean && invstd && sums && dw && ws && N > 0 && H > 0 && W > 0 && Cout > 0 && count >= 0,
+              "conv3x3_first_wgrad_bn: bad arguments");
+  MAU_REQUIRE(Cin >= 1 && Cin <= 8, "conv3x3_first_wgrad_bn: %d input channels (this kernel serves <= 8)", Cin);
+  MAU_REQUIRE(dtype == MAU_BF16 || dtype == MAU_F16, "conv3x3_first_wgrad_bn: 16-bit activation types only");
+  const int C8 = round_up(Cout, 8);
+  MAU_REQUIRE(ldda % 8 == 0 && ldz % 8 == 0 && ldda >= C8 && ldz >= C8, "conv3x3_first_wgrad_bn: bad ld");
+  MAU_REQUIRE(((uintptr_t)x8 % 16) == 0 && ((uintptr_t)da % 16) == 0 && ((uintptr_t)z % 16) == 0, "conv3x3_first_wgrad_bn: bad alignment");
+  firstw::WP p{};
+  p.x8 = x8;
+  p.lddz = C8;
+  p.Cout = Cout;
+  p.ws = ws;
+  p.N = N;
+  p.H = H;
+  p.W = W;
+  firstw::BNArgs bn;
+  bn.da = da;
+  bn.z = z;
+  bn.ldda = ldda;
+  bn.ldz = ldz;
+  bn.scale = scale;
+  bn.shift = shift;
+  bn.mean = mean;
+  bn.invstd = invstd;
+  bn.sums = sums;
+  bn.inv_count = count > 0 ? 1.0 / count : 0.0;
+  return firstw::launch<true>(p, bn, dw, Cin, dtype, stream);
+}
+
+}
diff --git a/metadata-augmented-unet-for-lst-ndvi_amd/csrc/mau_common.h b/metadata-augmented-unet-for-lst-ndvi_amd/csrc/mau_common.h
--- a/metadata-augmented-unet-for-lst-ndvi_amd/csrc/mau_common.h
+++ b/metadata-augmented-unet-for-lst-ndvi_amd/csrc/mau_common.h
@@ -75,6 +75,28 @@
   return r;
 }
 template <typename T>
+struct Lp8;
+template <>
+struct Lp8<bf16> {
+  typedef bf16x8 vec;
+  static __device__ __forceinline__ vec from(const F8& r) {
+    vec a;
+#pragma unroll
+    for (int i = 0; i < 8; ++i) a[i] = (bf16)r.v[i];
+    return a;
+  }
+};
+template <>
+struct Lp8<f16> {
+  typedef f16x8 vec;
+  static __device__ __forceinline__ vec from(const F8& r) {
+    vec a;
+#pragma unroll
+    for (int i = 0; i < 8; ++i) a[i] = (f16)opaque(r.v[i]);
+    return a;
+  }
+};
+template <typename T>
 __device__ __forceinline__ void store8(T* p, const F8& r);
 template <>
 __device__ __forceinline__ void store8<float>(float* p, const F8& r) {
@@ -89,18 +111,12 @@
 }
 template <>
 __device__ __forceinline__ void store8<bf16>(bf16* p, const F8& r) {
-  bf16x8 a;
-#pragma unroll
-  for (int i = 0; i < 8; ++i) a[i] = (bf16)r.v[i];
-  *reinterpret_cast<bf16x8*>(p) = a;
+  *reinterpret_cast<bf16x8*>(p) = Lp8<bf16>::from(r);
 }
 
 template <>
 __device__ __forceinline__ void store8<f16>(f16* p, const F8& r) {
-  f16x8 a;
-#pragma unroll
-  for (int i = 0; i < 8; ++i) a[i] = (f16)opaque(r.v[i]);
-  *reinterpret_cast<f16x8*>(p) = a;
+  *reinterpret_cast<f16x8*>(p) = Lp8<f16>::from(r);
 }
 
 template <typename T>
@@ -148,18 +164,12 @@
 }
 template <>
 __device__ __forceinline__ void store8_nt<bf16>(bf16* p, const F8& r) {
-  bf16x8 a;
-#pragma unroll
-  for (int i = 0; i < 8; ++i) a[i] = (bf16)r.v[i];
-  __builtin_nontemporal_store(a, reinterpret_cast<bf16x8*>(p));
+  __builtin_nontemporal_store(Lp8<bf16>::from(r), reinterpret_cast<bf16x8*>(p));
 }
 
 template <>
 __device__ __forceinline__ void store8_nt<f16>(f16* p, const F8& r) {
-  f16x8 a;
-#pragma unroll
-  for (int i = 0; i < 8; ++i) a[i] = (f16)opaque(r.v[i]);
-  __builtin_nontemporal_store(a, reinterpret_cast<f16x8*>(p));
+  __builtin_nontemporal_store(Lp8<f16>::from(r), reinterpret_cast<f16x8*>(p));
 }
 
 __device__ __forceinline__ float coef(const float* __restrict__ p, int c, int C) {
diff --git a/metadata-augmented-unet-for-lst-ndvi_amd/functional.py b/metadata-augmented-unet-for-lst-ndvi_amd/functional.py
--- a/metadata-augmented-unet-for-lst-ndvi_amd/functional.py
+++ b/metadata-augmented-unet-for-lst-ndvi_amd/functional.py
@@ -300,6 +300,7 @@
 _PACK_MULTI = True
 _INFER_POOL_FUSED = True
 _FIRST_WGRAD = True
+_FIRST_DZ_FUSED_MIN_WORK = 2 * 64 * 64 + 1
 _SIDE_STREAMS = {}
 
 
@@ -322,6 +323,7 @@
 
 _Geom = namedtuple("_Geom", "N H W Cin Cout ldy code act_dt dev stream")
 _Saved = namedtuple("_Saved", "x x1 emb weight y scale shift mean invstd a w2 out argidx")
+_DzOperands = namedtuple("_DzOperands", "da sums count")
 
 
 def _ptr(t):
@@ -547,9 +549,10 @@
     ctx.save_for_backward(*_Saved(x, x1, emb, weight, y, *coef, a, head[2] if head is not None else None, out, argidx))
 
 
-def _dz_begin(g: _Geom, sv):
+def _dz_begin(g: _Geom, sv, need_dy=True):
     slab = torch.empty((lib.mau_bn_bwd_rows(g.N * g.H * g.W), 2 * g.Cout), dtype=torch.float32, device=g.dev)
-    return slab, torch.empty_like(sv.y), (sv.scale.data_ptr(), sv.shift.data_ptr(), sv.mean.data_ptr(), sv.invstd.data_ptr())
+    dy = torch.empty_like(sv.y) if need_dy else None
+    return slab, dy, (sv.scale.data_ptr(), sv.shift.data_ptr(), sv.mean.data_ptr(), sv.invstd.data_ptr())
 
 
 def _finish_sums(g: _Geom, st: BNState, slab):
@@ -594,9 +597,9 @@
     return dy, g32, None, None
 
 
-def _dz_generic(g: _Geom, st: BNState, ctx, sv, da, dpl):
+def _dz_generic(g: _Geom, st: BNState, ctx, sv, da, dpl, apply=True):
     y, ldy, npix, stream = sv.y, g.ldy, g.N * g.H * g.W, g.stream
-    slab, dy, cptrs = _dz_begin(g, sv)
+    slab, dy, cptrs = _dz_begin(g, sv, apply)
     dhw = dhb = None
     if ctx.head is not None:
         _, tanh0, hshape, _ = ctx.head
@@ -614,6 +617,8 @@
     da = _as_nhwc(da)
     call("mau_bn_relu_bwd_reduce", da.data_ptr(), _ld(da), y.data_ptr(), ldy, *cptrs, slab.data_ptr(), g.Cout, g.code, npix, g.Cout, stream)
     sums, count, g32 = _finish_sums(g, st, slab)
+    if not apply:
+        return _DzOperands(da, sums, count), g32, dhw, dhb
     call("mau_bn_relu_bwd_apply", da.data_ptr(), _ld(da), y.data_ptr(), ldy, *cptrs, sums.data_ptr(), count, dy.data_ptr(), ldy, g.code, npix, g.Cout, stream)
     return dy, g32, dhw, dhb
 
@@ -640,7 +645,13 @@
     dw = slot.view_as(weight) if (slot is not None and weight.is_leaf and weight.grad is None and slot.device == g.dev) else torch.empty_like(weight)
     wstream = side.cuda_stream if side is not None else g.stream
     deferred = side is not None and overlap >= 2 and weight.is_leaf and weight.grad is None
-    if st.first and _FIRST_WGRAD:
+    reads = (x, x1, emb, dy)
+    if isinstance(dy, _DzOperands):
+        reads = (x, dy.da, dy.sums, sv.y, sv.scale, sv.shift, sv.mean, sv.invstd)
+        call("mau_conv3x3_first_wgrad_bn", x.data_ptr(), dy.da.data_ptr(), _ld(dy.da), sv.y.data_ptr(), g.ldy, sv.scale.data_ptr(), sv.shift.data_ptr(),
+             sv.mean.data_ptr(), sv.invstd.data_ptr(), dy.sums.data_ptr(), dy.count, dw.data_ptr(), acc.data_ptr(), g.Cin, g.Cout, g.code, g.N, g.H, g.W,
+             wstream)
+    elif st.first and _FIRST_WGRAD:
         call("mau_conv3x3_first_wgrad", x.data_ptr(), dy.data_ptr(), g.ldy, dw.data_ptr(), acc.data_ptr(), g.Cin, g.Cout, g.code, g.N, g.H, g.W, wstream)
     else:
         call("mau_conv3x3_wgrad2", x.data_ptr(), _ld(x), st.C0, _ptr(x1), _ld(x1) if x1 is not None else 0, C1,
@@ -649,7 +660,7 @@
         call("mau_conv3x3_unpack_wgrad", acc.data_ptr(), lib.mau_conv3x3_wgrad_splits(g.code, g.N, g.H, g.W, g.Cout, g.Cin),
              dw.data_ptr(), g.Cout, g.Cin, wstream)
     if deferred:
-        for t in (x, x1, emb, dy, dw):
+        for t in (*reads, dw):
             if t is not None:
                 t.record_stream(side)
         weight._mau_grad_stream = side
@@ -711,7 +722,10 @@
         needs = ctx.needs_input_grad
         dz = (_dz_fused_head if (ctx.head is not None and ctx.head[3])
               else _dz_fused_pool if (ctx.pooled and dpl is not None and sv.argidx is not None) else _dz_generic)
-        dy, g32, dhw, dhb = dz(g, st, ctx, sv, da, dpl)
+        if dz is _dz_generic and st.first and _FIRST_WGRAD and needs[3] and N * H * W >= _FIRST_DZ_FUSED_MIN_WORK:
+            dy, g32, dhw, dhb = _dz_generic(g, st, ctx, sv, da, dpl, apply=False)
+        else:
+            dy, g32, dhw, dhb = dz(g, st, ctx, sv, da, dpl)
         dgamma, dbeta = g32[Cout:], g32[:Cout]
         need_dx = needs[0] or (sv.x1 is not None and needs[1]) or (E and needs[2])
         overlap = _OVERLAP_WGRAD
```

After: 2635 images/s, median of 6. 1.2% higher.
